# olsonanl/signature_kmers

Hardware: AMD Instinct MI355X
Metric: k-mers/sec (extract+hash+count) at 1/2/4/8 GPUs; achieved HBM GB/s % (higher is better)
Workload: dtype u8

## Files before the change

### signature_kmers_amd/__init__.py

```python
from __future__ import annotations

import ctypes as C
import os
from dataclasses import dataclass

import numpy as np

__all__ = [
    "SkmError", "lib", "K", "UNDEFINED_FUNCTION", "STORED_DTYPE", "CALL_DTYPE",
    "SignatureBuilder", "KeptKmers", "CmphKmerDb", "FunctionCaller", "mph_build",
    "kmer_to_str", "str_to_kmer", "keys_from_strings", "device_count", "MatrixDistance", "SeqIdMap",
    "matrix_tile_rows", "KeptKmerDb", "DeviceKeptKmerDb", "kept_db_plan", "kept_slot",
]

K = 8
UNDEFINED_FUNCTION = 0xFFFF
_HERE = os.path.dirname(os.path.abspath(__file__))
LIB_PATH = os.environ.get("SKM_LIB_PATH") or os.path.join(_HERE, "libskm.so")

STORED_DTYPE = np.dtype([("avg_from_end", "<u2"), ("function_index", "<u2"), ("mean", "<u2"),
                         ("median", "<u2"), ("var", "<u2")])
CALL_DTYPE = np.dtype([("start", "<u4"), ("end", "<u4"), ("count", "<i4"), ("function_index", "<u2"),
                       ("pad", "<u2"), ("protein_length_median", "<u4"),
                       ("protein_length_med_avg_dev", "<f4")])
# ... 269 lines not shown
    def __init__(self, k):
        self.k = k

    def __del__(self):
        try:
            lib().skm_kept_free(C.byref(self.k))
        except Exception:
            pass


class SignatureBuilder:

    def __init__(self, n_functions: int, max_seqs_per_file: int = 100000, device: int = 0, rank: int = 0,
                 world_size: int = 1):
        self._h = C.c_void_p()
        opts = _BuildOpts(8, max_seqs_per_file, n_functions, 1, rank, world_size)
        self.rank, self.world_size = rank, world_size
        dev = (C.c_int * 1)(device)
        _check(lib().skm_build_create(C.byref(self._h), dev, 1, C.byref(opts)))
        self.n_functions = n_functions
        self.device = device

    def add_batch(self, residues, seq_off, seq_len, seq_func, seq_id=None):
        residues = np.ascontiguousarray(residues, dtype=np.uint8)
        seq_off = np.ascontiguousarray(seq_off, dtype=np.uint64)
        seq_len = np.ascontiguousarray(seq_len, dtype=np.uint32)
        seq_func = np.ascontiguousarray(seq_func, dtype=np.uint16)
        n = len(seq_len)
        assert len(seq_off) == n and len(seq_func) == n
        if n:
            end = seq_off.astype(np.int64) + seq_len.astype(np.int64)
            if end.max() > len(residues):
                raise SkmError("seq_off/seq_len exceed the residue buffer")
        sid = None if seq_id is None else np.ascontiguousarray(seq_id, dtype=np.uint32)
        _check(lib().skm_build_add_batch(self._h, _ptr(residues), _ptr(seq_off), _ptr(seq_len), _ptr(seq_func),
                                         _ptr(sid) if sid is not None else None, n))

    def reserve(self, n_residues: int, n_seqs: int):
        _check(lib().skm_build_reserve(self._h, int(n_residues), int(n_seqs)))

    def set_transport(self, transport: "GlooTransport"):
        self._transport = transport
        _check(lib().skm_build_set_transport(self._h, transport.ptr))

    def set_comm(self, unique_id: bytes):
        buf = (C.c_uint8 * 128).from_buffer_copy(bytes(unique_id))
        _check(lib().skm_build_set_comm(self._h, buf))

    def prepare(self):
        _check(lib().skm_build_prepare(self._h))

    def run(self):
        _check(lib().skm_build_run(self._h))

    def timings(self) -> dict:
        ms = (C.c_float * 17)()
        n = lib().skm_build_last_timings(self._h, ms, 17)
        names = ["extract_count", "scan", "extract_scatter", "bucket_process", "overflow", "chains", "stats", "total",
                 "exchange", "partition", "bucket_kernel", "big_groups", "chain_tail", "giant_start", "giant_end",
                 "tail_wait", "groupby_wait"]
        return {names[i]: float(ms[i]) for i in range(n)}

    def set_kernel_timing(self, enable: bool, only: str | None = None):
        _check(lib().skm_build_set_kernel_timing(self._h, 1 if enable else 0, only.encode() if only else None))

    def kernel_timings(self) -> dict:
        n = lib().skm_build_kernel_timings(self._h, None, 0, None, None, 0)
        if n <= 0:
            return {}
        ms = (C.c_float * n)()
        cnt = (C.c_uint64 * n)()
        buf = C.create_string_buffer(64 * n + 64)
        lib().skm_build_kernel_timings(self._h, buf, len(buf), ms, cnt, n)
        names = buf.value.decode().split("\n")[:n]
        return {names[i]: (float(ms[i]), int(cnt[i])) for i in range(n)}

    def set_option(self, name: str, value: int):
        _check(lib().skm_build_set_option(self._h, name.encode(), int(value)))

    def passes(self) -> int:
        return self.counters()["passes"]

    def counters(self) -> dict:
        v = (C.c_uint64 * 50)()
        n = lib().skm_build_counters(self._h, v, 50)
        names = ["windows", "kept", "overflow_subbuckets", "chain_jobs", "chain_samples", "sequences", "grouped",
                 "overflow_elements", "overflow_kept", "big_groups", "big_kept", "passes", "valid", "giant_chains",
                 "giant_max", "redone", "cap_overflow_scratch", "cap_split", "cap_long_samples", "cap_long_jobs",
                 "demand_overflow_scratch", "demand_split", "demand_long_samples", "demand_long_jobs",
                 "long_samples", "routed", "add_batch_us", "prepare_upload_us", "prepare_plan_us", "prepare_rest_us",
                 "pass_groups", "add_pack_us", "add_dma_wait_us", "finish_us", "finish_wait_us", "finish_copy_us",
                 "finish_chunks", "finish_select_dev_us", "finish_sort_dev_us", "finish_gather_dev_us",
                 "finish_d2h_dev_us", "finish_max_chunk", "finish_wide_index", "kept_cap",
                 "free_after_prepare", "recs_rot", "overflow_light_subbuckets", "overflow_light_elements",
                 "groupby_tasks", "groupby_batches"]
        return {names[i]: int(v[i]) for i in range(n)}

    def debug_jobs(self, k: int = 64) -> list:
        v = (C.c_uint32 * k)()
        _check(lib().skm_build_debug_jobs(self._h, v, k))
        return [int(x) for x in v]

    def debug_overflow(self, k: int = 4096) -> list:
        v = (C.c_uint32 * k)()
        n = lib().skm_build_debug_overflow(self._h, v, k)
        return [int(x) for x in v[:min(max(n, 0), k)]]

    def debug_stamps(self, enable: bool) -> list:
        v = (C.c_uint64 * 32)()
        _check(lib().skm_build_debug_stamps(self._h, 1 if enable else 0, v, 32))
        return [int(x) for x in v]

    def finish(self) -> KeptKmers:
        k = _Kept()
        _check(lib().skm_build_finish(self._h, C.byref(k)))
        return self._kept(k)

    def finish_slice(self, slice_bits: int, slice_: int) -> KeptKmers:
        k = _Kept()
        _check(lib().skm_build_finish_slice(self._h, int(slice_bits), int(slice_), C.byref(k)))
        return self._kept(k)

    def signature_flags(self) -> np.ndarray:
        n = self.counters()["sequences"]
        out = np.zeros(max(n, 1), np.uint8)
        _check(lib().skm_build_signature_flags(self._h, _ptr(out), n))
        return out[:n]

    def kept_db(self, load_pct: int = 0, slots: int = 0, release_work: bool = False) -> "DeviceKeptKmerDb":
        opts = _KeptDbOpts(int(load_pct), 1 if release_work else 0, int(slots))
        h = C.c_void_p()
        _check(lib().skm_build_kept_db(self._h, C.byref(opts), C.byref(h)))
        return DeviceKeptKmerDb(h, self.device)

    def mph_db(self, seed: int = 1, release_work: bool = False, verify: bool = False, mph_path: str | None = None,
               dat_path: str | None = None) -> "CmphKmerDb":
        opts = _MphDbOpts(int(seed), 1 if release_work else 0, 1 if verify else 0, 0,
                          mph_path.encode() if mph_path else None, dat_path.encode() if dat_path else None)
        h = C.c_void_p()
        st = _MphStats()
        _check(lib().skm_build_mph_db(self._h, C.byref(opts), C.byref(h), C.byref(st)))
        db = CmphKmerDb(device=self.device, handle=h)
        db.stats = {n: getattr(st, n) for n, _ in _MphStats._fields_ if n != "pad"}
        return db

    @staticmethod
    def _kept(k) -> KeptKmers:
        owner = _KeptOwner(k)
        n = int(k.n)
        if n:
            kb = (C.c_char * (8 * n)).from_address(C.cast(k.keys, C.c_void_p).value)
            db = (C.c_char * (10 * n)).from_address(C.cast(k.data, C.c_void_p).value)
            kb._owner = db._owner = owner
            keys = np.frombuffer(kb, np.uint64)
            data = np.frombuffer(db, STORED_DTYPE)
        else:
            keys, data = np.zeros(0, np.uint64), np.zeros(0, STORED_DTYPE)
        nf = int(k.n_functions)
        df = np.ctypeslib.as_array(k.distinct_functions, shape=(max(nf, 1),))[:nf].copy()
        sw = np.ctypeslib.as_array(k.seqs_with_func, shape=(max(nf, 1),))[:nf].copy()
        return KeptKmers(keys, data, df, sw, int(k.n_seqs_with_signature), int(k.distinct_signatures),
                         int(k.n_windows))

    def close(self):
        if self._h:
            lib().skm_build_destroy(self._h)
            self._h = C.c_void_p()

    def __del__(self):
        try:
            self.close()
        except Exception:
            pass


class GlooTransport:

    def __init__(self):
# ... 743 lines not shown
```

### signature_kmers_amd/csrc/skm_build.hip

```cpp
#include <hip/hip_runtime.h>

#include <algorithm>
#include <type_traits>
#include <chrono>
#include <cmath>
#include <cstdio>
#include <cstdlib>
#include <cstring>
#include <deque>
#include <memory>
#include <numeric>
#include <string>
#include <thread>
#include <vector>

#include "skm_common.h"
#include "skm_keptdb.h"
#include "skm_mphdb.h"
#include "skm_pool.h"
#include "skm_output.h"
#include "skm_util.h"

#if defined(SKM_WITH_RCCL)
#include <rccl/rccl.h>
// ... 275 lines not shown
            uint32_t t = s_wave[w];
            s_wave[w] = acc;
            acc += t;
        }
        s_wave[nw] = acc;
    }
    __syncthreads();
    uint32_t r = s_wave[wave] + x - v;
    total = s_wave[nw];
    __syncthreads();
    return r;
}

__device__ __forceinline__ uint32_t wg_exclusive_scan1(uint32_t v, uint32_t* s_wave, uint32_t& total) {
    const uint32_t lane = threadIdx.x & 63u, wave = threadIdx.x >> 6, nw = blockDim.x >> 6;
    const uint32_t x = wave_incl_scan(v);
    if (lane == 63) s_wave[wave] = x;
    __syncthreads();
    uint32_t pre = 0, tot = 0;
    for (uint32_t w = 0; w < nw; ++w) {
        const uint32_t t = s_wave[w];
        pre += w < wave ? t : 0u;
        tot += t;
    }
    total = tot;
    return pre + x - v;
}

constexpr uint64_t LENS_SEL_SHIFT = 62;
constexpr uint64_t LENS_IN_RECS = 1, LENS_IN_TMP = 2, LENS_IN_BIG = 3;
constexpr uint64_t LENS_OFF_MASK = (1ull << LENS_SEL_SHIFT) - 1;
constexpr int SMALLC = 8;

struct Job {
    uint64_t lens_off;
    uint32_t n;
    uint32_t out_idx;
};

struct GRes {
    uint32_t best_f, avg, cbest, rb;
    uint16_t mean, median, var;
    bool kept;
};


struct GlbView {
    const uint64_t* hi;
    const uint64_t* lo;
    __device__ __forceinline__ uint32_t func(uint64_t j) const { return (uint32_t)(hi[j] & 0xFFFFu); }
    __device__ __forceinline__ uint64_t lov(uint64_t j) const { return lo[j]; }
};

template <int N>
__device__ __forceinline__ void reg_sort(uint32_t* v) {
#pragma unroll
    for (int k = 2; k <= N; k <<= 1)
#pragma unroll
        for (int j = k >> 1; j > 0; j >>= 1)
#pragma unroll
            for (int i = 0; i < N; ++i) {
                const int l = i ^ j;
                if (l > i) {
                    const bool asc = (i & k) == 0;
                    const uint32_t a = v[i], b = v[l];
                    v[i] = asc ? min(a, b) : max(a, b);
                    v[l] = asc ? max(a, b) : min(a, b);
                }
            }
}

__device__ __forceinline__ void stats_small(GRes& r, uint32_t x0, uint32_t x1, uint32_t n) {
    r.median = 0;
    r.var = 0;
    if (n == 2) {
        const uint16_t sum = (uint16_t)(x0 + x1);
        const double mean = (double)sum / 2.0;
        const double tmp = (double)x1 - mean;
        const double v = 0.0 * 1.0 / 2.0 + tmp * tmp / 1.0;
        r.var = d2u16(v);
    }
}

__device__ __forceinline__ void mark_seq(uint32_t* f, uint32_t s) {
    uint32_t* w = f + (s >> 5);
    const uint32_t m = 1u << (s & 31u);
    if (!(*w & m)) atomicOr(w, m);
}

template <int N>
__device__ __forceinline__ void mark_seqs(uint32_t* w, const uint32_t (&s)[N]) {
    uint32_t cur[N];
#pragma unroll
    for (int u = 0; u < N; ++u) cur[u] = s[u] != 0xFFFFFFFFu ? w[s[u] >> 5] : 0xFFFFFFFFu;
#pragma unroll
    for (int u = 0; u < N; ++u) {
        const uint32_t m = 1u << (s[u] & 31u);
        if (!(cur[u] & m)) atomicOr(w + (s[u] >> 5), m);
    }
}

struct Seq8 {
    uint32_t s[8];
};
__device__ __attribute__((noinline)) void mark_seqs8(uint32_t* w, Seq8 q) { mark_seqs<8>(w, q.s); }

template <int N, class V>
__device__ GRes group_thread(const V& v, uint64_t a, uint32_t c, const uint32_t* __restrict__ glen,
                             uint32_t* __restrict__ flags) {
    GRes r;
    r.kept = false;
    uint32_t fn[N], of[N];
#pragma unroll
    for (int t = 0; t < N; ++t) {
        if ((uint32_t)t < c) {
            fn[t] = v.func(a + t);
            of[t] = (uint32_t)(v.lov(a + t) & 0xFFFFu);
        } else {
            fn[t] = 0x10000u;
            of[t] = 0x10000u;
        }
    }
    uint32_t best_f = fn[0], best_c = 0, rb = 0, run_s = 0;
#pragma unroll
    for (int t = 1; t <= N; ++t) {
        if ((uint32_t)t <= c) {
            const bool end = ((uint32_t)t == c) || fn[t < N ? t : N - 1] != fn[t - 1];
            if (end) {
                const uint32_t len = t - run_s;
                if (len > best_c) {
                    best_c = len;
                    best_f = fn[t - 1];
                    rb = run_s;
                }
                run_s = t;
            }
        }
    }
    if ((float)best_c < float(c) * 0.8f) return r;
    r.kept = true;
    r.best_f = best_f;
    r.cbest = best_c;
    r.rb = rb;
    reg_sort<N>(of);
    const uint32_t k = c / 2;
    uint32_t avg = 0;
#pragma unroll
    for (int t = 0; t < N; ++t)
        if ((uint32_t)t == k) avg = of[t];
    r.avg = avg;
    uint32_t sum = 0;
    uint32_t lr0 = 0, lr1 = 0;
    for (uint32_t t = 0; t < c; ++t) {
        const uint64_t lo = v.lov(a + t);
        const uint32_t s = (uint32_t)(lo >> 36);
        mark_seq(flags, s);
        if (t >= rb && t < rb + best_c) {
            const uint32_t len = glen[s];
            sum += len;
            const uint32_t q = rb + best_c - 1 - t;
            if (q == 0) lr0 = len;
            if (q == 1) lr1 = len;
        }
    }
    r.mean = d2u16((double)(uint16_t)sum / (double)best_c);
    r.median = 0;
    r.var = 0;
    if (best_c <= 2) stats_small(r, lr0, lr1, best_c);
    return r;
}

template <class V>
__device__ GRes group_wave(const V& v, uint64_t a, uint32_t c, const uint32_t* __restrict__ glen,
                           uint32_t* __restrict__ flags) {
    const uint32_t lane = threadIdx.x & 63u;
    GRes r;
    r.kept = false;
    uint32_t best_f = 0, best_c = 0, rb = 0, run_s = 0;
    uint32_t run_f = v.func(a);
    for (uint32_t base = 0; base < c; base += 64) {
        const uint32_t t = base + lane;
        const bool valid = t < c;
        const uint32_t f = valid ? v.func(a + t) : 0xFFFFFFFFu;
        const uint32_t fp = (valid && t > 0) ? v.func(a + t - 1) : 0xFFFFFFFFu;
        uint64_t m = __ballot(valid && t > 0 && f != fp);
        while (m) {
            const int q = __ffsll((long long)m) - 1;
            m &= m - 1;
            const uint32_t pos = base + (uint32_t)q;
            const uint32_t len = pos - run_s;
            if (len > best_c) {
                best_c = len;
                best_f = run_f;
                rb = run_s;
            }
            run_s = pos;
            run_f = (uint32_t)__shfl((int)f, q, 64);
        }
    }
    {
        const uint32_t len = c - run_s;
        if (len > best_c) {
            best_c = len;
            best_f = run_f;
            rb = run_s;
        }
    }
    if ((float)best_c < float(c) * 0.8f) return r;
    r.kept = true;
    r.best_f = best_f;
    r.cbest = best_c;
    r.rb = rb;
    uint32_t vmin = 0xFFFFu, vmax = 0;
    for (uint32_t t = lane; t < c; t += 64) {
        const uint32_t o = (uint32_t)(v.lov(a + t) & 0xFFFFu);
        vmin = min(vmin, o);
        vmax = max(vmax, o);
    }
    vmin = wave_min(vmin);
    vmax = wave_max(vmax);
    const uint32_t k = c / 2;
    while (vmin < vmax) {
        const uint32_t mid = (vmin + vmax) >> 1;
        uint32_t cnt = 0;
        for (uint32_t t = lane; t < c; t += 64) cnt += (uint32_t)(v.lov(a + t) & 0xFFFFu) <= mid;
        cnt = wave_sum(cnt);
        if (cnt >= k + 1)
            vmax = mid;
        else
            vmin = mid + 1;
    }
    r.avg = vmin;
    uint32_t sum = 0;
    for (uint32_t t = lane; t < c; t += 64) {
        const uint32_t s = (uint32_t)(v.lov(a + t) >> 36);
        mark_seq(flags, s);
        if (t >= rb && t < rb + best_c) sum += glen[s];
    }
    sum = wave_sum(sum);
    r.mean = d2u16((double)(uint16_t)sum / (double)best_c);
    r.median = 0;
    r.var = 0;
    return r;
}

__device__ __forceinline__ uint32_t wg_sum(uint32_t x, uint32_t* s_wave) {
    const uint32_t lane = threadIdx.x & 63u, wave = threadIdx.x >> 6, nw = blockDim.x >> 6;
    x = wave_sum(x);
    if (lane == 0) s_wave[wave] = x;
    __syncthreads();
    uint32_t t = 0;
    for (uint32_t w = 0; w < nw; ++w) t += s_wave[w];
    __syncthreads();
    return t;
}

__device__ __forceinline__ uint32_t wg_max(uint32_t x, uint32_t* s_wave) {
    const uint32_t lane = threadIdx.x & 63u, wave = threadIdx.x >> 6, nw = blockDim.x >> 6;
    x = wave_max(x);
    if (lane == 0) s_wave[wave] = x;
    __syncthreads();
    uint32_t t = 0;
    for (uint32_t w = 0; w < nw; ++w) t = max(t, s_wave[w]);
    __syncthreads();
    return t;
}

__device__ __forceinline__ uint32_t wg_min(uint32_t x, uint32_t* s_wave) {
    const uint32_t lane = threadIdx.x & 63u, wave = threadIdx.x >> 6, nw = blockDim.x >> 6;
    x = wave_min(x);
    if (lane == 0) s_wave[wave] = x;
    __syncthreads();
    uint32_t t = 0xFFFFFFFFu;
    for (uint32_t w = 0; w < nw; ++w) t = min(t, s_wave[w]);
    __syncthreads();
    return t;
}

template <class V>
__device__ bool group_block(const V& v, uint64_t a, uint32_t c, const uint32_t* __restrict__ glen,
                            uint32_t* __restrict__ flags, uint32_t* heads, uint32_t hcap, uint32_t* s_wave, GRes& r) {
    const uint32_t tid = threadIdx.x, nt = blockDim.x;
    r.kept = false;
    uint32_t H = 0;
    for (uint32_t t0 = 0; t0 < c; t0 += nt) {
        const uint32_t t = t0 + tid;
        const bool head = t < c && (t == 0 || v.func(a + t) != v.func(a + t - 1));
        uint32_t tot;
        const uint32_t pos = wg_exclusive_scan(head ? 1u : 0u, s_wave, tot);
        if (head && H + pos < hcap) heads[H + pos] = t;
        H += tot;
    }
    if (H > hcap) return false;
    __syncthreads();
    uint32_t lmax = 0;
    for (uint32_t j = tid; j < H; j += nt) lmax = max(lmax, (j + 1 < H ? heads[j + 1] : c) - heads[j]);
    const uint32_t best_c = wg_max(lmax, s_wave);
    uint32_t fmin = 0xFFFFFFFFu;
    for (uint32_t j = tid; j < H; j += nt)
        if ((j + 1 < H ? heads[j + 1] : c) - heads[j] == best_c) fmin = min(fmin, (v.func(a + heads[j]) << 16) | j);
    const uint32_t fj = wg_min(fmin, s_wave);
    if ((float)best_c < float(c) * 0.8f) return true;
    const uint32_t rb = heads[fj & 0xFFFFu];
    r.kept = true;
    r.best_f = fj >> 16;
    r.cbest = best_c;
    r.rb = rb;
    uint32_t k = c / 2, pre = 0;
    for (int b = 15; b >= 0; --b) {
        uint32_t n0 = 0;
        for (uint32_t t = tid; t < c; t += nt) {
            const uint32_t o = (uint32_t)(v.lov(a + t) & 0xFFFFu);
            n0 += (o >> b) == (pre >> b);
        }
        n0 = wg_sum(n0, s_wave);
        if (k >= n0) {
            k -= n0;
            pre |= 1u << b;
        }
    }
    r.avg = pre;
    uint32_t sum = 0;
    for (uint32_t t = tid; t < c; t += nt) {
        const uint32_t s = (uint32_t)(v.lov(a + t) >> 36);
        mark_seq(flags, s);
        if (t >= rb && t < rb + best_c) sum += glen[s];
    }
    sum = wg_sum(sum, s_wave);
    r.mean = d2u16((double)(uint16_t)sum / (double)best_c);
    r.median = 0;
    r.var = 0;
    return true;
}

enum : uint32_t {
    RUN_FLAGS = 0,
    RUN_LONG_CUR = 1,
    RUN_LONG_N = 2,
    RUN_LONG_FLUSHED = 3,
    RUN_ACC_BPK_TASKS = 4,
    RUN_ACC_BPK_BATCHES = 5,
    RUN_SNAP = 28,
    RUN_DEM_TOT = 8,
    RUN_DEM_SPLIT = 9,
    RUN_DEM_LONG = 10,
    RUN_DEM_LJOBS = 11,
    RUN_LONG_WANT = 12,
    RUN_LONG_WANTJ = 13,
    RUN_ACC_LIGHT_SUB = 14,
    RUN_ACC_LIGHT_ELEMS = 15,
    RUN_ACC_NOVF = 16,
    RUN_ACC_JOBS = 17,
    RUN_ACC_LENS = 18,
    RUN_ACC_OVF_ELEMS = 19,
    RUN_ACC_OVF_KEPT = 20,
    RUN_ACC_BIG = 21,
    RUN_ACC_BIG_KEPT = 22,
    RUN_ACC_GROUPED = 23,
    RUN_LAST_NOVF = 24,
    RUN_LAST_JOBS = 25,
    RUN_NLOC = 26,
    RUN_SLOTS = 64
};
constexpr unsigned long long RUN_F_ARENA = 1;
constexpr unsigned long long RUN_F_RERUN = 2;
constexpr unsigned long long RUN_F_CAP = 4;
enum : uint32_t {
    PLAN_NOVF = 0,
    PLAN_NSPLIT = 1,
    PLAN_NHEAVY = 2,
    PLAN_SKIP = 3,
    PLAN_Q_SPLIT = 4,
    PLAN_Q_HEAVY = 5,
    PLAN_Q_REST = 6,
    PLAN_Q_LIGHT = 7,
    PLAN_ELEMS = 8,
    PLAN_NLOC = 9,
    PLAN_SLOTS = 16
};

constexpr int JOB_CLASSES = 32;
constexpr int JOB_WG = 256;

__device__ __forceinline__ uint32_t job_class(uint32_t n) { return 31u - (uint32_t)__clz(n | 1u); }

__device__ __forceinline__ void job_chunk(const unsigned long long* nj_p, uint64_t cap, uint64_t& a, uint64_t& e) {
    const uint64_t nj = min((uint64_t)*nj_p, cap);
    const uint64_t chunk = (nj + gridDim.x - 1) / gridDim.x;
    a = min(nj, (uint64_t)blockIdx.x * chunk);
    e = min(nj, a + chunk);
}

__global__ __launch_bounds__(JOB_WG) void k_job_count(const Job* __restrict__ jobs, const unsigned long long* nj_p,
                                                      uint64_t cap, uint32_t* __restrict__ hist) {
    __shared__ uint32_t h[JOB_CLASSES];
    if (threadIdx.x < JOB_CLASSES) h[threadIdx.x] = 0;
    __syncthreads();
    uint64_t a, e;
    job_chunk(nj_p, cap, a, e);
    for (uint64_t j = a + threadIdx.x; j < e; j += blockDim.x) atomicAdd(&h[job_class(jobs[j].n)], 1u);
    __syncthreads();
    if (threadIdx.x < JOB_CLASSES) hist[blockIdx.x * JOB_CLASSES + threadIdx.x] = h[threadIdx.x];
}

constexpr uint32_t LONG_CLASS = 14;

__global__ void k_job_scan(const uint32_t* __restrict__ hist, uint32_t nwg, uint64_t* __restrict__ offs,
                           uint32_t long_class) {
    __shared__ uint64_t tot[JOB_CLASSES];
    const uint32_t c = threadIdx.x;
    if (c < JOB_CLASSES) {
        uint64_t t = 0;
        for (uint32_t w = 0; w < nwg; ++w) t += hist[w * JOB_CLASSES + c];
        tot[c] = t;
    }
    __syncthreads();
    if (c == 0) {
        uint64_t nl = 0;
        for (uint32_t cc = long_class; cc < JOB_CLASSES; ++cc) nl += tot[cc];
        offs[(uint64_t)nwg * JOB_CLASSES] = nl;
    }
    if (c < JOB_CLASSES) {
        uint64_t base = 0;
        for (uint32_t cc = JOB_CLASSES - 1; cc > c; --cc) base += tot[cc];
// ... 1414 lines not shown
    if (b >= NB) return;
    uint32_t w0 = rb * SCAN_ROWS, w1 = min(nwg, w0 + SCAN_ROWS);
    uint32_t s = 0;
    for (uint32_t w = w0; w < w1; ++w) s += hist[(uint64_t)w * NB + b];
    partial[(uint64_t)rb * NB + b] = s;
}

__global__ void k_bstart(const uint32_t* __restrict__ partial, uint32_t nrb, uint32_t NB, int b1_bits,
                         uint32_t* __restrict__ rbbase, uint32_t* __restrict__ bstart, uint64_t* __restrict__ owner_start,
                         uint32_t nowners) {
    __shared__ uint32_t s_wave[34];
    __shared__ unsigned long long s_tot[64];
    const uint32_t per = (NB + blockDim.x - 1) / blockDim.x;
    const uint32_t b0 = threadIdx.x * per;
    uint32_t local = 0;
    for (uint32_t b = b0; b < min(NB, b0 + per); ++b) {
        uint32_t acc = 0;
        for (uint32_t rb = 0; rb < nrb; ++rb) {
            uint32_t v = partial[(uint64_t)rb * NB + b];
            rbbase[(uint64_t)rb * NB + b] = acc;
            acc += v;
        }
        bstart[b] = acc;
        local += acc;
    }
    uint32_t total;
    uint32_t ex = wg_exclusive_scan(local, s_wave, total);
    uint32_t run = ex;
    for (uint32_t b = b0; b < min(NB, b0 + per); ++b) {
        uint32_t t = bstart[b];
        bstart[b] = run;
        run += t;
    }
    __syncthreads();
    if (threadIdx.x < nowners) {
        uint32_t ob = threadIdx.x << b1_bits;
        s_tot[threadIdx.x] = bstart[ob];
    }
    if (threadIdx.x == 0) s_tot[nowners] = total;
    __syncthreads();
    if (threadIdx.x <= nowners) owner_start[threadIdx.x] = s_tot[threadIdx.x];
    for (uint32_t b = b0; b < min(NB, b0 + per); ++b) {
        uint32_t o = b >> b1_bits;
        uint32_t rel = bstart[b] - (uint32_t)s_tot[o];
        for (uint32_t rb = 0; rb < nrb; ++rb) rbbase[(uint64_t)rb * NB + b] += rel;
    }
    __syncthreads();
    for (uint32_t b = b0; b < min(NB, b0 + per); ++b) bstart[b] -= (uint32_t)s_tot[b >> b1_bits];
    if (threadIdx.x == 0) bstart[NB] = 0;
}

__global__ void k_coloffs(const uint32_t* __restrict__ hist, const uint32_t* __restrict__ rbbase, uint32_t nwg, uint32_t NB,
                          uint32_t* __restrict__ offs) {
    uint32_t b = blockIdx.x * blockDim.x + threadIdx.x;
    uint32_t rb = blockIdx.y;
    if (b >= NB) return;
    uint32_t w0 = rb * SCAN_ROWS, w1 = min(nwg, w0 + SCAN_ROWS);
    uint32_t run = rbbase[(uint64_t)rb * NB + b];
    for (uint32_t w = w0; w < w1; ++w) {
        uint64_t idx = (uint64_t)w * NB + b;
        uint32_t v = hist[idx];
        offs[idx] = run;
        run += v;
    }
}

struct BucketArgs {
    uint64_t* recs_hi;
    const uint64_t* recs_lo;
    uint64_t* tmp_hi;
    uint64_t* tmp_lo;
    const uint64_t* bstart;
    const uint64_t* seg_start;
    const uint32_t* seg_len;
    uint32_t nsrc;
    uint32_t* sub_tab;
    unsigned long long* kept_ctr;

    uint32_t nbuckets;
    uint32_t bucket_base;
    int rem_bits;
    const uint32_t* glen;
    uint32_t* flags;
    unsigned long long* ctr;
    uint64_t* out_keys;
    skm_stored_kmer_data* out_data;
    Job* jobs;
    uint32_t* lens;
    OvfEntry* ovf;
    uint32_t ovf_cap;
    unsigned long long* stamps;
    uint64_t* big_desc;
    uint32_t big_cap;
    unsigned long long* big_ctr;
    int prio;
    int pshift;
    const uint32_t* skip;
    uint32_t sub_target;
    const uint32_t* order;
};

#define SKM_STAMP(i)                                                          \
    do {                                                                      \
        if (A.stamps && threadIdx.x == 0) {                                   \
            const uint64_t _t = __builtin_amdgcn_s_memtime();                 \
            atomicAdd(&A.stamps[(i)], (unsigned long long)(_t - *L.tlast));   \
            *L.tlast = _t;                                                    \
        }                                                                     \
    } while (0)

constexpr uint32_t JOB_KEPT = 0x8000u;
constexpr uint32_t JOB_COUNT_MASK = 0x0FFFu;

struct SubLds {
    uint64_t* hi;
    uint64_t* lo;
    uint32_t* tab;
    uint16_t* slot;
    uint16_t* rank;
    uint16_t* goff;
    uint16_t* glist;
    uint16_t* order;
    uint16_t* big;
    uint32_t* wave;
    uint32_t* nbig;
    uint64_t* tlast;
    uint32_t* ccnt;
    uint32_t* lens32;
    uint64_t lens_sel;
};

__device__ __forceinline__ uint64_t kept_hi(uint64_t h43, uint32_t avg) { return (1ull << 63) | (h43 << 16) | avg; }
__device__ __forceinline__ uint64_t kept_lo(uint32_t f, uint32_t mean, uint32_t med, uint32_t var) {
    return (uint64_t)f | ((uint64_t)mean << 16) | ((uint64_t)med << 32) | ((uint64_t)var << 48);
}

__device__ __forceinline__ void write_kept(const BucketArgs& A, uint64_t o, uint64_t H, uint64_t L) {
    A.out_keys[o] = (H >> 16) & KEY_MASK;
    skm_stored_kmer_data d;
    d.avg_from_end = (uint16_t)(H & 0xFFFFu);
    d.function_index = (uint16_t)(L & 0xFFFFu);
    d.mean = (uint16_t)(L >> 16);
    d.median = (uint16_t)(L >> 32);
    d.var = (uint16_t)(L >> 48);
    A.out_data[o] = d;
}



__device__ __forceinline__ uint64_t shfl_xor_u64(uint64_t v, int m) {
    return ((uint64_t)(uint32_t)__shfl_xor((int)(uint32_t)(v >> 32), m, 64) << 32) |
           (uint32_t)__shfl_xor((int)(uint32_t)v, m, 64);
}


__device__ __forceinline__ void bm_combine(uint32_t& cand, uint32_t& cc) {
#pragma unroll
    for (int d = 1; d < 64; d <<= 1) {
        const uint32_t oc = xs(cand, d), on = xs(cc, d);
        if (oc == cand) {
            cc += on;
        } else if (cc >= on) {
            cc -= on;
        } else {
            cand = oc;
            cc = on - cc;
// ... 19 lines not shown
        }
    }
    return key;
}

template <int S>
__device__ __forceinline__ uint32_t seg_bitonic32(uint32_t key, uint32_t m) {
#pragma unroll
    for (int k = 2; k <= S; k <<= 1) {
#pragma unroll
        for (int j = k >> 1; j > 0; j >>= 1) {
            const uint32_t ok = xs(key, j);
            const bool take_min = ((m & (uint32_t)j) == 0) == ((m & (uint32_t)k) == 0);
            key = take_min ? min(key, ok) : max(key, ok);
        }
    }
    return key;
}

template <int S>
__device__ __forceinline__ uint32_t seg_reduce_max(uint32_t x) {
#pragma unroll
    for (int d = 1; d < S; d <<= 1) x = max(x, xs(x, d));
    return x;
}

template <int S>
__device__ __forceinline__ uint32_t seg_reduce_sum(uint32_t x) {
#pragma unroll
    for (int d = 1; d < S; d <<= 1) x += xs(x, d);
    return x;
}

template <int S>
__device__ __forceinline__ void seg_groups(const SubLds& L, uint32_t q0, uint32_t qend, uint32_t G, uint32_t M,
                                           const BucketArgs& A, uint64_t hprefix, uint32_t* jobinfo,
                                           uint32_t* fmean) {
    const uint32_t lane = threadIdx.x & 63u;
    const uint32_t m = lane & (uint32_t)(S - 1);
    const uint32_t sbase = lane - m;
    const uint32_t q = q0 + lane / (uint32_t)S;
    const bool gv = q < qend;
    uint32_t rep = 0, a = 0, c = 0;
    if (gv) {
        const uint32_t g = L.big[q];
        rep = L.glist[g];
        a = L.goff[rep];
        c = (g + 1 < G ? L.goff[L.glist[g + 1]] : M) - a;
    }
    const bool real = gv && m < c;
    uint64_t key = ~0ull;
    uint32_t pay = 0;
    if (real) {
        const uint32_t j = L.order[a + m];
        const uint64_t hj = L.hi[j], lj = L.lo[j];
        key = ((hj & 0xFFFFull) << 48) | (lj >> 16);
        pay = (uint32_t)(hj >> 47);
    }
    key = seg_bitonic64<S>(key, pay, m);
    const uint32_t f = (uint32_t)(key >> 48);
    const uint32_t fprev = (uint32_t)__shfl_up((int)f, 1, 64);
    const bool head = !real || m == 0 || f != fprev;
    const uint64_t H = __ballot(head);
    const uint64_t above = lane == 63 ? 0ull : (H & ~((2ull << lane) - 1ull));
    const uint32_t nh = above ? (uint32_t)__ffsll((long long)above) - 1u : 64u;
    const uint32_t rlen = min(nh, sbase + c) - lane;
    const uint32_t v = (real && head) ? ((rlen << 16) | (0xFFFFu - f)) : 0u;
    const uint32_t best = seg_reduce_max<S>(v);
    const uint32_t cbest = best >> 16, bf = 0xFFFFu - (best & 0xFFFFu);
    const bool kept = gv && !((float)cbest < float(c) * 0.8f);
    const bool inrun = real && f == bf;
    const uint32_t len16 = pay >> 1;
    const uint32_t sum = seg_reduce_sum<S>(inrun ? len16 : 0u);
    const uint32_t i = (uint32_t)(key & ((1u << ELEM_I_BITS) - 1));
    const uint32_t off = real ? ((len16 - i) & 0xFFFFu) : 0x10000u;
    const uint32_t osort = seg_bitonic32<S>(off, m);
    const uint32_t avg = (uint32_t)__shfl((int)osort, (int)(sbase + (c >> 1)), 64);
    const uint64_t R = __ballot(inrun);
    const uint64_t segmask = (S == 64) ? ~0ull : (((1ull << S) - 1ull) << sbase);
    const uint64_t Rs = R & segmask;
    const uint32_t rs = Rs ? (uint32_t)__ffsll((long long)Rs) - 1u : sbase;
    const uint32_t s = (uint32_t)(key >> ELEM_I_BITS) & ((1u << ELEM_S_BITS) - 1u);
    const uint32_t len = (pay & 1u) ? A.glen[s] : len16;
    if (kept && real) mark_seq(A.flags, s);
    const uint32_t x0 = (uint32_t)__shfl((int)len, (int)(rs + cbest - 1), 64);
    const uint32_t x1 = (uint32_t)__shfl((int)len, (int)rs, 64);
    if (kept && inrun && cbest >= 3) L.lens32[2 * a + (rs + cbest - 1 - lane)] = len;
    if (kept && m == 0) {
        GRes r;
        r.kept = true;
        r.best_f = bf;
        r.cbest = cbest;
        r.avg = avg;
        r.mean = d2u16((double)(uint16_t)sum / (double)cbest);
        stats_small(r, x0, cbest == 2 ? x1 : 0u, cbest);
        const uint64_t h43 = key_h43(hprefix, (L.hi[rep] >> 16) & REM_MASK, A.rem_bits, A.pshift);
        L.hi[rep] = kept_hi(h43, r.avg);
        if (cbest >= 3) {
            jobinfo[rep] = (a << 16) | JOB_KEPT | cbest;
            fmean[rep] = bf | ((uint32_t)r.mean << 16);
        } else {
            jobinfo[rep] = JOB_KEPT;
            L.lo[rep] = kept_lo(bf, r.mean, r.median, r.var);
        }
    }
}

constexpr uint32_t LPER = CAP / BPK_THREADS;

__device__ __forceinline__ void load_batch(const uint64_t* __restrict__ src_hi, const uint64_t* __restrict__ src_lo,
                                           uint32_t n, uint64_t (&eh)[LPER], uint64_t (&el)[LPER]) {
#pragma unroll
    for (uint32_t u = 0; u < LPER; ++u) {
        const uint32_t j = threadIdx.x + u * BPK_THREADS;
        if (j < n) {
            eh[u] = __builtin_nontemporal_load(src_hi + j);
            el[u] = __builtin_nontemporal_load(src_lo + j);
        }
    }
}

__device__ __forceinline__ uint32_t process_sub(const uint64_t* __restrict__ src_hi, const uint64_t* __restrict__ src_lo,
                                            uint32_t n, const BucketArgs& A, uint64_t hprefix, const SubLds& L) {
    const uint32_t tid = threadIdx.x, nt = blockDim.x;
    const uint32_t EMPTY = 0xFFFFFFFFu;
    uint64_t eh[LPER], el[LPER];
    load_batch(src_hi, src_lo, n, eh, el);
    for (uint32_t t = tid; t < (uint32_t)TAB; t += nt) L.tab[t] = EMPTY;
#pragma unroll
    for (uint32_t u = 0; u < LPER; ++u) {
        const uint32_t j = tid + u * BPK_THREADS;
        if (j < n) {
            L.hi[j] = eh[u];
            L.lo[j] = el[u];
        }
    }
    if (tid == 0) *L.nbig = 0;
    if (tid < 8) L.ccnt[tid] = 0;
    __syncthreads();
    SKM_STAMP(2);
    for (uint32_t j = tid; j < n; j += nt) {
        const uint32_t rem = (uint32_t)(L.hi[j] >> 16) & REM_MASK;
        uint32_t slot = (rem * 0x9E3779B1u) >> (32 - TAB_BITS);
        uint32_t rk = 0;
        while (true) {
            const uint32_t cur = atomicCAS(&L.tab[slot], EMPTY, (j << 16) | 1u);
            if (cur == EMPTY) break;
            if (((uint32_t)(L.hi[cur >> 16] >> 16) & REM_MASK) == rem) {
                rk = atomicAdd(&L.tab[slot], 1u) & 0xFFFFu;
                break;
            }
            slot = (slot + 1) & (TAB - 1);
        }
        L.slot[j] = (uint16_t)slot;
        L.rank[j] = (uint16_t)rk;
    }
    __syncthreads();
    SKM_STAMP(3);
    uint32_t M = 0, G = 0;
    {
        const uint32_t j0 = tid * LPER;
        uint32_t ev[LPER], loc = 0;
#pragma unroll
        for (uint32_t u = 0; u < LPER; ++u) {
            const uint32_t j = j0 + u;
            ev[u] = j < n ? L.tab[L.slot[j]] : 0u;
            const uint32_t cnt = ev[u] & 0xFFFFu;
            loc += (cnt > 1 && (ev[u] >> 16) == j) ? ((cnt << 13) | 1u) : 0u;
        }
        uint32_t tot;
        uint32_t v = wg_exclusive_scan1(loc, L.wave, tot);
        uint32_t ms[LPER];
#pragma unroll
        for (uint32_t u = 0; u < LPER; ++u) {
            const uint32_t j = j0 + u;
            const uint32_t cnt = ev[u] & 0xFFFFu;
            ms[u] = 0xFFFFFFFFu;
            if (j < n && cnt > 1 && (ev[u] >> 16) == j) {
                L.goff[j] = (uint16_t)(v >> 13);
                L.glist[v & 0x1FFFu] = (uint16_t)j;
                v += (cnt << 13) | 1u;
            } else if (j < n && cnt == 1) {
                const uint64_t H = L.hi[j], Lo = L.lo[j];
                ms[u] = (uint32_t)(Lo >> 36);
                L.hi[j] = kept_hi(key_h43(hprefix, (H >> 16) & REM_MASK, A.rem_bits, A.pshift), (uint32_t)(Lo & 0xFFFFu));
                L.lo[j] = kept_lo((uint32_t)(H & 0xFFFFu), d2u16((double)(uint16_t)(H >> 48) / 1.0), 0, 0);
                L.rank[j] = 0xFFFFu;
            }
        }
        mark_seqs<LPER>(A.flags, ms);
        M = tot >> 13;
        G = tot & 0x1FFFu;
    }
    __syncthreads();
    SKM_STAMP(4);
    for (uint32_t j = tid; j < n; j += nt) {
        const uint32_t e = L.tab[L.slot[j]];
        if ((e & 0xFFFFu) > 1) L.order[L.goff[e >> 16] + L.rank[j]] = (uint16_t)j;
    }
    uint32_t* ccnt = L.ccnt;
    auto cls_of = [](uint32_t c) -> uint32_t {
        return c > 64u ? 6u : 31u - (uint32_t)__clz(c - 1u) - 0u;
    };
    for (uint32_t g = tid; g < G; g += nt) {
        const uint32_t a = L.goff[L.glist[g]];
        const uint32_t c = g + 1 < G ? L.goff[L.glist[g + 1]] - a : M - a;
        atomicAdd(&ccnt[cls_of(c)], 1u);
    }
    __syncthreads();
    SKM_STAMP(5);
    uint32_t* jobinfo = L.tab;
    uint32_t* fmean = L.tab + CAP;
    for (uint32_t j = tid; j < n; j += nt) jobinfo[j] = L.rank[j] == 0xFFFFu ? JOB_KEPT : 0u;
    uint32_t* cstart = ccnt + 8;
    uint32_t* tstart = ccnt + 16;
    if (tid == 0) {
        uint32_t run = 0, acc = 0;
        for (int q = 0; q < 7; ++q) {
            const uint32_t t = ccnt[q];
            ccnt[q] = run;
            cstart[q] = run;
            tstart[q] = acc;
            const uint32_t per = q < 6 ? (64u >> (q + 1)) : 1u;
            acc += (t + per - 1) / per;
            run += t;
        }
        cstart[7] = run;
        tstart[7] = acc;
    }
    unsigned long long big_base = 0;
    if (tid == 0 && cstart[7] > cstart[6]) big_base = atomicAdd(A.big_ctr, (unsigned long long)(cstart[7] - cstart[6]));
    __syncthreads();
    for (uint32_t g = tid; g < G; g += nt) {
        const uint32_t a = L.goff[L.glist[g]];
        const uint32_t c = g + 1 < G ? L.goff[L.glist[g + 1]] - a : M - a;
        L.big[atomicAdd(&ccnt[cls_of(c)], 1u)] = (uint16_t)g;
    }
    if (tid == 0) *reinterpret_cast<unsigned long long*>(L.wave + 44) = big_base;
    __syncthreads();
    SKM_STAMP(6);
    {
        const uint32_t ntask = tstart[6];
        const uint32_t nbig = cstart[7] - cstart[6];
        const uint64_t bbase = *reinterpret_cast<const unsigned long long*>(L.wave + 44);
        const uint32_t wave = tid >> 6, nwaves = nt >> 6, lane = tid & 63u;
        uint64_t* slots = reinterpret_cast<uint64_t*>(L.lens32);
        uint64_t* slots_lo = const_cast<uint64_t*>(src_lo);
        (void)wave;
        (void)nwaves;
        for (;;) {
            uint32_t t = 0;
            if (lane == 0) t = atomicAdd(&ccnt[7], 1u);
            t = (uint32_t)__builtin_amdgcn_readfirstlane((int)t);
            if (t >= nbig + ntask) break;
            if (t < nbig) {
                const uint32_t g = L.big[cstart[6] + t];
                const uint32_t rep = L.glist[g];
                const uint32_t a = L.goff[rep];
                const uint32_t c = g + 1 < G ? L.goff[L.glist[g + 1]] - a : M - a;
                for (uint32_t u = lane; u < c; u += 64) {
                    const uint32_t j = L.order[a + u];
                    const uint64_t hj = L.hi[j], lj = L.lo[j];
                    slots[a + u] = ((hj & 0xFFFFull) << 48) | (lj >> 16);
                    slots_lo[a + u] = elem_len(hj, lj, A.glen);
                }
                const uint64_t q = bbase + t;
                if (lane == 0 && q < A.big_cap) {
                    A.big_desc[2 * q] = key_h43(hprefix, (L.hi[rep] >> 16) & REM_MASK, A.rem_bits, A.pshift) |
                                        ((uint64_t)c << KEY_BITS);
                    A.big_desc[2 * q + 1] = L.lens_sel + 2 * a;
                }
                continue;
            }
// ... 141 lines not shown
        __syncthreads();
        if (task >= ntasks) break;
        const uint32_t bucket = task / BPK_PARTS, part = task % BPK_PARTS;
        const uint64_t r0 = A.bstart[bucket], r1 = A.bstart[bucket + 1];
        const uint64_t n = r1 - r0;
        if (n == 0) continue;
        const uint64_t hprefix = (uint64_t)(A.bucket_base + bucket) << A.rem_bits;

        const bool direct = n <= (uint64_t)CAP && A.nsrc == 1;
        uint32_t nsub = 1;
        if (direct) {
            if (part) continue;
        } else {
            const uint32_t* tab = A.sub_tab + (uint64_t)bucket * SUB_TAB;
            const uint32_t all = tab[0];
            const uint32_t d0 = (uint32_t)((uint64_t)part * all / BPK_PARTS), d1 = (uint32_t)((uint64_t)(part + 1) * all / BPK_PARTS);
            if (d0 == d1) continue;
            nsub = d1 - d0;
            for (uint32_t d = threadIdx.x; d <= nsub; d += blockDim.x) s_sub[d] = tab[1 + d0 + d];
            __syncthreads();
            SKM_STAMP(9);
        }
        struct Batch {
            uint32_t a, cnt;
        };
        auto next_batch = [&](uint32_t& d) -> Batch {
            if (direct) {
                if (d >= 1) return Batch{0, 0};
                d = 1;
                return Batch{0, (uint32_t)n};
            }
            while (d < nsub) {
                const uint32_t a = s_sub[d];
                if (s_sub[d + 1] - a == 0 || s_sub[d + 1] - a > (uint32_t)CAP) {
                    ++d;
                    continue;
                }
                uint32_t d2 = d + 1;
                while (d2 < nsub && s_sub[d2 + 1] - a <= (uint32_t)CAP) ++d2;
                d = d2;
                return Batch{a, s_sub[d2] - a};
            }
            return Batch{0, 0};
        };
        const uint64_t* base_hi = A.tmp_hi + r0;
        const uint64_t* base_lo = A.tmp_lo + r0;
        const uint64_t sel = LENS_IN_TMP;
        uint32_t d = 0, nb = 0;
        for (Batch cur = next_batch(d); cur.cnt; cur = next_batch(d)) {
            L.lens_sel = (sel << LENS_SEL_SHIFT) | (2 * (r0 + cur.a));
            L.lens32 = reinterpret_cast<uint32_t*>(const_cast<uint64_t*>(base_hi + cur.a));
            process_sub(base_hi + cur.a, base_lo + cur.a, cur.cnt, A, hprefix, L);
            __syncthreads();
            SKM_STAMP(10);
            ++nb;
        }
        worked += nb ? 1u : 0u;
        batches += nb;
    }
    if (threadIdx.x == 0 && worked) {
        atomicAdd(&A.ctr[CTR_BPK_TASKS], (unsigned long long)worked);
        atomicAdd(&A.ctr[CTR_BPK_BATCHES], (unsigned long long)batches);
    }
}

struct BigOut {
    uint64_t h43;
    uint64_t lens_off;
    uint32_t n;
    uint16_t avg, func, mean, pad0;
    uint32_t pad1;
};
static_assert(sizeof(BigOut) == 32, "BigOut layout");

struct BigArgs {
    const uint64_t* desc;
    const unsigned long long* ndesc;
    uint32_t cap;
    const uint64_t* recs_hi;
    const uint64_t* tmp_hi;
    const uint64_t* recs_lo;
    const uint64_t* tmp_lo;
    uint32_t* flags;
    BigOut* out;
};

template <int E>
__device__ __forceinline__ uint32_t ballot_count(const bool (&p)[E]) {
    uint32_t n = 0;
#pragma unroll
    for (int e = 0; e < E; ++e) n += (uint32_t)__popcll(__ballot(p[e]));
    return n;
}

template <int E, int D>
__device__ __forceinline__ void bitonic_cross(uint64_t (&ky)[E], bool take_min) {
#pragma unroll
    for (int e = 0; e < E; ++e) {
        const uint64_t o = xshfl64<D>(ky[e]);
        ky[e] = take_min ? (o < ky[e] ? o : ky[e]) : (o > ky[e] ? o : ky[e]);
    }
}

template <int E>
__device__ __forceinline__ void big_group(const BigArgs& B, uint64_t g, uint64_t* mem, const uint64_t* mlen,
                                          uint32_t c, uint64_t h43, uint64_t lens_off) {
    const uint32_t lane = threadIdx.x & 63u;
    uint32_t fo[E];
    uint64_t ky[E];
#pragma unroll
    for (int e = 0; e < E; ++e) {
        const uint32_t t = lane * E + (uint32_t)e;
        fo[e] = 0xFFFFFFFFu;
        ky[e] = ~0ull;
        if (t < c) {
            const uint64_t v = mem[t];
            const uint32_t len = (uint32_t)mlen[t];
            const uint32_t i = (uint32_t)v & ((1u << ELEM_I_BITS) - 1u);
            fo[e] = ((uint32_t)(v >> 48) << 16) | ((len - i) & 0xFFFFu);
            ky[e] = (v << 16) | t;
        }
    }
    uint32_t cand = 0xFFFFFFFFu, cc = 0;
#pragma unroll
    for (int e = 0; e < E; ++e) {
        if (fo[e] != 0xFFFFFFFFu) {
            const uint32_t f = fo[e] >> 16;
            if (cc == 0) {
                cand = f;
                cc = 1;
            } else if (f == cand) {
                ++cc;
            } else {
                --cc;
            }
        }
    }
    bm_combine(cand, cc);
    bool p[E];
#pragma unroll
    for (int e = 0; e < E; ++e) p[e] = (fo[e] >> 16) == cand;
    const uint32_t nb = ballot_count<E>(p);
    BigOut o;
    o.h43 = h43;
    o.lens_off = lens_off;
    o.n = 0;
    o.avg = o.func = o.mean = 0;
    o.pad0 = 0;
    o.pad1 = 0;
    if ((float)nb < float(c) * 0.8f) {
        if (lane == 0) B.out[g] = o;
        return;
    }
    constexpr int MC = E < 8 ? E : 8;
#pragma unroll
    for (int e0 = 0; e0 < E; e0 += MC) {
        uint32_t ms[MC];
#pragma unroll
        for (int u = 0; u < MC; ++u)
            ms[u] = fo[e0 + u] != 0xFFFFFFFFu ? (uint32_t)(ky[e0 + u] >> (16 + ELEM_I_BITS)) : 0xFFFFFFFFu;
        if constexpr (E > 16) {
            Seq8 q;
#pragma unroll
            for (int u = 0; u < 8; ++u) q.s[u] = ms[u];
            mark_seqs8(B.flags, q);
        } else {
            mark_seqs<MC>(B.flags, ms);
        }
    }
    uint32_t sum = 0;
#pragma unroll
    for (int e = 0; e < E; ++e) {
        if (fo[e] != 0xFFFFFFFFu && p[e]) sum += (uint32_t)mlen[ky[e] & 0xFFFFu];
        if (!p[e]) ky[e] = ~0ull;
    }
    sum = wave_sum(sum);
    uint32_t k = c / 2, pre = 0;
#pragma unroll 1
    for (int b = 15; b >= 0; --b) {
#pragma unroll
        for (int e = 0; e < E; ++e) {
            const uint32_t v = fo[e] == 0xFFFFFFFFu ? 0x10000u : (fo[e] & 0xFFFFu);
            p[e] = ((v >> b) ^ (pre >> b)) == 0u;
        }
        const uint32_t n0 = ballot_count<E>(p);
        if (k >= n0) {
            k -= n0;
            pre |= 1u << b;
        }
    }
#pragma unroll 1
    for (uint32_t kk = 2; kk <= 64u * E; kk <<= 1) {
        const bool asc_lane = ((lane * (uint32_t)E) & kk) == 0;
#pragma unroll 1
        for (uint32_t jj = kk >> 1; jj >= (uint32_t)E; jj >>= 1) {
            const uint32_t d = jj / (uint32_t)E;
            const bool take_min = ((lane & d) == 0) == asc_lane;
            switch (d) {
                case 1: bitonic_cross<E, 1>(ky, take_min); break;
                case 2: bitonic_cross<E, 2>(ky, take_min); break;
                case 4: bitonic_cross<E, 4>(ky, take_min); break;
                case 8: bitonic_cross<E, 8>(ky, take_min); break;
                case 16: bitonic_cross<E, 16>(ky, take_min); break;
                default: bitonic_cross<E, 32>(ky, take_min); break;
            }
        }
#pragma unroll
        for (int jj = E / 2; jj > 0; jj >>= 1) {
            if ((uint32_t)jj < kk) {
#pragma unroll
                for (int e = 0; e < E; ++e) {
                    const int l = e ^ jj;
                    if (l > e) {
                        const bool asc = (((lane * (uint32_t)E) + (uint32_t)e) & kk) == 0;
                        const uint64_t x = ky[e], y = ky[l];
                        const bool sw = asc ? (y < x) : (x < y);
                        ky[e] = sw ? y : x;
                        ky[l] = sw ? x : y;
                    }
                }
            }
        }
    }
    uint32_t* lens = reinterpret_cast<uint32_t*>(mem);
#pragma unroll
    for (int e = 0; e < E; ++e) {
        const uint32_t t = lane * E + (uint32_t)e;
        if (t < nb) lens[nb - 1 - t] = (uint32_t)mlen[ky[e] & 0xFFFFu];
    }
    o.n = nb;
    o.avg = (uint16_t)pre;
    o.func = (uint16_t)cand;
    o.mean = d2u16((double)(uint16_t)sum / (double)nb);
    if (lane == 0) B.out[g] = o;
}

constexpr int BIG_WG = 256;

template <bool LARGE>
__global__ __launch_bounds__(BIG_WG, LARGE ? 3 : 4) void k_big_groups(BigArgs B) {
    const uint64_t nd = min((uint64_t)*B.ndesc, (uint64_t)B.cap);
    const uint64_t nw = (uint64_t)gridDim.x * (BIG_WG / 64);
    for (uint64_t g = (uint64_t)blockIdx.x * (BIG_WG / 64) + (threadIdx.x >> 6); g < nd; g += nw) {
        const uint64_t d0 = B.desc[2 * g], d1 = B.desc[2 * g + 1];
        const uint32_t c = (uint32_t)(d0 >> KEY_BITS);
        if (LARGE != (c > 1024u)) continue;
        const uint64_t h43 = d0 & KEY_MASK;
        const uint64_t sel = d1 >> LENS_SEL_SHIFT, off = d1 & LENS_OFF_MASK;
        uint64_t* mem = const_cast<uint64_t*>(sel == LENS_IN_RECS ? B.recs_hi : B.tmp_hi) + off / 2;
        const uint64_t* mlen = (sel == LENS_IN_RECS ? B.recs_lo : B.tmp_lo) + off / 2;
// ... 341 lines not shown
                    s_lo[j] = ~0ull;
                }
            }
            __syncthreads();
            bitonic_lds(s_hi, s_lo, CAP, 2, CAP, CAP);
            for (uint32_t j = tid; j < CAP; j += nt) {
                ghi[c0 + j] = s_hi[j];
                glo[c0 + j] = s_lo[j];
            }
            __threadfence_block();
            __syncthreads();
        }
        for (uint32_t k = 2 * CAP; k <= N; k <<= 1) {
            for (uint32_t j = k >> 1; j >= (uint32_t)CAP; j >>= 1) {
                for (uint32_t t = tid; t < N / 2; t += nt) {
                    const uint32_t i = 2 * t - (t & (j - 1));
                    if (i >= nch) continue;
                    const uint32_t l = j == (k >> 1) ? (i ^ (k - 1)) : i + j;
                    const uint64_t ah = ghi[i], al = glo[i], bh = ghi[l], bl = glo[l];
                    if (elem_less(bh, bl, ah, al)) {
                        ghi[i] = bh;
                        glo[i] = bl;
                        ghi[l] = ah;
                        glo[l] = al;
                    }
                }
                __threadfence_block();
                __syncthreads();
            }
            for (uint32_t c0 = 0; c0 < nch; c0 += CAP) {
                for (uint32_t j = tid; j < CAP; j += nt) {
                    s_hi[j] = ghi[c0 + j];
                    s_lo[j] = glo[c0 + j];
                }
                __syncthreads();
                bitonic_lds(s_hi, s_lo, CAP, k, k, CAP >> 1);
                for (uint32_t j = tid; j < CAP; j += nt) {
                    ghi[c0 + j] = s_hi[j];
                    glo[c0 + j] = s_lo[j];
                }
                __threadfence_block();
                __syncthreads();
            }
        }
        uint32_t G = 0;
        for (uint32_t c0 = 0; c0 < n; c0 += nt) {
            const uint32_t t = c0 + tid;
            const bool head = t < n && (t == 0 || (ghi[t] >> 16) != (ghi[t - 1] >> 16));
            uint32_t tot;
            const uint32_t pos = wg_exclusive_scan(head ? 1u : 0u, s_wave, tot);
            if (head) {
                heads[G + pos] = t;
                jobinfo[t] = 0;
            }
            G += tot;
        }
        __threadfence_block();
        __syncthreads();
        const GlbView V{ghi, glo};
        auto stage = [&](const GRes& r, uint32_t a) {
            if (!r.kept) return;
            const uint64_t h43 = key_h43(hprefix, ghi[a] >> 16, A.rem_bits, A.pshift);
            if (r.cbest >= 3) {
                jobinfo[a] = ((uint64_t)(a + r.rb) << 32) | r.cbest;
                fmean[a] = r.best_f | ((uint32_t)r.mean << 16);
            } else {
                glo[a] = kept_lo(r.best_f, r.mean, r.median, r.var);
            }
            ghi[a] = kept_hi(h43, r.avg);
        };
        for (uint32_t g0 = 0; g0 < G; g0 += nt) {
            if (tid == 0) s_nbig = 0;
            __syncthreads();
            const uint32_t g = g0 + tid;
            if (g < G) {
                const uint32_t a = heads[g];
                const uint32_t b = g + 1 < G ? heads[g + 1] : n;
                const uint32_t c = b - a;
                if (c > (uint32_t)SMALLC) {
                    s_big[atomicAdd(&s_nbig, 1u)] = g;
                } else {
                    GRes r;
                    if (c <= 4)
                        r = group_thread<4>(V, a, c, A.glen, A.flags);
                    else if (c <= 8)
                        r = group_thread<8>(V, a, c, A.glen, A.flags);
                    else
                        r = group_thread<16>(V, a, c, A.glen, A.flags);
                    stage(r, a);
                }
            }
            __syncthreads();
            const uint32_t nbig = s_nbig;
            for (uint32_t bi = tid >> 6; bi < nbig; bi += nt >> 6) {
                const uint32_t gg = s_big[bi];
                const uint32_t a = heads[gg];
                const uint32_t b = gg + 1 < G ? heads[gg + 1] : n;
                if (b - a > OVF_BLOCK_GROUP) continue;
                const GRes r = group_wave(V, a, b - a, A.glen, A.flags);
                if ((tid & 63u) == 0) stage(r, a);
            }
            for (uint32_t bi = 0; bi < nbig; ++bi) {
                const uint32_t gg = s_big[bi];
                const uint32_t a = heads[gg];
                const uint32_t b = gg + 1 < G ? heads[gg + 1] : n;
                if (b - a <= OVF_BLOCK_GROUP) continue;
                GRes r;
                if (!group_block(V, a, b - a, A.glen, A.flags, reinterpret_cast<uint32_t*>(s_hi), 2 * CAP, s_wave, r)) {
                    if (tid < 64) r = group_wave(V, a, b - a, A.glen, A.flags);
                }
                if (tid == 0) stage(r, a);
                __syncthreads();
            }
            __threadfence_block();
            __syncthreads();
        }
        unsigned long long* s_base = reinterpret_cast<unsigned long long*>(s_wave + 36);
        for (uint32_t g0 = 0; g0 < G; g0 += nt) {
            const uint32_t g = g0 + tid;
            const uint32_t a = g < G ? heads[g] : 0u;
            const uint64_t H = g < G ? ghi[a] : 0ull;
            const bool kept = (H >> 63) != 0;
            const uint64_t jb = kept ? jobinfo[a] : 0ull;
            const uint32_t jn = (uint32_t)(jb & 0xFFFFFFFFu);
            uint32_t islot = OVF_INLINE_CAP;
            if (jn >= inline_min) islot = atomicAdd(&s_ninl, 1u);
            const bool inl = islot < OVF_INLINE_CAP;
            uint32_t K, J, Lt;
            const uint32_t kpos = wg_exclusive_scan(kept ? 1u : 0u, s_wave, K);
            const uint32_t jpos = wg_exclusive_scan((jn && !inl) ? 1u : 0u, s_wave, J);
            const uint32_t lpos = wg_exclusive_scan(jn, s_wave, Lt);
            if (K == 0) continue;
            if (tid == 0) {
                s_base[0] = atomicAdd(A.kept_ctr, (unsigned long long)K);
                atomicAdd(&A.ctr[0], (unsigned long long)K);
                if (J) {
                    s_base[1] = atomicAdd(&A.ctr[3], (unsigned long long)J);
                    s_base[2] = atomicAdd(&A.ctr[4], (unsigned long long)Lt);
                }
                s_nbig = 0;
            }
            __syncthreads();
            if (kept) {
                const uint64_t o = s_base[0] + kpos;
                if (jn) {
                    const uint32_t fm = fmean[a];
                    write_kept(A, o, H, kept_lo(fm & 0xFFFFu, fm >> 16, 0, 0));
                    Job jbr;
                    jbr.lens_off = s_base[2] + lpos;
                    jbr.n = jn;
                    jbr.out_idx = (uint32_t)o;
                    if (inl) {
                        s_inl[islot][0] = jbr.lens_off;
                        s_inl[islot][1] = ((uint64_t)jn << 32) | (uint32_t)o;
                    } else {
                        A.jobs[s_base[1] + jpos] = jbr;
                    }
                    if (jn <= 64) {
                        const uint64_t start = jb >> 32;
                        for (uint32_t t = 0; t < jn; ++t)
                            A.lens[jbr.lens_off + t] = A.glen[glo[start + jn - 1 - t] >> 36];
                    } else {
                        const uint32_t bi = atomicAdd(&s_nbig, 1u);
                        s_big[bi] = g;
                        s_lo[bi] = jbr.lens_off;
                    }
                } else {
                    write_kept(A, o, H, glo[a]);
                }
            }
            __syncthreads();
            const uint32_t nb = s_nbig;
            for (uint32_t q = 0; q < nb; ++q) {
                const uint32_t gg = s_big[q];
                const uint32_t aa = heads[gg];
                const uint64_t jbq = jobinfo[aa];
                const uint32_t nq = (uint32_t)(jbq & 0xFFFFFFFFu);
                const uint64_t start = jbq >> 32;
                const uint64_t loff = s_lo[q];
                for (uint32_t t = tid; t < nq; t += nt) A.lens[loff + t] = A.glen[glo[start + nq - 1 - t] >> 36];
            }
            __syncthreads();
        }
        __threadfence_block();
        __syncthreads();
        const uint32_t ninl = min(s_ninl, OVF_INLINE_CAP);
        const uint32_t wave = tid >> 6, pairs = (nt >> 6) / 2;
        if (ninl && prio == 1) __builtin_amdgcn_s_setprio(1);
        if (ninl && prio == 2) __builtin_amdgcn_s_setprio(2);
        if (ninl && prio >= 3) __builtin_amdgcn_s_setprio(3);
        for (uint32_t q = wave / 2; q < ninl; q += pairs) {
            const uint64_t off = s_inl[q][0], w = s_inl[q][1];
// ... 301 lines not shown
            }
            const uint32_t pre = (uint32_t)__popcll(peers & lt);
            const uint32_t tg = tag & 0x1FFFFFFu;
            if (v && pre == 0) s_wc[wave][d] = (tg << 7) | (uint32_t)__popcll(peers);
            __syncthreads();
            if (v) {
                uint32_t o = s_run[d] + pre;
                for (uint32_t w = 0; w < wave; ++w) {
                    const uint32_t c = s_wc[w][d];
                    if ((c >> 7) == tg) o += c & 127u;
                }
                b[o] = k;
            }
            __syncthreads();
            for (uint32_t dd = tid; dd < RBINS; dd += nt) {
                uint32_t add = 0;
                for (uint32_t w = 0; w < nw; ++w) {
                    const uint32_t c = s_wc[w][dd];
                    if ((c >> 7) == tg) add += c & 127u;
                }
                s_run[dd] += add;
            }
            __syncthreads();
        }
        uint32_t* t = a;
        a = b;
        b = t;
    }
    return a;
}

constexpr uint32_t HV_FT = 4096;
constexpr uint32_t HV_NBK = 4096;
constexpr uint32_t HV_BCAP = 512;

__device__ __forceinline__ void wave_hist_add(uint32_t* h, uint32_t bin, bool v) {
    const uint32_t lane = threadIdx.x & 63u;
    uint64_t act = __ballot(v);
    while (act) {
        const uint32_t l0 = (uint32_t)__ffsll((long long)act) - 1u;
        const uint32_t b0 = (uint32_t)__builtin_amdgcn_readlane((int)bin, (int)l0);
        const uint64_t m = __ballot(v && bin == b0) & act;
        if (lane == l0) atomicAdd(&h[b0], (uint32_t)__popcll(m));
        act &= ~m;
    }
}

template <int E>
__device__ __forceinline__ void wave_sort_desc(uint64_t (&v)[E]) {
    const uint32_t lane = threadIdx.x & 63u;
#pragma unroll
    for (int k = 2; k <= 64 * E; k <<= 1) {
#pragma unroll
        for (int j = k >> 1; j > 0; j >>= 1) {
            if (j >= 64) {
#pragma unroll
                for (int e = 0; e < E; ++e) {
                    const int pe = e ^ (j >> 6);
                    if (pe > e) {
                        const bool up = (((uint32_t)e * 64u + lane) & (uint32_t)k) == 0;
                        const uint64_t a = v[e], b = v[pe];
                        if (up ? a < b : a > b) {
                            v[e] = b;
                            v[pe] = a;
                        }
                    }
                }
            } else {
#pragma unroll
                for (int e = 0; e < E; ++e) {
                    const uint32_t i = (uint32_t)e * 64u + lane;
                    const uint64_t o = xs64(v[e], j);
                    const bool keep_max = ((i & (uint32_t)j) == 0) == ((i & (uint32_t)k) == 0);
                    v[e] = keep_max ? (v[e] > o ? v[e] : o) : (v[e] < o ? v[e] : o);
                }
            }
        }
    }
}

template <int E>
__device__ __forceinline__ void heavy_bucket_out(const uint32_t* __restrict__ ks, const uint32_t* __restrict__ ls,
                                                 uint32_t a, uint32_t c, uint32_t nb, uint32_t* __restrict__ out,
                                                 uint32_t* flags) {
    const uint32_t lane = threadIdx.x & 63u;
    uint64_t v[E];
#pragma unroll
    for (int e = 0; e < E; ++e) {
        const uint32_t i = (uint32_t)e * 64u + lane;
        v[e] = i < c ? ((uint64_t)ks[a + i] << 32) | ls[a + i] : 0ull;
    }
    wave_sort_desc<E>(v);
#pragma unroll
    for (int e = 0; e < E; ++e) {
        const uint32_t i = (uint32_t)e * 64u + lane;
        if (i < nb) {
            out[i] = (uint32_t)v[e];
            mark_seq(flags, (uint32_t)(v[e] >> 32) - 1u);
        }
    }
}

__global__ __launch_bounds__(HEAVY_WG) void k_heavy(BucketArgs A, HeavyArgs H) {
    static_assert(RBINS <= HEAVY_WG, "one radix bin per thread in the scan");
    __shared__ uint32_t s_hist[RBINS], s_run[RBINS + 48];
    __shared__ uint32_t s_wc[HEAVY_WG / 64][RBINS];
    __shared__ __align__(16) uint32_t s_wave[48];
    __shared__ uint32_t s_bm[2 * (HEAVY_WG / 64)];
    __shared__ uint32_t s_cur, s_sel[3], s_key;
    __shared__ uint32_t s_fb[HV_FT];
    __shared__ uint32_t s_bk[HV_NBK];
    __shared__ uint32_t s_oh[256], s_ol[256];
    static_assert(HV_FT == HV_NBK, "s_fb doubles as the per-bucket best counts");
    const uint32_t tid = threadIdx.x, nt = blockDim.x, lane = tid & 63u, wave = tid >> 6, nw = nt >> 6;
    const uint64_t lt = (1ull << lane) - 1ull;
    const uint32_t nkeys = (uint32_t)*H.nkeys;
    uint32_t tag = 0;
    for (uint32_t q = tid; q < (HEAVY_WG / 64) * RBINS; q += nt) (&s_wc[0][0])[q] = 0;
    __syncthreads();
    constexpr uint32_t U = SPLIT_U;
    for (;;) {
        __syncthreads();
        if (tid == 0) s_key = (uint32_t)min((unsigned long long)nkeys, atomicAdd(H.queue, 1ull));
        __syncthreads();
        const uint32_t q = s_key;
        if (q >= nkeys) break;
        const HeavyKey K = H.keys[q];
        const uint64_t* rec = H.rec + K.off;
        const uint32_t* rlen = H.len + K.off;
        const uint32_t n = K.n;
        uint32_t best_f = 0, cb = 0, NBK = 0;
        bool bucketed = false;
        if (H.fast) {
            NBK = 1;
            while (NBK < HV_NBK && NBK * 256u < n) NBK <<= 1;
            for (uint32_t d = tid; d < HV_FT; d += nt) s_fb[d] = 0;
            for (uint32_t d = tid; d < NBK; d += nt) s_bk[d] = 0;
            for (uint32_t d = tid; d < 256; d += nt) s_oh[d] = 0;
            __syncthreads();
            for (uint32_t j0 = 0; j0 < n; j0 += nt * U) {
                uint64_t x[U];
#pragma unroll
                for (uint32_t u = 0; u < U; ++u) {
                    const uint32_t j = j0 + u * nt + tid;
                    x[u] = j < n ? rec[j] : ~0ull;
                }
#pragma unroll
                for (uint32_t u = 0; u < U; ++u) {
                    const bool v = x[u] != ~0ull;
                    const uint32_t f = v ? hr_func(x[u]) : 0xFFFFFFFFu;
                    const uint32_t f0 = (uint32_t)__builtin_amdgcn_readfirstlane((int)f);
                    const uint64_t same = __ballot(v && f == f0);
                    if (v && f != f0) atomicAdd(&s_fb[f], 1u);
                    if (v && f == f0 && (same & lt) == 0) atomicAdd(&s_fb[f], (uint32_t)__popcll(same));
                    wave_hist_add(s_oh, hr_off(x[u]) >> 8, v);
                    if (v) atomicAdd(&s_bk[(uint32_t)(((uint64_t)hr_seq(x[u]) * NBK) / H.n_total)], 1u);
                }
            }
            __syncthreads();
            uint32_t cm = 0;
            for (uint32_t d = tid; d < HV_FT; d += nt) cm = max(cm, s_fb[d]);
            cm = wg_max(cm, s_wave);
            uint32_t fm = 0;
            for (uint32_t d = tid; d < HV_FT; d += nt)
                if (s_fb[d] == cm) fm = max(fm, HV_FT - 1u - d);
            fm = wg_max(fm, s_wave);
            best_f = HV_FT - 1u - fm;
            cb = cm;
            uint32_t bm = 0;
            for (uint32_t d = tid; d < NBK; d += nt) bm = max(bm, s_bk[d]);
            bm = wg_max(bm, s_wave);
            bucketed = bm <= HV_BCAP;
        } else {
            uint32_t cand = 0xFFFFFFFFu, cc = 0;
            for (uint32_t j0 = 0; j0 < n; j0 += nt * U) {
                uint32_t f[U];
    #pragma unroll
                for (uint32_t u = 0; u < U; ++u) {
                    const uint32_t j = j0 + u * nt + tid;
                    f[u] = j < n ? hr_func(rec[j]) : 0xFFFFFFFFu;
                }
// ... 22 lines not shown
                    const uint32_t c1 = s_bm[2 * w], n1 = s_bm[2 * w + 1];
                    if (c1 == c0) {
                        n0 += n1;
                    } else if (n0 >= n1) {
                        n0 -= n1;
                    } else {
                        c0 = c1;
                        n0 = n1 - n0;
                    }
                }
                s_sel[0] = c0;
            }
            __syncthreads();
            best_f = s_sel[0];
            cb = 0;
            for (uint32_t j0 = 0; j0 < n; j0 += nt * U) {
                uint32_t f[U];
    #pragma unroll
                for (uint32_t u = 0; u < U; ++u) {
                    const uint32_t j = j0 + u * nt + tid;
                    f[u] = j < n ? hr_func(rec[j]) : 0xFFFFFFFFu;
                }
    #pragma unroll
                for (uint32_t u = 0; u < U; ++u) cb += f[u] == best_f;
            }
            cb = wg_sum(cb, s_wave);
        }
        if ((float)cb < float(n) * 0.8f) continue;
        uint32_t pre = 0;
        uint16_t mean = 0;
        const uint32_t* sorted = nullptr;
        if (bucketed) {
            {
                const uint32_t per = (NBK + nt - 1) / nt, b0 = min(NBK, tid * per), b1 = min(NBK, b0 + per);
                uint32_t loc = 0;
                for (uint32_t d = b0; d < b1; ++d) loc += s_bk[d];
                uint32_t tot;
                uint32_t x = wg_exclusive_scan(loc, s_wave, tot);
                for (uint32_t d = b0; d < b1; ++d) {
                    const uint32_t c = s_bk[d];
                    s_bk[d] = x;
                    x += c;
                }
            }
            for (uint32_t d = tid; d < NBK; d += nt) s_fb[d] = 0;
            for (uint32_t d = tid; d < 256; d += nt) s_ol[d] = 0;
            if (tid == 0) {
                uint32_t kk = n / 2, d = 0;
                while (kk >= s_oh[d]) kk -= s_oh[d++];
                s_sel[0] = d;
                s_sel[1] = kk;
            }
            __syncthreads();
            const uint32_t hb = s_sel[0], krem = s_sel[1];
            uint32_t* ks = H.s0 + K.off;
            uint32_t* ls = H.s1 + K.off;
            uint32_t sum = 0;
            for (uint32_t j0 = 0; j0 < n; j0 += nt * U) {
                uint64_t x[U];
                uint32_t ln[U];
#pragma unroll
                for (uint32_t u = 0; u < U; ++u) {
                    const uint32_t j = j0 + u * nt + tid;
                    x[u] = j < n ? rec[j] : ~0ull;
                    ln[u] = j < n ? rlen[j] : 0u;
                }
#pragma unroll
                for (uint32_t u = 0; u < U; ++u) {
                    if (x[u] == ~0ull) continue;
                    const uint32_t sq = hr_seq(x[u]);
                    const uint32_t bk = (uint32_t)(((uint64_t)sq * NBK) / H.n_total);
                    const uint32_t off = hr_off(x[u]);
                    if ((off >> 8) == hb) atomicAdd(&s_ol[off & 255u], 1u);
                    const bool best = hr_func(x[u]) == best_f;
                    const uint32_t slot = atomicAdd(&s_bk[bk], 1u);
                    if (best) {
                        sum += ln[u] & 0xFFFFu;
                        atomicAdd(&s_fb[bk], 1u);
                        ks[slot] = sq + 1u;
                        ls[slot] = ln[u];
                    } else {
                        ks[slot] = 0u;
                        ls[slot] = 0u;
                        mark_seq(A.flags, sq);
                    }
                }
            }
            sum = wg_sum(sum, s_wave);
            mean = d2u16((double)(uint16_t)sum / (double)cb);
            if (tid == 0) {
                uint32_t kk = krem, d = 0;
                while (kk >= s_ol[d]) kk -= s_ol[d++];
                s_sel[0] = (hb << 8) | d;
            }
            {
                const uint32_t per = (NBK + nt - 1) / nt, r0 = min(NBK, tid * per), r1 = min(NBK, r0 + per);
                uint32_t loc = 0;
                for (uint32_t r = r0; r < r1; ++r) loc += s_fb[NBK - 1 - r];
                uint32_t tot;
                uint32_t x = wg_exclusive_scan(loc, s_wave, tot);
                for (uint32_t r = r0; r < r1; ++r) {
                    const uint32_t c = s_fb[NBK - 1 - r];
                    s_fb[NBK - 1 - r] = x;
                    x += c;
                }
            }
            __syncthreads();
            pre = s_sel[0];
        } else {
            if (tid == 0) s_cur = 0;
            for (uint32_t d = tid; d < 256; d += nt) s_hist[d] = 0;
            __syncthreads();
            uint32_t* sa = H.s0 + K.off;
            uint32_t* sb = H.s1 + K.off;
            uint32_t sum = 0, smax = 0;
            for (uint32_t j0 = 0; j0 < n; j0 += nt * U) {
                uint64_t l[U];
                uint32_t f[U], gl[U];
    #pragma unroll
                for (uint32_t u = 0; u < U; ++u) {
                    const uint32_t j = j0 + u * nt + tid;
                    const uint64_t x = j < n ? rec[j] : ~0ull;
                    f[u] = j < n ? hr_func(x) : 0xFFFFFFFFu;
                    gl[u] = j < n ? rlen[j] & 0xFFFFu : 0u;
                    l[u] = x;
                }
    #pragma unroll
                for (uint32_t u = 0; u < U; ++u) gl[u] = f[u] == best_f ? gl[u] : 0u;
    #pragma unroll
                for (uint32_t u = 0; u < U; ++u) {
                    const bool v = f[u] != 0xFFFFFFFFu;
                    const uint32_t s = hr_seq(l[u]);
                    const bool best = f[u] == best_f;
                    if (v && !best) mark_seq(A.flags, s);
                    wave_hist_add(s_hist, hr_off(l[u]) >> 8, v);
                    if (best) {
                        sum += gl[u];
                        smax = max(smax, s);
                    }
                    const uint64_t bm = __ballot(best);
                    uint32_t base = 0;
                    if (bm) {
                        const uint32_t leader = (uint32_t)(__ffsll((long long)bm) - 1);
                        if (lane == leader) base = atomicAdd(&s_cur, (uint32_t)__popcll(bm));
                        base = (uint32_t)__shfl((int)base, (int)leader, 64);
                    }
                    if (best) sa[base + (uint32_t)__popcll(bm & lt)] = s;
                }
            }
            sum = wg_sum(sum, s_wave);
            smax = wg_max(smax, s_wave);
            mean = d2u16((double)(uint16_t)sum / (double)cb);
            uint32_t k = n / 2;
            for (int sh = 8; sh >= 0; sh -= 8) {
                if (sh == 0) {
                    for (uint32_t d = tid; d < 256; d += nt) s_hist[d] = 0;
                    __syncthreads();
                    for (uint32_t j0 = 0; j0 < n; j0 += nt * U) {
                        uint32_t o[U];
    #pragma unroll
                        for (uint32_t u = 0; u < U; ++u) {
                            const uint32_t j = j0 + u * nt + tid;
                            o[u] = j < n ? hr_off(rec[j]) : 0xFFFFFFFFu;
                        }
    #pragma unroll
                        for (uint32_t u = 0; u < U; ++u)
                            if (o[u] != 0xFFFFFFFFu && (o[u] >> 8) == (pre >> 8)) atomicAdd(&s_hist[o[u] & 255u], 1u);
                    }
                }
                __syncthreads();
                if (tid == 0) {
                    uint32_t d = 0;
                    while (k >= s_hist[d]) k -= s_hist[d++];
                    s_sel[0] = d;
                    s_sel[1] = k;
                }
                __syncthreads();
                pre |= s_sel[0] << sh;
                k = s_sel[1];
                __syncthreads();
            }
            int bits = 0;
            while (bits < 32 && (smax >> bits)) bits += RB;
            sorted = wg_radix_sort_u32(sa, sb, cb, bits, s_hist, s_wc, s_run, tag);
            __syncthreads();
        }
        if (tid == 0) {
            s_sel[0] = (uint32_t)atomicAdd(A.kept_ctr, 1ull);
            atomicAdd(&A.ctr[0], 1ull);
            bool g = false;
            if (H.giant_min && cb >= H.giant_min) {
                const uint64_t c = atomicAdd(&H.gcount[1], (unsigned long long)cb);
                if (c + cb <= H.gcap) {
                    g = true;
                    s_cur = (uint32_t)c;
                    s_sel[1] = (uint32_t)atomicAdd(&H.gcount[0], 1ull);
                    atomicAdd(&H.gstat[0], 1ull);
                    atomicMax(&H.gstat[1], (unsigned long long)cb);
                }
            }
            if (!g) {
                s_sel[1] = (uint32_t)atomicAdd(&A.ctr[3], 1ull);
                s_cur = (uint32_t)atomicAdd(&A.ctr[4], (unsigned long long)cb);
            }
            s_sel[2] = g ? 1u : 0u;
        }
        __syncthreads();
        const uint32_t o = s_sel[0], jb = s_sel[1], loff = s_cur;
        const bool giant = s_sel[2] != 0;
        uint32_t* lens_out = giant ? H.gsamples : A.lens;
        if (bucketed) {
            const uint32_t* ks = H.s0 + K.off;
            const uint32_t* ls = H.s1 + K.off;
            for (uint32_t bk = wave; bk < NBK; bk += nw) {
                const uint32_t a = bk ? s_bk[bk - 1] : 0u, c = s_bk[bk] - a;
                const uint32_t nb = (bk ? s_fb[bk - 1] : cb) - s_fb[bk];
                if (nb == 0) continue;
                uint32_t* out = lens_out + (uint64_t)loff + s_fb[bk];
                if (c <= 64)
                    heavy_bucket_out<1>(ks, ls, a, c, nb, out, A.flags);
                else if (c <= 128)
                    heavy_bucket_out<2>(ks, ls, a, c, nb, out, A.flags);
                else if (c <= 256)
                    heavy_bucket_out<4>(ks, ls, a, c, nb, out, A.flags);
                else
                    heavy_bucket_out<8>(ks, ls, a, c, nb, out, A.flags);
            }
        } else {
            for (uint32_t t0 = 0; t0 < cb; t0 += nt * U) {
                uint32_t sv[U];
    #pragma unroll
                for (uint32_t u = 0; u < U; ++u) {
                    const uint32_t t = t0 + u * nt + tid;
                    sv[u] = t < cb ? sorted[cb - 1 - t] : 0u;
                }
    #pragma unroll
                for (uint32_t u = 0; u < U; ++u) {
                    const uint32_t t = t0 + u * nt + tid;
                    if (t < cb) {
                        lens_out[(uint64_t)loff + t] = A.glen[sv[u]];
                        mark_seq(A.flags, sv[u]);
                    }
                }
            }
        }
        if (tid == 0) {
            const uint64_t h43 = key_h43((uint64_t)(A.bucket_base + K.bucket) << A.rem_bits, K.rem, A.rem_bits, A.pshift);
            write_kept(A, o, kept_hi(h43, pre), kept_lo(best_f, mean, 0, 0));
            Job jbr;
            jbr.n = cb;
            jbr.out_idx = o;
            if (giant) {
                jbr.lens_off = reinterpret_cast<uint64_t>(H.gsamples + loff);
                H.gjobs[jb] = jbr;
            } else {
                jbr.lens_off = loff;
                A.jobs[jb] = jbr;
            }
        }
        __syncthreads();
    }
}

struct PlanArgs {
    const OvfEntry* in;
    OvfEntry* out;
    const unsigned long long* ctr;
    const unsigned long long* kept;
    const unsigned long long* nloc;
    unsigned long long* run;
    uint32_t* plan;
    const uint32_t* prev_plan;
    const unsigned long long* prev_ctr;
    uint32_t ovf_cap, split_min, heavy_min, big_cap;
    uint64_t kept_cap, tot_cap, split_cap;
};

constexpr uint32_t PLAN_BINS = 3 * 32;

__device__ __forceinline__ uint32_t plan_bin(uint32_t n, uint32_t split_min, uint32_t heavy_min) {
    const uint32_t tier = (n >= split_min ? 1u : 0u) + (n >= heavy_min ? 1u : 0u);
    return PLAN_BINS - 1u - (tier * 32u + (31u - (uint32_t)__clz(n | 1u)));
}

__global__ __launch_bounds__(1024) void k_ovf_plan(PlanArgs P) {
    __shared__ uint32_t s_cnt[PLAN_BINS];
    __shared__ unsigned long long s_part[1024];
    __shared__ unsigned long long s_tot, s_elems, s_split;
    __shared__ uint32_t s_nsplit, s_nheavy;
    const uint32_t tid = threadIdx.x, nt = blockDim.x;
    const uint64_t raw = P.ctr[1] & 0xFFFFFFFFull;
    const uint32_t n = (uint32_t)min<uint64_t>(raw, P.ovf_cap);
    for (uint32_t i = tid; i < PLAN_BINS; i += nt) s_cnt[i] = 0;
    if (tid == 0) {
        s_tot = s_elems = s_split = 0;
        s_nsplit = s_nheavy = 0;
    }
    __syncthreads();
    for (uint32_t i = tid; i < n; i += nt) atomicAdd(&s_cnt[plan_bin(P.in[i].n, P.split_min, P.heavy_min)], 1u);
    __syncthreads();
    if (tid == 0) {
        uint32_t r = 0;
        for (uint32_t b = 0; b < PLAN_BINS; ++b) {
            const uint32_t c = s_cnt[b];
            s_cnt[b] = r;
            r += c;
        }
    }
    __syncthreads();
    unsigned long long lt = 0, le = 0, ls = 0;
    uint32_t lns = 0, lnh = 0;
    for (uint32_t i = tid; i < n; i += nt) {
        OvfEntry e = P.in[i];
        const uint32_t pos = atomicAdd(&s_cnt[plan_bin(e.n, P.split_min, P.heavy_min)], 1u);
        uint64_t np = 1;
        while (np < e.n) np <<= 1;
        e.npad = (uint32_t)np;
        P.out[pos] = e;
        lt += np;
        le += e.n;
        if (e.n >= P.split_min) {
            ls += e.n;
            ++lns;
        }
// ... 57 lines not shown
        P.plan[PLAN_NLOC] = (uint32_t)min<uint64_t>(nl, 0xFFFFFFFFull);
        R[RUN_ACC_NOVF] += n;
        R[RUN_ACC_OVF_ELEMS] += s_elems;
        R[RUN_ACC_GROUPED] += nl;
        R[RUN_LAST_NOVF] = n;
    }
}

__global__ void k_poison_jobs(Job* __restrict__ jobs, uint64_t n, uint64_t samples, uint32_t idx,
                             skm_stored_kmer_data* __restrict__ out) {
    const uint64_t t = (uint64_t)blockIdx.x * blockDim.x + threadIdx.x;
    for (uint64_t j = t; j < n; j += (uint64_t)gridDim.x * blockDim.x) jobs[j] = Job{samples, 8u, idx};
    if (t == 0) out[idx] = skm_stored_kmer_data{0xC0DE, 0xC0DE, 0xC0DE, 0xC0DE, 0xC0DE};
}

__global__ void k_pass_account(const unsigned long long* __restrict__ ctr, unsigned long long* __restrict__ run,
                               uint64_t jobs_cap, uint64_t jobs2_cap, uint64_t big_cap, uint64_t lens_cap) {
    const unsigned long long j = ctr[3] + ctr[8 + 3];
    run[RUN_ACC_JOBS] += j;
    run[RUN_ACC_LENS] += ctr[8 + 4];
    run[RUN_ACC_OVF_KEPT] += ctr[8];
    run[RUN_ACC_BIG] += ctr[5];
    run[RUN_ACC_BIG_KEPT] += ctr[6];
    run[RUN_ACC_LIGHT_SUB] += ctr[21];
    run[RUN_ACC_LIGHT_ELEMS] += ctr[22];
    run[RUN_ACC_BPK_TASKS] += ctr[CTR_BPK_TASKS];
    run[RUN_ACC_BPK_BATCHES] += ctr[CTR_BPK_BATCHES];
    run[RUN_LAST_JOBS] = j;
    if (ctr[3] > jobs_cap || ctr[8 + 3] > jobs2_cap || ctr[5] > big_cap || ctr[8 + 4] > lens_cap)
        atomicOr(&run[RUN_FLAGS], RUN_F_CAP);
}

__global__ void k_kept_finalize(uint64_t* __restrict__ keys, const skm_stored_kmer_data* __restrict__ data,
                                const unsigned long long* __restrict__ n_p, uint32_t nf, uint32_t* __restrict__ dfunc) {
    extern __shared__ uint32_t s_h[];
    const uint64_t n = *n_p;
    const bool lds = nf <= 16384;
    if (lds)
        for (uint32_t f = threadIdx.x; f < nf; f += blockDim.x) s_h[f] = 0;
    __syncthreads();
    for (uint64_t i = (uint64_t)blockIdx.x * blockDim.x + threadIdx.x; i < n; i += (uint64_t)gridDim.x * blockDim.x) {
        keys[i] = decode_key(unmix43(keys[i]));
        uint32_t f = data[i].function_index;
        if (f < nf) {
            if (lds)
                atomicAdd(&s_h[f], 1u);
            else
                atomicAdd(&dfunc[f], 1u);
        }
    }
    __syncthreads();
    if (lds)
        for (uint32_t f = threadIdx.x; f < nf; f += blockDim.x)
            if (s_h[f]) atomicAdd(&dfunc[f], s_h[f]);
}

__global__ void k_func_hist_seqs(const SeqMeta* __restrict__ meta, uint32_t nseq, uint32_t nf, uint32_t* __restrict__ swf) {
    extern __shared__ uint32_t s_h[];
    const bool lds = nf <= 16384;
    if (lds)
        for (uint32_t f = threadIdx.x; f < nf; f += blockDim.x) s_h[f] = 0;
    __syncthreads();
    for (uint32_t s = blockIdx.x * blockDim.x + threadIdx.x; s < nseq; s += gridDim.x * blockDim.x) {
        uint32_t f = meta[s].func;
        if (f < nf) {
            if (lds)
                atomicAdd(&s_h[f], 1u);
            else
                atomicAdd(&swf[f], 1u);
        }
    }
    __syncthreads();
    if (lds)
        for (uint32_t f = threadIdx.x; f < nf; f += blockDim.x)
            if (s_h[f]) atomicAdd(&swf[f], s_h[f]);
}

__global__ void k_flags_from_bits(const uint32_t* __restrict__ bits, uint32_t nseq, uint8_t* __restrict__ flags) {
    for (uint32_t w = blockIdx.x * blockDim.x + threadIdx.x; w < (nseq + 31) / 32; w += gridDim.x * blockDim.x) {
        const uint32_t v = bits[w];
        const uint32_t n = min(32u, nseq - 32 * w);
        uint8_t* o = flags + 32 * (uint64_t)w;
        for (uint32_t t = 0; t < n; ++t) o[t] = (uint8_t)((v >> t) & 1u);
    }
}

__global__ void k_count_flags(const uint8_t* __restrict__ flags, uint32_t nseq, unsigned long long* __restrict__ out) {
    uint32_t local = 0;
    for (uint32_t s = blockIdx.x * blockDim.x + threadIdx.x; s < nseq; s += gridDim.x * blockDim.x) local += flags[s] ? 1u : 0u;
#pragma unroll
    for (int d = 32; d > 0; d >>= 1) local += __shfl_down(local, d, 64);
    if ((threadIdx.x & 63) == 0 && local) atomicAdd(out, (unsigned long long)local);
}

__global__ void k_send_counts(const uint64_t* __restrict__ bstart, uint32_t NB, uint32_t NB1, uint32_t W,
                              const unsigned long long* __restrict__ expect, unsigned long long* __restrict__ run,
                              uint32_t* __restrict__ out) {
    const uint32_t t = blockIdx.x * blockDim.x + threadIdx.x;
    if (t < NB) out[t] = (uint32_t)(bstart[t + 1] - bstart[t]);
    if (t < W && bstart[(uint64_t)(t + 1) * NB1] - bstart[(uint64_t)t * NB1] != expect[t])
        atomicOr(&run[RUN_FLAGS], (unsigned long long)RUN_F_CAP);
}

__global__ __launch_bounds__(1024) void k_recv_plan(const uint32_t* __restrict__ cnt, uint32_t W, uint32_t NB1,
                                                    const unsigned long long* __restrict__ expect,
                                                    unsigned long long* __restrict__ run,
                                                    uint64_t* __restrict__ seg_start, uint32_t* __restrict__ seg_len,
                                                    uint64_t* __restrict__ vstart) {
    __shared__ uint32_t s_wave[17];
    __shared__ unsigned long long s_tot[64];
    const uint32_t tid = threadIdx.x, nt = blockDim.x;
    const uint32_t N = W * NB1;
    {
        const uint32_t per = (N + nt - 1) / nt, a = min(N, tid * per), e = min(N, a + per);
        uint32_t loc = 0;
        for (uint32_t i = a; i < e; ++i) loc += cnt[i];
        uint32_t tot;
        uint64_t run_ = wg_exclusive_scan(loc, s_wave, tot);
        for (uint32_t i = a; i < e; ++i) {
            seg_start[i] = run_;
            seg_len[i] = cnt[i];
            run_ += cnt[i];
        }
    }
    if (tid < 64) s_tot[tid] = 0;
    __syncthreads();
    for (uint32_t i = tid; i < N; i += nt) atomicAdd(&s_tot[i / NB1], (unsigned long long)cnt[i]);
    __syncthreads();
    if (tid < W && s_tot[tid] != expect[tid]) atomicOr(&run[RUN_FLAGS], (unsigned long long)RUN_F_CAP);
    {
        const uint32_t per = (NB1 + nt - 1) / nt, a = min(NB1, tid * per), e = min(NB1, a + per);
        uint32_t loc = 0;
        for (uint32_t k = a; k < e; ++k)
            for (uint32_t p = 0; p < W; ++p) loc += cnt[(uint64_t)p * NB1 + k];
        uint32_t tot;
        uint64_t run_ = wg_exclusive_scan(loc, s_wave, tot);
        for (uint32_t k = a; k < e; ++k) {
            vstart[k] = run_;
            for (uint32_t p = 0; p < W; ++p) run_ += cnt[(uint64_t)p * NB1 + k];
        }
        if (tid == 0) vstart[NB1] = tot;
    }
}

__global__ __launch_bounds__(256) void k_slice_select(const uint64_t* __restrict__ keys,
                                                      const skm_stored_kmer_data* __restrict__ data, uint64_t n,
                                                      int bits, uint64_t slice, unsigned long long* __restrict__ cursor,
                                                      uint64_t* __restrict__ out_keys,
                                                      skm_stored_kmer_data* __restrict__ out_data) {
    const uint32_t lane = threadIdx.x & 63u;
    const uint64_t stride = (uint64_t)gridDim.x * blockDim.x;
    for (uint64_t b0 = (uint64_t)blockIdx.x * blockDim.x; b0 < n; b0 += stride) {
        const uint64_t j = b0 + threadIdx.x;
        const uint64_t k = j < n ? keys[j] : 0ull;
        const bool in = j < n && (bits == 0 || (slice_hash(k) >> (64 - bits)) == slice);
        const uint64_t m = __ballot(in);
        if (!m) continue;
        unsigned long long base = 0;
        if (lane == 0) base = atomicAdd(cursor, (unsigned long long)__popcll(m));
        base = __shfl(base, 0, 64);
        if (in && out_keys) {
            const uint64_t o = base + (uint64_t)__popcll(m & ((1ull << lane) - 1ull));
            out_keys[o] = k;
            out_data[o] = data[j];
        }
    }
// ... 27 lines not shown
    int chain_streams = 1;
    int poison_jobs = 0;
    int route_vacate = 0;
    int tail_async = 1;
    int big_grid = 2048;
    int big_grid_large = 512;
    int big_split = 0;
    int part_order = 1;
    int emit_group = 0;
    int route_first = -1;
    int route_first_min = 1 << 17;
    int route_heavy_min = 1 << 14;
    int chain_cus = 0;
    int side_cus = 0;
    int serial_overflow = 0;
    int stage_round = 1;
    int lane_long = 1 << 20;
    int lane_grid = 256;
    int lane_streams = 1;
    int lane_tail = 1 << 16;
    int sub_target = 0;
    int heavy_lsd = 0;
    int handoff_index_limit = 0;
    int handoff_max_chunk = 0;
};

}

using namespace skm;

struct ChainSet {
    DevBuf hist, offs, sorted, long_off;
};

struct skm_build {
    skm_build_opts opts{};
    int device = 0;
    hipStream_t stream = nullptr;
    struct EvSet {
        hipEvent_t ev[16] = {}, o[3] = {}, o3[3] = {};
    };
    std::deque<EvSet> evsets;
    hipEvent_t* ev = nullptr;
    hipEvent_t* ev_o = nullptr;
    hipEvent_t* ev_o3 = nullptr;
    float last_ms[17] = {};
    uint64_t ovf_elems = 0, ovf_kept = 0, ovf_light_sub = 0, ovf_light_elems = 0, bpk_tasks = 0, bpk_batches = 0;

    uint8_t* st_pin[2] = {};
    size_t st_fill[2] = {};
    hipEvent_t st_ev[2] = {};
    bool st_busy[2] = {};
    int st_cur = 0;
    uint64_t rp_total = 0;
    uint64_t rp_dev = 0;
    uint64_t res_cap = 0;
    std::vector<SeqMeta> h_meta;
    std::vector<uint32_t> h_seqid;
    std::unique_ptr<HostPool> pool;
    HandoffStats handoff;
    std::vector<uint32_t> h_keep;
    std::vector<uint64_t> h_cum;
    double add_s = 0, add_pack_s = 0, add_wait_s = 0, prep_upload_s = 0, prep_plan_s = 0, prep_rest_s = 0;
    uint64_t n_windows = 0;
    bool seqid_strict = true;
    bool prepared = false, ran = false;
    bool work_released = false;

    DevBuf d_res, d_meta, d_blk2seq, d_glen;
    uint64_t rp = 0;
    uint32_t nseq = 0;
    int world = 1, rank = 0;
    int owner_bits = 0, b1_bits = 12;
    uint32_t s_base = 0;
    uint32_t n_total = 0;
    std::vector<uint32_t> g_seqid;
    bool g_strict = true;
    DevBuf d_hist, d_offs, d_partial, d_rbbase, d_bstart32, d_bstart, d_owner_start;
    DevBuf d_recs_hi, d_recs_lo, d_tmp_hi, d_tmp_lo;
    DevBuf d_stg_hi, d_stg_lo;
    DevBuf d_part_order;
    DevBuf d_cur0, d_cur1, d_slices;
    DevBuf d_flagbits;
    DevBuf d_keys, d_data, d_ctr, d_flags, d_dfunc, d_swf, d_ovf, d_ovf_hi, d_ovf_lo, d_ovf_heads, d_ovf_job, d_ovf_fm;
    DevBuf d_jobs, d_lens, d_stamps, d_big_desc, d_big_out;
    uint64_t big_cap = 0, n_big = 0, big_kept = 0;
    bool stamps = false;
    uint32_t n_cus = 0;
    uint64_t jobs_cap = 0, lens_cap = 0, n_jobs = 0, n_lens = 0;
    uint32_t n_overflow = 0, n_overflow_last = 0;
    uint32_t nwg = 0;
    uint64_t span = 0;
    uint64_t n_kept = 0;
    uint64_t ovf_cap = 0;

    DevBuf d_rhi, d_rlo;
    DevBuf d_cnt_send, d_cnt_recv;
    DevBuf d_seg_start, d_seg_len, d_vstart;
    std::vector<uint64_t> xs_send, xs_recv;
    DevBuf d_xs;
    uint64_t n_local_max = 0;
    uint64_t n_local = 0;
    uint64_t cap_local = 0;

#if defined(SKM_WITH_RCCL)
    ncclComm_t comm = nullptr;
#endif
    std::vector<skm_build*> group;
    skm_transport tp{};

    hipStream_t stream2 = nullptr, stream3 = nullptr;
    hipStream_t stream_tail = nullptr;
    hipStream_t stream_tail2 = nullptr;
    hipEvent_t ev_tail_bp = nullptr, ev_tail_done[2] = {}, ev_tail2 = nullptr;
    bool tail_pending[2] = {};
    hipEvent_t ev_tail_jobs = nullptr;
    bool jobs_pending = false;
    uint64_t free_after_prepare = 0;
    hipEvent_t ev_part = nullptr, ev_split = nullptr, ev_light = nullptr;
    DevBuf d_hv_keys, d_hv_rec, d_hv_len, d_hv_s0, d_hv_s1;
    DevBuf d_sub_tab, d_jobs2, d_jobs3;

    unsigned long long* h_pin = nullptr;
    OvfEntry* h_ovf = nullptr;
    size_t h_ovf_cap = 0;
    unsigned long long* pinned_ctr() {
        if (!h_pin) SKM_HIP(hipHostMalloc(reinterpret_cast<void**>(&h_pin), 128 * 8, hipHostMallocDefault));
        return h_pin;
    }
    OvfEntry* pinned_ovf(size_t n) {
        if (n > h_ovf_cap) {
            if (h_ovf) SKM_HIP(hipHostFree(h_ovf));
            h_ovf = nullptr;
            h_ovf_cap = std::max<size_t>(n, 1024);
            SKM_HIP(hipHostMalloc(reinterpret_cast<void**>(&h_ovf), sizeof(OvfEntry) * h_ovf_cap, hipHostMallocDefault));
        }
        return h_ovf;
    }

    uint64_t jobs2_cap = 0;
    ChainSet cs_main, cs_ovf, cs_ovf3;
    uint32_t n_ovf_heavy = 0;

    int pass_bits = 0;
    uint64_t pass_max = 0;
    uint64_t valid_total = 0;
    DevBuf d_ids;
    DevBuf d_bloom;
    std::vector<uint64_t> cnt64;
    bool route = false;
    bool route_first = false;
    uint64_t routed = 0;
    DevBuf d_posg, d_histg, d_npos;
    uint32_t emit_g = 1;
    DevBuf d_selrows, d_seloff;
    uint64_t sel_span = 0;
    uint32_t sel_wg = SEL_WG;
    hipStream_t stx = nullptr;
    hipEvent_t ev_staged = nullptr, ev_emit = nullptr;
    int64_t emit_q = -1;
    uint32_t pf_nwg = 1;
    uint64_t pf_span = 0;
    uint64_t kept_cap = 0;
    hipEvent_t ev_start = nullptr;
    struct Acc {
        uint64_t novf, jobs, lens, ovf_elems, ovf_kept, big, big_kept, grouped;
// ... 642 lines not shown
        b->d_bloom.ensure(nbl / 8);
        hipLaunchKernelGGL(k_bloom_pack, dim3((uint32_t)(nbl / 32 + 255) / 256), dim3(256), 0, b->stream,
                           bl8[k].as<uint8_t>(), b->d_bloom.as<uint32_t>());
        SKM_HIP(hipGetLastError());
    }
    std::vector<uint64_t> ok(bs.size(), 1), heavy(bs.size(), 0);
    std::vector<uint64_t> routed_m(bs.size()), routed_n(bs.size());
    auto count_routed = [&]() {
        for (size_t k = 0; k < bs.size(); ++k) {
            skm_build* b = bs[k];
            const uint32_t P = 1u << pb;
            DevBuf d_cnt;
            d_cnt.ensure(8 * 64);
            SKM_HIP(hipMemsetAsync(d_cnt.p, 0, 8 * 64, b->stream));
            if (b->rp)
                hipLaunchKernelGGL(k_pass_ids, dim3(1024), dim3(256), 4u * 64 + (uint32_t)(nbl / 8), b->stream,
                                   b->d_res.as<uint8_t>(), b->rp, pb, 0, nullptr, d_cnt.as<unsigned long long>(),
                                   b->d_bloom.as<uint32_t>(), 64u, nullptr, 0, route_arg(b));
            SKM_HIP(hipGetLastError());
            uint64_t cnt[64];
            SKM_HIP(hipMemcpyAsync(cnt, d_cnt.p, sizeof(cnt), hipMemcpyDeviceToHost, b->stream));
            SKM_HIP(hipStreamSynchronize(b->stream));
            const int R = b->tune.route_vacate > 0 ? std::min(b->tune.route_vacate, (int)P - 1) : (int)(P >> 1);
            uint64_t natural_late = 0, late = 0, m = 0;
            if (first) {
                natural_late = cnt[0];
            } else {
                for (int p = (int)P - R; p < (int)P; ++p) {
                    for (int i = 0; i < (64 >> pb); ++i) natural_late += b->cnt64[p * (64 >> pb) + i];
                    late += cnt[p];
                }
            }
            for (uint32_t p = 0; p < P; ++p) m = std::max<uint64_t>(m, cnt[p]);
            size_t fr = 0, tot = 0;
            SKM_HIP(hipMemGetInfo(&fr, &tot));
            const uint64_t budget = b->tune.mem_budget_mb > 0 ? (uint64_t)b->tune.mem_budget_mb << 20 : (uint64_t)fr;
            const bool forced = b->tune.passes > 0;
            const bool giant = b->tune.giant_class > 0 || (b->tune.giant_class < 0 && (pb == 0 || b->world > 1));
            ok[k] = m < (1ull << 32) - (1ull << 28) &&
                    (forced || m <= b->pass_max || work_fits(pass_work(m, pb, b->rp, giant), budget));
            routed_m[k] = m;
            routed_n[k] = natural_late - late;
            heavy[k] = first ? cnt[0] : 0;
        }
    };
    auto turn_off = [&]() {
        for (auto* b : bs) b->route_first = false;
    };
    count_routed();
    if (first) {
        const std::vector<uint64_t> all = W > 1 ? allgather_u64(bs, heavy) : heavy;
        uint64_t any = 0;
        for (auto v : all) any |= v;
        if (!any) return turn_off();
        if (pb < 2 && b0->tune.passes <= 0 && pb < 6) {
            ++pb;
            for (auto* b : bs) {
                size_passes(b, pb);
                b->route_first = true;
            }
            count_routed();
        }
        if (pb == 0) return turn_off();
    }
    {
        const std::vector<uint64_t> all = W > 1 ? allgather_u64(bs, ok) : ok;
        for (auto v : all)
            if (!v) return turn_off();
    }
    for (size_t k = 0; k < bs.size(); ++k) {
        bs[k]->pass_max = routed_m[k];
        bs[k]->routed = routed_n[k];
        bs[k]->route = true;
    }
}

void check_not_released(const Ranks& bs) {
    for (auto* b : bs)
        SKM_CHECK(!b->work_released, SKM_E_STATE,
                  "the build's work buffers were released (skm_build_kept_db release_work): the handle can only be "
                  "read out and destroyed");
}

void prepare(const Ranks& bs) {
    check_not_released(bs);
    bool need = false;
    for (auto* b : bs) need |= !b->prepared;
    if (!need) return;
    using clk = std::chrono::steady_clock;
    const auto t0 = clk::now();
    for (auto* b : bs) prepare_local(b);
    for (auto* b : bs) SKM_HIP(hipStreamSynchronize(b->stream));
    const auto t1 = clk::now();
    for (auto* b : bs) size_passes(b);
    {
        std::vector<uint64_t> mine;
        for (auto* b : bs) mine.push_back((uint64_t)b->pass_bits);
        const std::vector<uint64_t> all = bs[0]->world > 1 ? allgather_u64(bs, mine) : mine;
        uint64_t pb = 0;
        for (auto v : all) pb = std::max(pb, v);
        for (auto* b : bs)
            if ((uint64_t)b->pass_bits != pb) size_passes(b, (int)pb);
        route_plan(bs);
        for (auto* b : bs) SKM_HIP(hipStreamSynchronize(b->stream));
    }
    const auto t2 = clk::now();
    for (auto* b : bs) {
        b->prep_upload_s = std::chrono::duration<double>(t1 - t0).count();
        b->prep_plan_s = std::chrono::duration<double>(t2 - t1).count();
    }
    for (auto* b : bs) size_local(b);
    skm_build* b0 = bs[0];
    if (b0->world == 1) {
        b0->s_base = 0;
        b0->n_total = b0->nseq;
        b0->d_glen.ensure(4 * (b0->nseq + 1));
        std::vector<uint32_t> len(b0->nseq);
        for (uint32_t s = 0; s < b0->nseq; ++s) len[s] = b0->h_meta[s].len;
        if (b0->nseq) SKM_HIP(hipMemcpyAsync(b0->d_glen.p, len.data(), 4 * b0->nseq, hipMemcpyHostToDevice, b0->stream));
        ensure_local(b0, b0->pass_max);
    } else {
        std::vector<uint64_t> mine;
        for (auto* b : bs) mine.push_back(b->nseq);
        const std::vector<uint64_t> ns = allgather_u64(bs, mine);
        uint64_t tot = 0;
        for (auto v : ns) tot += v;
        SKM_CHECK(tot < (1ull << ELEM_S_BITS), SKM_E_ARG, "too many sequences in one build");
        std::vector<uint64_t> bytes(ns.size());
        for (size_t r = 0; r < ns.size(); ++r) bytes[r] = 4 * ns[r];
        std::vector<DevBuf> lens_src(bs.size()), ids_src(bs.size()), ids_all(bs.size());
        std::vector<const void*> src_l, src_i;
        std::vector<void*> dst_l, dst_i;
        for (size_t k = 0; k < bs.size(); ++k) {
            skm_build* b = bs[k];
            uint64_t base = 0;
            for (int r = 0; r < b->rank; ++r) base += ns[r];
            b->s_base = (uint32_t)base;
            b->n_total = (uint32_t)tot;
            std::vector<uint32_t> len(b->nseq);
            for (uint32_t s = 0; s < b->nseq; ++s) len[s] = b->h_meta[s].len;
            lens_src[k].ensure(4 * (b->nseq + 1));
            ids_src[k].ensure(4 * (b->nseq + 1));
            ids_all[k].ensure(4 * (tot + 1));
            b->d_glen.ensure(4 * (tot + 1));
            SKM_HIP(hipMemcpy(lens_src[k].p, len.data(), 4 * b->nseq, hipMemcpyHostToDevice));
            SKM_HIP(hipMemcpy(ids_src[k].p, b->h_seqid.data(), 4 * b->nseq, hipMemcpyHostToDevice));
            src_l.push_back(lens_src[k].p);
            src_i.push_back(ids_src[k].p);
            dst_l.push_back(b->d_glen.p);
            dst_i.push_back(ids_all[k].p);
        }
        if (is_group(bs)) {
            allgatherv(bs, src_l, dst_l, bytes);
            allgatherv(bs, src_i, dst_i, bytes);
        } else {
            allgatherv(bs, {src_l[0]}, {dst_l[0]}, bytes);
            allgatherv(bs, {src_i[0]}, {dst_i[0]}, bytes);
        }
        sync_all(bs);
        pass_peer_counts(bs);
        for (size_t k = 0; k < bs.size(); ++k) {
            skm_build* b = bs[k];
            b->g_seqid.resize(tot);
            if (tot) SKM_HIP(hipMemcpy(b->g_seqid.data(), ids_all[k].p, 4 * tot, hipMemcpyDeviceToHost));
            b->g_strict = true;
            for (uint64_t s = 1; s < tot; ++s)
                if (b->g_seqid[s] <= b->g_seqid[s - 1]) b->g_strict = false;
            ensure_local(b, std::max(b->pass_max, b->n_local_max));
        }
    }
    for (auto* b : bs) {
        if (!b->tot_cap) {
            b->tot_cap = b->cap_local / 8 * 5 + (1u << 16);
            b->split_cap = b->tot_cap / 2;
            b->long_cap = b->pass_bits ? b->valid_total / 8 + (1u << 16) : 0;
        }
        alloc_caps(b);
        size_arena(b);
        b->d_flags.ensure(std::max<uint64_t>(b->n_total, 1));
        b->d_flagbits.ensure(4 * ((b->n_total + 31) / 32 + 1));
        {
            size_t fr = 0, tot = 0;
            SKM_HIP(hipMemGetInfo(&fr, &tot));
            b->free_after_prepare = fr;
        }
        SKM_HIP(hipStreamSynchronize(b->stream));
        b->prepared = true;
        b->ran = false;
    }
    for (auto* b : bs) b->prep_rest_s = std::chrono::duration<double>(clk::now() - t2).count();
}

void emit_group(skm_build* b, uint32_t g, hipStream_t st) {
    const uint32_t G = b->emit_g;
    const uint32_t NB = 1u << (b->owner_bits + b->b1_bits);
    const int rem_bits = KEY_BITS - b->pass_bits - b->owner_bits - b->b1_bits;
    const uint64_t cap = std::max<uint64_t>(b->pass_max, 1);
#define SKM_EMIT(GG)                                                                                                    \
    SKM_LAUNCH_AS(b, "k_pass_emit", k_pass_emit<GG>, dim3(b->sel_wg), dim3(EMIT_THREADS), 0, st, b->d_res.as<uint8_t>(), \
                  b->d_ids.as<uint8_t>(), b->rp, g * G, b->sel_span, b->d_seloff.as<uint64_t>(), b->sel_wg, \
                  b->d_posg.as<uint64_t>(), cap)
    if (G == 16)
        SKM_EMIT(16);
    else if (G == 8)
        SKM_EMIT(8);
    else if (G == 4)
        SKM_EMIT(4);
    else if (G == 2)
        SKM_EMIT(2);
    else
        SKM_EMIT(1);
#undef SKM_EMIT
    SKM_HIP(hipMemsetAsync(b->d_histg.p, 0, sizeof(uint32_t) * NB * G, st));
    SKM_LAUNCH(b, k_pass_hist, dim3(256, G), dim3(PH_THREADS), 4u * NB, st, b->d_posg.as<uint64_t>(), cap,
               b->d_npos.as<unsigned long long>() + (uint64_t)g * G, NB, rem_bits, b->d_histg.as<uint32_t>());
    SKM_LAUNCH(b, k_pass_starts, dim3(G), dim3(1024), 0, st, b->d_histg.as<uint32_t>(), NB,
               b->owner_bits + b->b1_bits - SC_L0_BITS, (g & 1u) * G, b->d_bstart.as<uint64_t>(),
               b->d_cur0.as<unsigned long long>(), b->d_cur1.as<unsigned long long>(), b->d_slices.as<uint32_t>(),
               b->world == 1 && b->tune.part_order ? b->d_part_order.as<uint32_t>() : nullptr);
    SKM_HIP(hipGetLastError());
    if (st != b->stream) SKM_HIP(hipEventRecord(b->ev_emit, st));
}

inline uint32_t pass_par(const skm_build* b, uint32_t pass) { return tail_async_on(b) ? pass & 1u : 0u; }
inline unsigned long long* pass_ctr(skm_build* b, uint32_t pass) {
    return b->d_ctr.as<unsigned long long>() + 32 + 32 * pass_par(b, pass);
}
inline uint64_t* pass_hi(skm_build* b, uint32_t pass) { return (pass_par(b, pass) ? b->d_stg_hi : b->d_tmp_hi).as<uint64_t>(); }
inline uint64_t* pass_lo(skm_build* b, uint32_t pass) { return (pass_par(b, pass) ? b->d_stg_lo : b->d_tmp_lo).as<uint64_t>(); }

void join_tail_par(skm_build* b, uint32_t par) {
    if (!b->tail_pending[par]) return;
    SKM_HIP(hipStreamWaitEvent(b->stream, b->ev_tail_done[par], 0));
    b->tail_pending[par] = false;
}
void join_tail(skm_build* b) {
    join_tail_par(b, 0);
    join_tail_par(b, 1);
}

void phase_extract(skm_build* b, uint32_t pass) {
    hipStream_t st = b->stream;
    const int nbits = b->owner_bits + b->b1_bits;
    const uint32_t NB = 1u << nbits;
    const uint32_t nowners = 1u << b->owner_bits;
    SKM_HIP(hipEventRecord(b->ev[0], st));
    const size_t lds_cnt = sizeof(uint32_t) * NB;
    ExtractArgs X;
    X.res = b->d_res.as<uint8_t>();
    X.rp = b->rp;
    X.span = b->span;
    X.owner_bits = b->owner_bits;
    X.b1_bits = b->b1_bits;
    X.pass_bits = b->pass_bits;
    X.pass_id = pass;
    X.pos_cap = b->pass_max;
    X.ids = nullptr;
    X.hist = b->d_hist.as<uint32_t>();
    X.offs = b->d_offs.as<uint32_t>();
    X.owner_start = b->d_owner_start.as<uint64_t>();
    X.blk2seq = b->d_blk2seq.as<uint32_t>();
    X.meta = b->d_meta.as<SeqMeta>();
    X.s_base = b->s_base;
// ... 181 lines not shown
        SKM_HIP(hipMemcpy(b->d_xs.as<uint64_t>() + (uint64_t)P * W, b->xs_recv.data(), 8ull * P * W, hipMemcpyHostToDevice));
    }
}

uint64_t giant_cap(const skm_build* b) { return std::min<uint64_t>(std::max<uint64_t>(b->split_cap, 1), 1ull << 28); }

int giant_class(const skm_build* b) {
    return b->tune.giant_class >= 0 ? b->tune.giant_class : (b->pass_bits == 0 || b->world > 1 ? 14 : 0);
}

constexpr uint32_t JOB_NWG = 256;
constexpr uint32_t LONG_GRID = 2048;

void launch_chains(skm_build* b, hipStream_t st, const Job* jobs, const unsigned long long* nj_d, uint64_t cap,
                   ChainSet& cs, const uint32_t* lens, const uint32_t* recs32, const uint32_t* tmp32,
                   const uint32_t* big32, skm_stored_kmer_data* out, uint32_t long_class,
                   hipStream_t st_short = nullptr, hipEvent_t ev_sorted = nullptr, uint32_t max_wgs = 0) {
    const Tune& tn = b->tune;
    SKM_LAUNCH(b, k_job_count, dim3(JOB_NWG), dim3(JOB_WG), 0, st, jobs, nj_d, cap, cs.hist.as<uint32_t>());
    SKM_LAUNCH(b, k_job_scan, dim3(1), dim3(64), 0, st, cs.hist.as<uint32_t>(), JOB_NWG, cs.offs.as<uint64_t>(),
                       long_class);
    SKM_LAUNCH(b, k_job_scatter, dim3(JOB_NWG), dim3(JOB_WG), 0, st, jobs, nj_d, cap, cs.offs.as<uint64_t>(),
                       cs.sorted.as<Job>());
    if (ev_sorted) SKM_HIP(hipEventRecord(ev_sorted, st));
    const uint64_t* nlong_d = cs.offs.as<uint64_t>() + (uint64_t)JOB_NWG * JOB_CLASSES;
    const auto* nlong_u = reinterpret_cast<const unsigned long long*>(nlong_d);
    if (b->pass_bits == 0) {
        const uint32_t lds = (uint32_t)tn.chain_lds_kb * 1024u;
        static bool attr = false;
        if (lds > 65536 && !attr) {
            SKM_HIP(hipFuncSetAttribute(reinterpret_cast<const void*>(k_chain_long),
                                        hipFuncAttributeMaxDynamicSharedMemorySize, (int)lds));
            attr = true;
        }
        SKM_LAUNCH(b, k_chain_long, dim3(LONG_GRID), dim3(128), lds, st, cs.sorted.as<Job>(), nullptr, nlong_u,
                   lens, recs32, tmp32, big32, out, tn.chain_prio);
    } else {
        SKM_LAUNCH(b, k_long_plan, dim3(1), dim3(1024), 0, st, cs.sorted.as<Job>(), nlong_d,
                           cs.long_off.as<uint64_t>(), b->d_run.as<unsigned long long>(), b->long_cap,
                           b->long_jobs_cap);
        SKM_LAUNCH(b, k_long_stash, dim3(LONG_GRID), dim3(256), 0, st, cs.sorted.as<Job>(), nlong_d,
                           cs.long_off.as<uint64_t>(), lens, recs32, tmp32, big32, b->d_long_arena.as<uint32_t>(),
                           b->d_long_jobs.as<Job>());
    }
    hipStream_t ss = st;
    if (st_short && ev_sorted) {
        SKM_HIP(hipStreamWaitEvent(st_short, ev_sorted, 0));
        ss = st_short;
    }
    SKM_LAUNCH(b, k_chains, dim3(max_wgs ? max_wgs : (uint32_t)std::max(1, tn.chain_grid)), dim3(256), 0, ss,
               cs.sorted.as<Job>(), nlong_u, nj_d, cap, lens, recs32, tmp32, big32, out, 0u);
    SKM_HIP(hipGetLastError());
}

void phase_group(skm_build* b, uint32_t pass) {
    hipStream_t st = b->stream, st2 = b->stream2, st3 = b->stream3;
    const bool multi = b->world > 1;
    const uint32_t NB1 = 1u << b->b1_bits;
    SKM_HIP(hipEventRecord(b->ev[4], st));
    const uint32_t par = pass_par(b, pass);
    unsigned long long* ctr_d = pass_ctr(b, pass);
    SKM_HIP(hipMemsetAsync(ctr_d, 0, 256, st));
    unsigned long long* run_d = b->d_run.as<unsigned long long>();
    uint32_t* plan_d = b->d_plan.as<uint32_t>() + par * PLAN_SLOTS;
    OvfEntry* ovf2_d = b->d_ovf2.as<OvfEntry>() + (uint64_t)par * std::max<uint64_t>(b->ovf_cap, 1);
    BucketArgs A;
    A.recs_hi = (multi ? b->d_rhi : b->d_recs_hi).as<uint64_t>();
    A.recs_lo = (multi ? b->d_rlo : b->d_recs_lo).as<uint64_t>();
    A.tmp_hi = pass_hi(b, pass);
    A.tmp_lo = pass_lo(b, pass);
    const uint32_t pc = pass_copy(b, pass);
    A.bstart = multi ? b->d_vstart.as<uint64_t>() : b->d_bstart.as<uint64_t>() + (uint64_t)pc * (NB1 + 1);
    A.seg_start = multi ? b->d_seg_start.as<uint64_t>() : nullptr;
    A.seg_len = multi ? b->d_seg_len.as<uint32_t>() : nullptr;
    A.nsrc = multi ? (uint32_t)b->world : 1u;
    A.sub_tab = b->d_sub_tab.as<uint32_t>();
    A.kept_ctr = b->d_ctr.as<unsigned long long>();
    A.nbuckets = NB1;
    A.bucket_base = (pass << (b->owner_bits + b->b1_bits)) | ((uint32_t)b->rank << b->b1_bits);
    A.rem_bits = KEY_BITS - b->pass_bits - b->owner_bits - b->b1_bits;
    A.pshift = KEY_BITS - b->pass_bits;
    A.glen = b->d_glen.as<uint32_t>();
    A.flags = b->d_flagbits.as<uint32_t>();
    A.ctr = ctr_d;
    A.out_keys = b->d_keys.as<uint64_t>();
    A.out_data = b->d_data.as<skm_stored_kmer_data>();
    A.jobs = b->d_jobs.as<Job>();
    A.lens = b->d_lens.as<uint32_t>();
    A.ovf = b->d_ovf.as<OvfEntry>();
    A.ovf_cap = (uint32_t)b->ovf_cap;
    A.prio = b->tune.bucket_prio;
    A.stamps = nullptr;
    A.big_desc = b->d_big_desc.as<uint64_t>();
    A.big_cap = (uint32_t)std::min<uint64_t>(b->big_cap, 0xFFFFFFFFull);
    A.big_ctr = ctr_d + 5;
    A.skip = nullptr;
    A.sub_target = (uint32_t)std::max(0, b->tune.sub_target);
    if (b->stamps) {
        SKM_HIP(hipMemsetAsync(b->d_stamps.p, 0, 32 * 8, st));
        A.stamps = b->d_stamps.as<unsigned long long>();
    }
    A.order = nullptr;
    if (b->tune.part_order) {
        A.order = b->d_part_order.as<uint32_t>() + (multi ? 0 : (uint64_t)pc * (NB1 + 1));
        if (multi || !b->pass_bits) SKM_LAUNCH(b, k_part_order, dim3(1), dim3(1024), 0, st, A.bstart, NB1, b->d_part_order.as<uint32_t>());
    }
    SKM_LAUNCH(b, k_partition, dim3(NB1), dim3(BP_THREADS), 0, st, A);
    SKM_HIP(hipGetLastError());
    SKM_HIP(hipEventRecord(b->ev[10], st));
    if (b->pass_bits && pass % b->emit_g == b->emit_g - 1) SKM_HIP(hipEventRecord(b->ev_staged, st));
    const unsigned long long* nloc_d;
    if (multi) {
        nloc_d = reinterpret_cast<const unsigned long long*>(b->d_vstart.as<uint64_t>() + NB1);
    } else {
        nloc_d = reinterpret_cast<const unsigned long long*>(A.bstart + NB1);
    }
    const uint32_t split_min = (uint32_t)std::max(b->tune.split_min, CAP + 1);
    const uint32_t key_min = (uint32_t)std::max(b->tune.heavy_min, 2);
    PlanArgs P;
    P.in = b->d_ovf.as<OvfEntry>();
    P.out = ovf2_d;
    P.ctr = ctr_d;
    P.kept = b->d_ctr.as<unsigned long long>();
    P.nloc = nloc_d;
    P.run = run_d;
    P.plan = plan_d;
    const bool prev = tail_async_on(b) && pass > 0;
    P.prev_plan = prev ? b->d_plan.as<uint32_t>() + (par ^ 1u) * PLAN_SLOTS : nullptr;
    P.prev_ctr = prev ? pass_ctr(b, pass - 1) : nullptr;
    P.big_cap = A.big_cap;
    P.ovf_cap = (uint32_t)b->ovf_cap;
    P.split_min = split_min;
    P.heavy_min = (uint32_t)b->tune.ovf_heavy;
    P.kept_cap = b->kept_cap;
    P.tot_cap = b->tot_cap;
    P.split_cap = b->split_cap;
    SKM_LAUNCH(b, k_ovf_plan, dim3(1), dim3(1024), 0, st, P);
    SKM_HIP(hipGetLastError());
    A.skip = plan_d + PLAN_SKIP;
    BucketArgs A2 = A, A3 = A;
    OvfScratch S;
    S.hi = b->d_ovf_hi.as<uint64_t>();
    S.lo = b->d_ovf_lo.as<uint64_t>();
    S.heads = b->d_ovf_heads.as<uint32_t>();
    S.jobinfo = b->d_ovf_job.as<uint64_t>();
    S.fmean = b->d_ovf_fm.as<uint32_t>();
    A2.ovf = ovf2_d;
    A2.ctr = ctr_d + 8;
    A2.jobs = b->d_jobs2.as<Job>();
    A2.lens = b->d_lens.as<uint32_t>();
    A3.ovf = A2.ovf;
    A3.ctr = A2.ctr;
    A3.jobs = A2.jobs;
    A3.lens = A2.lens;
    const uint32_t inline_min = (uint32_t)b->tune.ovf_inline_min;
    const int prio = b->tune.inline_prio;
    HeavyArgs H;
    H.keys = b->d_hv_keys.as<HeavyKey>();
    H.nkeys = ctr_d + 18;
    H.cursor = ctr_d + 19;
    H.queue = ctr_d + 20;
    H.rec = b->d_hv_rec.as<uint64_t>();
    H.len = b->d_hv_len.as<uint32_t>();
    H.s0 = b->d_hv_s0.as<uint32_t>();
    H.s1 = b->d_hv_s1.as<uint32_t>();
    H.fast = b->opts.n_functions <= HV_FT && !b->tune.heavy_lsd ? 1u : 0u;
    H.n_total = std::max<uint32_t>(b->n_total, 1);
    const int gs = (int)(pass % skm_build::GSLOTS);
    const uint32_t NP = 1u << b->pass_bits;
    const bool late = b->tune.giant_passes <= 0 || pass + (uint32_t)b->tune.giant_passes >= NP;
    const int gcls = giant_class(b);
    H.giant_min = gcls > 0 && late && pass < b->gsamples.size() ? 1u << gcls : 0u;
    H.gsamples = nullptr;
    H.gjobs = nullptr;
    H.gcount = nullptr;
    H.gcap = 0;
    H.gstat = nullptr;
    if (H.giant_min) {
        H.gsamples = b->gsamples[pass].as<uint32_t>();
        H.gjobs = b->gjobs[pass].as<Job>();
        H.gcount = b->gcount[pass].as<unsigned long long>();
        H.gcap = giant_cap(b);
        H.gstat = b->d_gstat.as<unsigned long long>();
    }
    const bool light = b->tune.ovf_light != 0;
    auto launch_overflow = [&]() {
    SKM_HIP(hipEventRecord(b->ev_part, st));
    SKM_HIP(hipStreamWaitEvent(st2, b->ev_part, 0));
    SKM_HIP(hipStreamWaitEvent(st3, b->ev_part, 0));
    if (prev) SKM_HIP(hipStreamWaitEvent(st2, b->evsets[pass - 1].o3[1], 0));
    if (b->jobs_pending) {
        SKM_HIP(hipStreamWaitEvent(st2, b->ev_tail_jobs, 0));
        SKM_HIP(hipStreamWaitEvent(st3, b->ev_tail_jobs, 0));
    }
    SKM_HIP(hipEventRecord(b->ev_o[0], st2));
    SKM_HIP(hipEventRecord(b->ev_o3[0], st3));
    if (H.giant_min) SKM_HIP(hipMemsetAsync(b->gcount[pass].p, 0, 16, st2));
    SKM_LAUNCH(b, k_ovf_split, dim3((uint32_t)std::max(1, b->tune.split_grid)), dim3(BP_THREADS), 0, st2, A2, H, key_min, plan_d);
    SKM_HIP(hipEventRecord(b->ev_split, st2));
    SKM_HIP(hipStreamWaitEvent(st3, b->ev_split, 0));
    if (light) {
        SKM_LAUNCH(b, k_ovf_light, dim3(LIGHT_GRID), dim3(BPK_THREADS), 0, st3, A3, plan_d,
                   ctr_d + 21);
        SKM_HIP(hipEventRecord(b->ev_light, st3));
    }
    SKM_LAUNCH(b, k_heavy, dim3((uint32_t)std::max(1, b->tune.heavy_grid)), dim3(HEAVY_WG), 0, st2, A2, H);
    SKM_HIP(hipGetLastError());
    if (H.giant_min) {
        SKM_HIP(hipEventRecord(b->gev_ready[gs], st2));
        SKM_HIP(hipStreamWaitEvent(b->gst[gs], b->gev_ready[gs], 0));
        SKM_LAUNCH(b, k_giant_order, dim3(1), dim3(1024), 0, b->gst[gs], H.gjobs, H.gcount);
        if (!b->giant_timed) SKM_HIP(hipEventRecord(b->ev_giant[0], b->gst[gs]));
        SKM_LAUNCH(b, k_chain_dyn, dim3(1024), dim3(128), 0, b->gst[gs], H.gjobs, H.gcount, A.out_data,
                           b->tune.chain_prio);
        SKM_HIP(hipGetLastError());
        if (!b->giant_timed) SKM_HIP(hipEventRecord(b->ev_giant[1], b->gst[gs]));
        b->giant_timed = true;
        SKM_HIP(hipEventRecord(b->gev_done[gs], b->gst[gs]));
        b->gused[gs] = true;
    }
    if (light) SKM_HIP(hipStreamWaitEvent(st2, b->ev_light, 0));
    SKM_LAUNCH(b, k_overflow, dim3((uint32_t)std::max(1, b->tune.ovf_grid)), dim3(BP_THREADS), 0, st2, A2, S, plan_d, -1, (int)PLAN_NHEAVY,
                       (int)PLAN_Q_HEAVY, inline_min, prio);
    SKM_HIP(hipEventRecord(b->ev_o[1], st2));
    SKM_LAUNCH(b, k_overflow, dim3((uint32_t)std::max(1, b->tune.ovf_grid)), dim3(BP_THREADS), 0, st3, A3, S, plan_d, (int)PLAN_NHEAVY,
                       (int)PLAN_NOVF, (int)PLAN_Q_REST, inline_min, prio);
    SKM_HIP(hipGetLastError());
    };
    if (!b->tune.serial_overflow) launch_overflow();
    BigArgs BA;
    BA.desc = A.big_desc;
    BA.ndesc = ctr_d + 5;
    BA.cap = A.big_cap;
    BA.recs_hi = A.recs_hi;
    BA.tmp_hi = A.tmp_hi;
    BA.recs_lo = A.recs_lo;
    BA.tmp_lo = A.tmp_lo;
    BA.flags = A.flags;
    BA.out = b->d_big_out.as<BigOut>();
    SKM_HIP(hipEventRecord(b->ev[15], st));
    if (b->jobs_pending) {
        SKM_HIP(hipStreamWaitEvent(st, b->ev_tail_jobs, 0));
        b->jobs_pending = false;
    }
    SKM_HIP(hipEventRecord(b->ev[11], st));
    SKM_LAUNCH(b, k_bucket_process, dim3(std::min<uint32_t>(NB1 * BPK_PARTS, 2u * b->n_cus)), dim3(BPK_THREADS), 0, st, A);
    SKM_HIP(hipGetLastError());
    SKM_HIP(hipEventRecord(b->ev[5], st));
    if (b->tune.serial_overflow) launch_overflow();
    if (b->pass_bits && pass + 1 < NP && (pass + 1) % b->emit_g == 0 && b->tune.prefetch) {
        SKM_HIP(hipStreamWaitEvent(b->stx, b->ev_staged, 0));
        emit_group(b, (pass + 1) / b->emit_g, b->stx);
        b->emit_q = (pass + 1) / b->emit_g;
    }
    const bool tail_async = tail_async_on(b);
    hipStream_t tt = tail_async ? b->stream_tail : st;
    if (tail_async) {
        SKM_HIP(hipEventRecord(b->ev_tail_bp, st));
        SKM_HIP(hipStreamWaitEvent(tt, b->ev_tail_bp, 0));
    }
    SKM_HIP(hipEventRecord(b->ev_o3[0], st3));
    SKM_HIP(hipStreamWaitEvent(st2, b->ev_o3[0], 0));
    launch_chains(b, st2, A2.jobs, ctr_d + 8 + 3, b->jobs2_cap, b->cs_ovf, A2.lens, reinterpret_cast<const uint32_t*>(A.recs_hi),
                  reinterpret_cast<const uint32_t*>(A.tmp_hi), nullptr, A.out_data, (uint32_t)b->tune.ovf_long_class, st3, b->ev_o3[2], (uint32_t)b->tune.ovf_chain_wgs);
    SKM_HIP(hipEventRecord(b->ev_o[2], st2));
    SKM_HIP(hipEventRecord(b->ev_o3[1], st3));
    if (light) SKM_HIP(hipStreamWaitEvent(tt, b->ev_light, 0));
    if (tail_async && b->tune.big_split) {
        SKM_HIP(hipStreamWaitEvent(b->stream_tail2, b->ev_tail_bp, 0));
        if (light) SKM_HIP(hipStreamWaitEvent(b->stream_tail2, b->ev_light, 0));
        SKM_LAUNCH(b, k_big_groups<true>, dim3((uint32_t)std::max(1, b->tune.big_grid_large)), dim3(BIG_WG), 0,
                   b->stream_tail2, BA);
        SKM_HIP(hipEventRecord(b->ev_tail2, b->stream_tail2));
        SKM_LAUNCH(b, k_big_groups<false>, dim3((uint32_t)std::max(1, b->tune.big_grid)), dim3(BIG_WG), 0, tt, BA);
        SKM_HIP(hipStreamWaitEvent(tt, b->ev_tail2, 0));
    } else {
        SKM_LAUNCH(b, k_big_groups<false>, dim3((uint32_t)std::max(1, b->tune.big_grid)), dim3(BIG_WG), 0, tt, BA);
        SKM_LAUNCH(b, k_big_groups<true>, dim3((uint32_t)std::max(1, b->tune.big_grid_large)), dim3(BIG_WG), 0, tt, BA);
    }
    SKM_LAUNCH(b, k_big_append, dim3(256), dim3(BIG_WG), 0, tt, BA.out, BA, A);
    SKM_HIP(hipGetLastError());
    SKM_HIP(hipEventRecord(b->ev[12], tt));
    launch_chains(b, tt, A.jobs, ctr_d + 3, b->jobs_cap, b->cs_main, A.lens, reinterpret_cast<const uint32_t*>(A.recs_hi),
                  reinterpret_cast<const uint32_t*>(A.tmp_hi), nullptr, A.out_data, (uint32_t)b->tune.main_long_class,
                  nullptr, tail_async ? b->ev_tail_jobs : nullptr);
    b->jobs_pending = tail_async;
    SKM_HIP(hipStreamWaitEvent(tt, b->ev_o[2], 0));
    SKM_HIP(hipStreamWaitEvent(tt, b->ev_o3[1], 0));
    SKM_HIP(hipEventRecord(b->ev[6], tt));
    SKM_LAUNCH(b, k_pass_account, dim3(1), dim3(1), 0, tt, ctr_d, run_d, b->jobs_cap, b->jobs2_cap, b->big_cap,
                       b->lens_cap);
    SKM_HIP(hipGetLastError());
    SKM_HIP(hipEventRecord(b->ev[7], tt));
    if (tail_async) {
        SKM_HIP(hipEventRecord(b->ev_tail_done[par], tt));
        b->tail_pending[par] = true;
    }
}

void alloc_caps(skm_build* b) {
    const uint64_t T = std::max<uint64_t>(b->tot_cap, 1), Sp = std::max<uint64_t>(b->split_cap, 1);
    b->d_ovf_hi.ensure(8 * T);
    b->d_ovf_lo.ensure(8 * T);
    b->d_ovf_heads.ensure(4 * T);
    b->d_ovf_job.ensure(8 * T);
    b->d_ovf_fm.ensure(4 * T);
    b->jobs2_cap = T / 3 + 16;
    b->d_jobs2.ensure(sizeof(Job) * b->jobs2_cap);
    const uint32_t key_min = (uint32_t)std::max(b->tune.heavy_min, 2);
    b->d_hv_keys.ensure(sizeof(HeavyKey) * (Sp / key_min + 16));
    b->d_hv_rec.ensure(8 * Sp);
    b->d_hv_len.ensure(4 * Sp);
    b->d_hv_s0.ensure(4 * Sp);
    b->d_hv_s1.ensure(4 * Sp);
    b->d_ovf2.ensure(2 * sizeof(OvfEntry) * std::max<uint64_t>(b->ovf_cap, 1));
    b->d_plan.ensure(2 * 4 * PLAN_SLOTS);
    b->d_run.ensure(8 * RUN_SLOTS);
    b->d_sub_tab.ensure(4ull * (1u << b->b1_bits) * SUB_TAB);
    b->d_stamps.ensure(32 * 8);
    const int cls = std::max(1, std::min(b->tune.main_long_class, b->tune.ovf_long_class));
    struct {
        ChainSet* cs;
        uint64_t cap, elems;
    } sets[2] = {{&b->cs_main, b->jobs_cap, b->cap_local}, {&b->cs_ovf, b->jobs2_cap, T}};
    for (auto& c : sets) {
        c.cs->hist.ensure(4ull * JOB_NWG * JOB_CLASSES);
        c.cs->offs.ensure(8ull * JOB_NWG * JOB_CLASSES + 16);
        c.cs->sorted.ensure(sizeof(Job) * c.cap);
        c.cs->long_off.ensure(8ull * (std::min(c.cap, (c.elems >> cls) + 16) + 8));
    }
    if (b->pass_bits) {
        b->long_jobs_cap = std::max<uint64_t>(b->long_jobs_cap, b->world * (b->valid_total >> cls) + 4096);
        b->d_long_jobs.ensure(sizeof(Job) * b->long_jobs_cap);
        b->d_long_arena.ensure(4 * std::max<uint64_t>(b->long_cap, 1));
    }
    const uint32_t NP = 1u << b->pass_bits;
    if (giant_class(b) > 0) {
        while (b->gsamples.size() < NP) {
            b->gsamples.emplace_back();
            b->gjobs.emplace_back();
            b->gcount.emplace_back();
        }
        for (uint32_t p = 0; p < NP; ++p) {
            b->gsamples[p].ensure(4 * giant_cap(b));
            b->gjobs[p].ensure(sizeof(Job) * (giant_cap(b) / (1u << giant_class(b)) + 16));
            b->gcount[p].ensure(16);
        }
    }
}

void begin_run(skm_build* b) {
    hipStream_t st = b->stream;
    alloc_caps(b);
    b->emit_q = -1;
    b->giant_timed = false;
    b->tail_pending[0] = b->tail_pending[1] = b->jobs_pending = false;
    SKM_HIP(hipEventRecord(b->ev_start, st));
    SKM_HIP(hipMemsetAsync(b->d_ctr.p, 0, 3 * 256, st));
    SKM_HIP(hipMemsetAsync(b->d_run.p, 0, 8 * RUN_SLOTS, st));
    SKM_HIP(hipMemsetAsync(b->d_flags.p, 0, b->n_total ? b->n_total : 1, st));
    SKM_HIP(hipMemsetAsync(b->d_flagbits.p, 0, 4 * ((b->n_total + 31) / 32 + 1), st));
    b->d_gstat.ensure(16);
    SKM_HIP(hipMemsetAsync(b->d_gstat.p, 0, 16, st));
    if (b->tune.poison_jobs && b->pass_bits && b->long_jobs_cap)
        hipLaunchKernelGGL(k_poison_jobs, dim3(256), dim3(256), 0, st, b->d_long_jobs.as<Job>(), b->long_jobs_cap,
                           reinterpret_cast<uint64_t>(b->d_long_arena.p), (uint32_t)b->kept_cap,
                           b->d_data.as<skm_stored_kmer_data>());
    if (b->pass_bits) {
        const uint32_t P = 1u << b->pass_bits;
        SKM_LAUNCH(b, k_pass_ids, dim3(b->sel_wg), dim3(256), 4u * P + (b->route ? (1u << BLOOM_BITS) / 8 : 0u), st,
                   b->d_res.as<uint8_t>(), b->rp, b->pass_bits, 0, b->d_ids.as<uint8_t>(), nullptr,
                   b->route ? b->d_bloom.as<uint32_t>() : nullptr, P, b->d_selrows.as<uint32_t>(), b->sel_span,
                   route_arg(b));
        SKM_LAUNCH(b, k_sel_scan, dim3(P), dim3(1024), 0, st, b->d_selrows.as<uint32_t>(), b->sel_wg, P,
                   b->d_seloff.as<uint64_t>(), b->d_npos.as<unsigned long long>(), b->pass_max,
                   b->d_run.as<unsigned long long>());
    }
    SKM_HIP(hipGetLastError());
    b->acc = skm_build::Acc{};
    b->kt_used = 0;
    b->kt_recs.clear();
    std::memset(b->pass_ms, 0, sizeof(b->pass_ms));
    for (bool& g : b->gused) g = false;
    for (bool& g : b->chain_used) g = false;
    b->n_kept = 0;
}

void use_evset(skm_build* b, uint32_t pass) {
    while (b->evsets.size() <= pass) {
        b->evsets.emplace_back();
        skm_build::EvSet& e = b->evsets.back();
        for (auto& x : e.ev) SKM_HIP(hipEventCreate(&x));
        for (auto& x : e.o) SKM_HIP(hipEventCreate(&x));
        for (auto& x : e.o3) SKM_HIP(hipEventCreate(&x));
    }
    b->ev = b->evsets[pass].ev;
    b->ev_o = b->evsets[pass].o;
    b->ev_o3 = b->evsets[pass].o3;
}

void pass_times(skm_build* b, uint32_t npass) {
    const int idx[11] = {0, 1, 2, 3, 5, 8, 9, 10, 11, 12, 13};
    const int from[11] = {0, 1, 2, 4, 12, 3, 4, 11, 5, 13, 15}, to[11] = {1, 2, 3, 12, 6, 4, 10, 5, 12, 14, 11};
    for (uint32_t p = 0; p < npass && p < b->evsets.size(); ++p) {
        const skm_build::EvSet& e = b->evsets[p];
        for (int i = 0; i < 11; ++i) {
            float t = 0.f;
            SKM_HIP(hipEventElapsedTime(&t, e.ev[from[i]], e.ev[to[i]]));
            b->pass_ms[idx[i]] += t;
        }
        float t2 = 0.f, t3 = 0.f;
        SKM_HIP(hipEventElapsedTime(&t2, e.o[0], e.o[2]));
        SKM_HIP(hipEventElapsedTime(&t3, e.o[0], e.o3[1]));
        b->pass_ms[4] += std::max(t2, t3);
    }
}

hipStream_t chain_stream(skm_build* b, int slot) {
    const int k = slot % std::max(1, std::min(b->tune.chain_streams, 1 + skm_build::GSLOTS));
    return k == 0 ? b->chain_st : b->gst[k - 1];
}

void flush_long_chains(skm_build* b, int slot) {
    join_tail(b);
    unsigned long long* run_d = b->d_run.as<unsigned long long>();
    unsigned long long* rng = run_d + RUN_SNAP + 2 * slot;
    SKM_LAUNCH(b, k_long_snap, dim3(1), dim3(1), 0, b->stream, run_d, rng, b->long_jobs_cap);
    SKM_HIP(hipEventRecord(b->chain_ev[0], b->stream));
    hipStream_t cs = chain_stream(b, slot);
    SKM_HIP(hipStreamWaitEvent(cs, b->chain_ev[0], 0));
    b->chain_used[slot % std::max(1, std::min(b->tune.chain_streams, 1 + skm_build::GSLOTS))] = true;
    const bool few = (1 << b->pass_bits) < 8;
    const int lmax = slot < 16 && !few ? b->tune.lane_long : std::min(b->tune.lane_long, b->tune.lane_tail);
    const uint32_t lane_max = lmax > 0 ? (uint32_t)lmax : 0u;
    SKM_LAUNCH(b, k_chain_long, dim3(LONG_GRID), dim3(128), 0, cs, b->d_long_jobs.as<Job>(), rng, rng + 1,
               nullptr, nullptr, nullptr, nullptr, b->d_data.as<skm_stored_kmer_data>(), b->tune.chain_prio,
               lane_max);
    if (lane_max) {
        const int ls = slot % std::max(1, std::min(b->tune.lane_streams, (int)skm_build::LANE_ST));
        hipStream_t lst = b->lane_st[ls];
        SKM_HIP(hipStreamWaitEvent(lst, b->chain_ev[0], 0));
        SKM_LAUNCH(b, k_chains_stash, dim3((uint32_t)std::max(1, b->tune.lane_grid)), dim3(256), 0, lst,
                   b->d_long_jobs.as<Job>(), rng, rng + 1, b->long_jobs_cap, b->d_data.as<skm_stored_kmer_data>(),
                   lane_max);
        b->lane_used[ls] = true;
    }
    SKM_HIP(hipGetLastError());
}

void phase_stats(skm_build* b) {
    hipStream_t st = b->stream;
    const uint32_t F = b->opts.n_functions;
    SKM_HIP(hipEventRecord(b->ev_tail[0], st));
    join_tail(b);
    if (b->n_total)
        SKM_LAUNCH(b, k_flags_from_bits, dim3(1024), dim3(256), 0, st, b->d_flagbits.as<uint32_t>(),
                   (uint32_t)b->n_total, b->d_flags.as<uint8_t>());
    SKM_HIP(hipMemsetAsync(b->d_dfunc.p, 0, sizeof(uint32_t) * (F ? F : 1), st));
    SKM_HIP(hipMemsetAsync(b->d_swf.p, 0, sizeof(uint32_t) * (F ? F : 1), st));
    const size_t lds_f = F <= 16384 ? sizeof(uint32_t) * F : 0;
    if (b->pass_bits) flush_long_chains(b, 16);
    SKM_LAUNCH(b, k_kept_finalize, dim3(2048), dim3(256), lds_f, st, b->d_keys.as<uint64_t>(),
                       b->d_data.as<skm_stored_kmer_data>(), b->d_ctr.as<unsigned long long>(), F,
                       b->d_dfunc.as<uint32_t>());
    if (b->nseq)
        SKM_LAUNCH(b, k_func_hist_seqs, dim3(256), dim3(256), lds_f, st, b->d_meta.as<SeqMeta>(), b->nseq, F,
                           b->d_swf.as<uint32_t>());
    if (b->pass_bits) {
        for (int k = 0; k < skm_build::LANE_ST; ++k) {
            if (!b->lane_used[k]) continue;
            SKM_HIP(hipEventRecord(b->lane_ev[k], b->lane_st[k]));
            SKM_HIP(hipStreamWaitEvent(st, b->lane_ev[k], 0));
            b->lane_used[k] = false;
        }
        for (int k = 0; k <= skm_build::GSLOTS; ++k) {
            if (!b->chain_used[k]) continue;
            const hipStream_t cs = chain_stream(b, k);
            hipEvent_t e = k == 0 ? b->chain_ev[2] : b->gev_done[k - 1];
            SKM_HIP(hipEventRecord(e, cs));
            SKM_HIP(hipStreamWaitEvent(st, e, 0));
        }
    }
    for (int g = 0; g < skm_build::GSLOTS; ++g)
        if (b->gused[g]) SKM_HIP(hipStreamWaitEvent(st, b->gev_done[g], 0));
    SKM_HIP(hipEventRecord(b->ev_tail[1], st));
    SKM_HIP(hipEventRecord(b->ev[7], st));
    SKM_HIP(hipGetLastError());
}

void phase_final(skm_build* b) {
    hipStream_t st = b->stream;
    SKM_LAUNCH(b, k_count_flags, dim3(256), dim3(256), 0, st, b->d_flags.as<uint8_t>(), b->n_total,
                       b->d_ctr.as<unsigned long long>() + 2);
    SKM_HIP(hipGetLastError());
    unsigned long long* pin = b->pinned_ctr();
    SKM_HIP(hipMemcpyAsync(pin + 48, b->d_gstat.p, 16, hipMemcpyDeviceToHost, st));
    SKM_HIP(hipMemcpyAsync(pin + 56, b->d_ctr.p, 8, hipMemcpyDeviceToHost, st));
    SKM_HIP(hipMemcpyAsync(pin + 64, b->d_run.p, 8 * RUN_SLOTS, hipMemcpyDeviceToHost, st));
    const bool canary = b->tune.poison_jobs && b->pass_bits && b->long_jobs_cap;
    if (canary)
        SKM_HIP(hipMemcpyAsync(pin + 42, b->d_data.as<skm_stored_kmer_data>() + b->kept_cap,
                               sizeof(skm_stored_kmer_data), hipMemcpyDeviceToHost, st));
    SKM_HIP(hipEventRecord(b->ev[8], st));
    SKM_HIP(hipEventSynchronize(b->ev[8]));
    const unsigned long long* R = pin + 64;
    b->giant_jobs = pin[48];
    b->giant_max = pin[49];
    b->n_kept = pin[56];
    b->run_flags = R[RUN_FLAGS];
    if (canary) {
        const auto* c = reinterpret_cast<const skm_stored_kmer_data*>(pin + 42);
        if (c->median != 0xC0DE || c->var != 0xC0DE) b->run_flags |= RUN_F_CAP;
    }
    for (int i = 0; i < 4; ++i) b->demand[i] = R[RUN_DEM_TOT + i];
    b->demand[2] = std::max<uint64_t>(b->demand[2], R[RUN_LONG_WANT]);
    b->demand[3] = std::max<uint64_t>(b->demand[3], R[RUN_LONG_WANTJ]);
    pass_times(b, 1u << b->pass_bits);
    for (int i = 0; i < 12; ++i) b->last_ms[i] = b->pass_ms[i];
    SKM_HIP(hipEventElapsedTime(&b->last_ms[6], b->ev[7], b->ev[8]));
    SKM_HIP(hipEventElapsedTime(&b->last_ms[7], b->ev_start, b->ev[8]));
    SKM_HIP(hipEventElapsedTime(&b->last_ms[12], b->ev_tail[0], b->ev_tail[1]));
    b->last_ms[15] = b->pass_ms[12];
    b->last_ms[16] = b->pass_ms[13];
    b->last_ms[13] = b->last_ms[14] = -1.0f;
    if (b->giant_timed) {
        SKM_HIP(hipEventElapsedTime(&b->last_ms[13], b->ev_start, b->ev_giant[0]));
        SKM_HIP(hipEventElapsedTime(&b->last_ms[14], b->ev_start, b->ev_giant[1]));
    }
    b->long_samples = R[RUN_LONG_CUR];
    kt_collect(b);
    b->n_overflow = (uint32_t)R[RUN_ACC_NOVF];
    b->n_overflow_last = (uint32_t)R[RUN_LAST_NOVF];
    b->n_jobs = R[RUN_ACC_JOBS];
    b->n_jobs_last = R[RUN_LAST_JOBS];
    b->n_lens = R[RUN_ACC_LENS];
    b->ovf_elems = R[RUN_ACC_OVF_ELEMS];
    b->ovf_kept = R[RUN_ACC_OVF_KEPT];
    b->n_big = R[RUN_ACC_BIG];
    b->big_kept = R[RUN_ACC_BIG_KEPT];
    b->ovf_light_sub = R[RUN_ACC_LIGHT_SUB];
    b->ovf_light_elems = R[RUN_ACC_LIGHT_ELEMS];
    b->bpk_tasks = R[RUN_ACC_BPK_TASKS];
    b->bpk_batches = R[RUN_ACC_BPK_BATCHES];
    b->n_local = R[RUN_ACC_GROUPED];
    b->ran = true;
}

void grow_caps(skm_build* b) {
    auto grow = [](uint64_t& cap, uint64_t dem) {
        if (dem > cap) cap = dem + dem / 8 + 1024;
    };
    grow(b->tot_cap, b->demand[0]);
    grow(b->split_cap, b->demand[1]);
    grow(b->long_cap, b->demand[2]);
    grow(b->long_jobs_cap, b->demand[3]);
    SKM_HIP(hipDeviceSynchronize());
    alloc_caps(b);
}

void run_once(const Ranks& bs) {
    for (auto* b : bs) begin_run(b);
    const uint32_t P = 1u << bs[0]->pass_bits;
    for (uint32_t pass = 0; pass < P; ++pass) {
        for (auto* b : bs) {
            use_evset(b, pass);
            phase_extract(b, pass);
        }
        if (bs[0]->world > 1) exchange(bs, pass);
        for (auto* b : bs) {
            phase_group(b, pass);
            const uint32_t nb = std::min<uint32_t>(P >= 2 ? std::min<uint32_t>(P, (uint32_t)std::max(1, b->tune.chain_batches)) : 1u, 16u);
            const uint32_t per = std::max<uint32_t>(1u, P / nb);
            if (nb > 1 && (pass + 1) % per == 0 && pass + 1 < P) {
                flush_long_chains(b, (int)((pass + 1) / per - 1));
            }
        }
    }
    for (auto* b : bs) phase_stats(b);
    if (bs[0]->world > 1) {
        std::vector<void*> df, sw, fl;
        for (auto* b : bs) {
            df.push_back(b->d_dfunc.p);
            sw.push_back(b->d_swf.p);
            fl.push_back(b->d_flags.p);
        }
        const uint32_t F = bs[0]->opts.n_functions;
        allreduce(bs, df, F, Red::SumU32);
        allreduce(bs, sw, F, Red::SumU32);
        allreduce(bs, fl, bs[0]->n_total, Red::MaxU8);
    }
    for (auto* b : bs) phase_final(b);
}

void run_ranks(const Ranks& bs) {
    check_not_released(bs);
    prepare(bs);
    for (int attempt = 0;; ++attempt) {
        run_once(bs);
        std::vector<uint64_t> mine;
        for (auto* b : bs) mine.push_back((b->run_flags & RUN_F_RERUN) ? 1u : 0u);
        const std::vector<uint64_t> all = bs[0]->world > 1 ? allgather_u64(bs, mine) : mine;
        bool redo = false;
        for (auto v : all) redo |= v != 0;
        if (!redo) break;
        SKM_CHECK(attempt < 3, SKM_E_STATE, "build work buffers did not converge");
        for (auto* b : bs) {
            grow_caps(b);
            ++b->n_redo;
        }
    }
    for (auto* b : bs) {
        SKM_CHECK(!(b->run_flags & RUN_F_ARENA), SKM_E_OOM,
                  "kept k-mer arena exhausted (raise the device memory budget or the key-range passes)");
        SKM_CHECK(!(b->run_flags & RUN_F_CAP), SKM_E_STATE, "build work list capacity exceeded");
    }
}

Ranks ranks_of(skm_build* b) {
    if (!b->group.empty()) return b->group;
    return Ranks{b};
}

}

__attribute__((constructor)) static void skm_hw_queues() {
// ... 458 lines not shown
    for (int i = 0; i < cap; ++i) out[i] = (uint32_t)i < n ? e[i].n : 0u;
    return (int)n;
}

int skm_debug_chain_bench(uint32_t n, uint32_t njobs, int mode, float* ms) {
    SKM_API_BEGIN
    SKM_CHECK(ms && n && njobs, SKM_E_ARG, "bad argument");
    std::vector<uint32_t> lens((size_t)n * njobs);
    uint32_t x = 12345;
    for (auto& v : lens) {
        x = x * 1664525u + 1013904223u;
        v = 240 + (x >> 16) % 121;
    }
    std::vector<Job> jobs(njobs);
    for (uint32_t i = 0; i < njobs; ++i) jobs[i] = Job{(uint64_t)i * n, n, i};
    DevBuf dl, dj, dout;
    dl.ensure(4 * lens.size());
    dj.ensure(sizeof(Job) * njobs);
    dout.ensure(std::max(sizeof(skm_stored_kmer_data), sizeof(double)) * njobs);
    SKM_HIP(hipMemcpy(dl.p, lens.data(), 4 * lens.size(), hipMemcpyHostToDevice));
    SKM_HIP(hipMemcpy(dj.p, jobs.data(), sizeof(Job) * njobs, hipMemcpyHostToDevice));
    DevBuf dn;
    dn.ensure(8);
    const unsigned long long nj64 = njobs;
    SKM_HIP(hipMemcpy(dn.p, &nj64, 8, hipMemcpyHostToDevice));
    hipEvent_t e0, e1;
    SKM_HIP(hipEventCreate(&e0));
    SKM_HIP(hipEventCreate(&e1));
    const uint64_t threads = ceil_div(njobs, 64) * 128;
    for (int it = 0; it < 2; ++it) {
        SKM_HIP(hipEventRecord(e0, 0));
        if (mode == 3 || mode == 4 || mode == 5)
            hipLaunchKernelGGL(k_chain_long_half, dim3(njobs), dim3(64), 0, 0, dj.as<Job>(), dl.as<uint32_t>(),
                               mode - 3, reinterpret_cast<double*>(dout.p));
        else if (mode == 2 || (mode == 0 && n >= (1u << LONG_CLASS)))
            hipLaunchKernelGGL(k_chain_long, dim3(njobs), dim3(128), 0, 0, dj.as<Job>(), nullptr, dn.as<unsigned long long>(),
                               dl.as<uint32_t>(), dl.as<uint32_t>(), dl.as<uint32_t>(), dl.as<uint32_t>(),
                               dout.as<skm_stored_kmer_data>(), 0);
        else
            hipLaunchKernelGGL(k_chains, dim3((uint32_t)ceil_div(threads, 256)), dim3(256), 0, 0, dj.as<Job>(), nullptr,
                               dn.as<unsigned long long>(), (uint64_t)njobs, dl.as<uint32_t>(), dl.as<uint32_t>(),
                               dl.as<uint32_t>(), dl.as<uint32_t>(), dout.as<skm_stored_kmer_data>());
        SKM_HIP(hipEventRecord(e1, 0));
        SKM_HIP(hipEventSynchronize(e1));
        SKM_HIP(hipEventElapsedTime(ms, e0, e1));
    }
    (void)hipEventDestroy(e0);
    (void)hipEventDestroy(e1);
    SKM_API_END
}

int skm_debug_chain_eval(const uint32_t* samples, uint32_t n, int mode, double* median, double* var) {
    SKM_API_BEGIN
    SKM_CHECK(samples && n && median && var && (mode == 1 || mode == 2), SKM_E_ARG, "bad argument");
    DevBuf dx, dout;
    dx.ensure(4ull * n);
    dout.ensure(16);
    SKM_HIP(hipMemcpy(dx.p, samples, 4ull * n, hipMemcpyHostToDevice));
    hipLaunchKernelGGL(k_chain_eval, dim3(1), dim3(128), 0, 0, dx.as<uint32_t>(), n, mode, dout.as<double>());
    SKM_HIP(hipGetLastError());
    double r[2];
    SKM_HIP(hipMemcpy(r, dout.p, 16, hipMemcpyDeviceToHost));
    *median = r[0];
    *var = r[1];
    SKM_API_END
}

int skm_debug_div_check(uint64_t nm, uint32_t per, uint64_t* mismatches) {
    SKM_API_BEGIN
    SKM_CHECK(mismatches && nm, SKM_E_ARG, "bad argument");
    DevBuf d;
    d.ensure(8);
    SKM_HIP(hipMemset(d.p, 0, 8));
    hipLaunchKernelGGL(k_div_check, dim3((uint32_t)ceil_div(nm, 256)), dim3(256), 0, 0, nm, per,
                       d.as<unsigned long long>());
    SKM_HIP(hipGetLastError());
    SKM_HIP(hipMemcpy(mismatches, d.p, 8, hipMemcpyDeviceToHost));
    SKM_API_END
}

int skm_build_counters(skm_build* b, uint64_t* out, int cap) {
    if (!b || !out) return SKM_E_ARG;
    auto us = [](double sec) { return (uint64_t)(sec * 1e6); };
    const uint64_t v[50] = {b->n_windows, b->n_kept, b->n_overflow, b->n_jobs, b->n_lens, b->nseq, b->n_local,
                            b->ovf_elems, b->ovf_kept, b->n_big, b->big_kept, 1ull << b->pass_bits, b->valid_total,
                            b->giant_jobs, b->giant_max, b->n_redo, b->tot_cap, b->split_cap, b->long_cap,
                            b->long_jobs_cap, b->demand[0], b->demand[1], b->demand[2], b->demand[3],
                            b->long_samples, b->routed, us(b->add_s), us(b->prep_upload_s), us(b->prep_plan_s),
                            us(b->prep_rest_s), b->pass_bits ? (1ull << b->pass_bits) / b->emit_g : 0ull, us(b->add_pack_s),
                            us(b->add_wait_s), us(b->handoff.total_s), us(b->handoff.wait_s),
                            us(b->handoff.copy_s), b->handoff.chunks, (uint64_t)(1e3 * b->handoff.select_ms),
                            (uint64_t)(1e3 * b->handoff.sort_ms), (uint64_t)(1e3 * b->handoff.gather_ms),
                            (uint64_t)(1e3 * b->handoff.d2h_ms), b->handoff.max_chunk,
                            (uint64_t)b->handoff.wide_index, b->kept_cap, b->free_after_prepare,
                            0ull , b->ovf_light_sub, b->ovf_light_elems, b->bpk_tasks,
                            b->bpk_batches};
    int n = std::min(cap, 50);
    for (int i = 0; i < n; ++i) out[i] = v[i];
    return n;
}

int skm_build_set_kernel_timing(skm_build* b, int enable, const char* only) {
    SKM_API_BEGIN
    SKM_CHECK(b, SKM_E_ARG, "null build");
    b->kt_mode = enable ? 1 : 0;
    b->kt_only = only ? std::string(only) : std::string();
    SKM_API_END
}

int skm_build_kernel_timings(skm_build* b, char* names, size_t names_cap, float* ms, uint64_t* launches, int cap) {
    if (!b) return SKM_E_ARG;
    const int n = (int)b->kt_names.size();
    std::string all;
    for (int k = 0; k < n; ++k) {
        if (k < cap) {
            if (ms) ms[k] = (float)b->kt_ms[k];
            if (launches) launches[k] = b->kt_n[k];
        }
        all += b->kt_names[k];
        all += '\n';
    }
    if (names && names_cap) {
        const size_t c = std::min(names_cap - 1, all.size());
        std::memcpy(names, all.data(), c);
        names[c] = 0;
    }
    return n;
}

int skm_build_last_timings(skm_build* b, float* ms, int cap) {
    if (!b || !ms) return SKM_E_ARG;
    int n = std::min(cap, 17);
    for (int i = 0; i < n; ++i) ms[i] = b->last_ms[i];
    return n;
}

int skm_build_finish(skm_build* b, skm_kept* out) {
    SKM_API_BEGIN
    SKM_CHECK(b && out, SKM_E_ARG, "null argument");
    check_transport(b);
    SKM_HIP(hipSetDevice(b->device));
    const Ranks bs = ranks_of(b);
    bool need = false;
    for (auto* x : bs) need |= !x->prepared || !x->ran;
    if (need) run_ranks(bs);
    std::memset(out, 0, sizeof(*out));
    const uint32_t F = b->opts.n_functions;
    std::vector<uint64_t> mine;
    for (auto* x : bs) mine.push_back(x->n_kept);
    const std::vector<uint64_t> nk = b->world > 1 ? allgather_u64(bs, mine) : mine;
    uint64_t total = 0;
    for (auto v : nk) total += v;
    const bool gather = b->world > 1 && b->rank == 0;
    const uint64_t n = gather ? total : b->n_kept;
    DevBuf gk, gd;
    const uint64_t* src_k = b->d_keys.as<uint64_t>();
    const skm_stored_kmer_data* src_d = b->d_data.as<skm_stored_kmer_data>();
    if (b->world > 1 && bs.size() > 1) {
        if (gather) {
            gk.ensure(8 * (total + 1));
            gd.ensure(sizeof(skm_stored_kmer_data) * (total + 1));
            uint64_t o = 0;
            for (auto* x : bs) {
                if (x->n_kept) {
                    SKM_HIP(hipMemcpy(gk.as<uint64_t>() + o, x->d_keys.p, 8 * x->n_kept, hipMemcpyDeviceToDevice));
                    SKM_HIP(hipMemcpy(gd.as<skm_stored_kmer_data>() + o, x->d_data.p,
                                      sizeof(skm_stored_kmer_data) * x->n_kept, hipMemcpyDeviceToDevice));
                }
                o += x->n_kept;
            }
            src_k = gk.as<uint64_t>();
            src_d = gd.as<skm_stored_kmer_data>();
        }
    } else if (b->world > 1) {
        const int W = b->world;
        A2A xk, xd;
        std::vector<uint64_t> so(W, 0), sck(W, 0), scd(W, 0), rok(W, 0), rod(W, 0), rck(W, 0), rcd(W, 0);
        sck[0] = 8 * b->n_kept;
        scd[0] = sizeof(skm_stored_kmer_data) * b->n_kept;
        if (gather) {
// ... 64 lines not shown
    out->n_records = b->n_local;
    SKM_API_END
}

int skm_build_finish_slice(skm_build* b, int slice_bits, uint32_t slice, skm_kept* out) {
    SKM_API_BEGIN
    SKM_CHECK(b && out, SKM_E_ARG, "null argument");
    SKM_CHECK(slice_bits >= 0 && slice_bits <= 16 && slice < (1u << slice_bits), SKM_E_ARG, "bad slice");
    check_transport(b);
    SKM_HIP(hipSetDevice(b->device));
    const Ranks bs = ranks_of(b);
    bool need = false;
    for (auto* x : bs) need |= !x->prepared || !x->ran;
    if (need) run_ranks(bs);
    std::memset(out, 0, sizeof(*out));
    hipStream_t st = b->stream;
    const uint32_t F = b->opts.n_functions;
    DevBuf cur, dk, dd;
    cur.ensure(8);
    SKM_HIP(hipMemsetAsync(cur.p, 0, 8, st));
    const uint64_t nk = b->n_kept;
    if (nk)
        hipLaunchKernelGGL(k_slice_select, dim3(2048), dim3(256), 0, st, b->d_keys.as<uint64_t>(),
                           b->d_data.as<skm_stored_kmer_data>(), nk, slice_bits, (uint64_t)slice,
                           cur.as<unsigned long long>(), nullptr, nullptr);
    SKM_HIP(hipGetLastError());
    uint64_t n = 0;
    SKM_HIP(hipMemcpyAsync(&n, cur.p, 8, hipMemcpyDeviceToHost, st));
    SKM_HIP(hipStreamSynchronize(st));
    if (n) {
        dk.ensure(8 * n);
        dd.ensure(sizeof(skm_stored_kmer_data) * n + 16);
        SKM_HIP(hipMemsetAsync(cur.p, 0, 8, st));
        hipLaunchKernelGGL(k_slice_select, dim3(2048), dim3(256), 0, st, b->d_keys.as<uint64_t>(),
                           b->d_data.as<skm_stored_kmer_data>(), nk, slice_bits, (uint64_t)slice,
                           cur.as<unsigned long long>(), dk.as<uint64_t>(), dd.as<skm_stored_kmer_data>());
        SKM_HIP(hipGetLastError());
    }
    out->distinct_functions = (uint32_t*)std::malloc(sizeof(uint32_t) * std::max<uint32_t>(F, 1));
    out->seqs_with_func = (uint32_t*)std::malloc(sizeof(uint32_t) * std::max<uint32_t>(F, 1));
    SKM_CHECK(out->distinct_functions && out->seqs_with_func, SKM_E_OOM, "host allocation failed");
    if (F) {
        SKM_HIP(hipMemcpyAsync(out->distinct_functions, b->d_dfunc.p, sizeof(uint32_t) * F, hipMemcpyDeviceToHost, st));
        SKM_HIP(hipMemcpyAsync(out->seqs_with_func, b->d_swf.p, sizeof(uint32_t) * F, hipMemcpyDeviceToHost, st));
    }
    unsigned long long ctr[3];
    SKM_HIP(hipMemcpyAsync(ctr, b->d_ctr.p, sizeof(ctr), hipMemcpyDeviceToHost, st));
    SKM_HIP(hipStreamSynchronize(st));
    if (!b->pool) b->pool.reset(new HostPool(HostPool::default_threads()));
    kept_handoff(dk.as<uint64_t>(), dd.as<skm_stored_kmer_data>(), n, st, b->pool.get(), &out->keys, &out->data,
                 &b->handoff, (uint64_t)b->tune.handoff_index_limit, (uint64_t)b->tune.handoff_max_chunk);
    out->n = n;
    out->n_functions = F;
    uint64_t total = b->n_kept;
    if (b->world > 1) {
        std::vector<uint64_t> mine;
        for (auto* x : bs) mine.push_back(x->n_kept);
        total = 0;
        for (auto v : allgather_u64(bs, mine)) total += v;
    }
    out->distinct_signatures = total;
    out->n_seqs_with_signature = ctr[2];
    out->n_windows = b->n_windows;
    out->n_records = b->n_local;
    SKM_API_END
}

int skm_build_signature_flags(skm_build* b, uint8_t* out, uint64_t cap) {
    SKM_API_BEGIN
    SKM_CHECK(b && out, SKM_E_ARG, "null argument");
    SKM_CHECK(b->ran, SKM_E_STATE, "no completed run");
    SKM_HIP(hipSetDevice(b->device));
    const uint64_t n = std::min<uint64_t>(cap, b->n_total);
    if (n) SKM_HIP(hipMemcpy(out, b->d_flags.p, n, hipMemcpyDeviceToHost));
    SKM_API_END
}

static void release_work(skm_build* b) {
    SKM_HIP(hipDeviceSynchronize());
    DevBuf* work[] = {
        &b->d_res, &b->d_meta, &b->d_blk2seq, &b->d_glen, &b->d_hist, &b->d_offs, &b->d_partial, &b->d_rbbase,
        &b->d_bstart32, &b->d_bstart, &b->d_owner_start, &b->d_recs_hi, &b->d_recs_lo, &b->d_tmp_hi, &b->d_tmp_lo,
        &b->d_stg_hi, &b->d_stg_lo, &b->d_part_order, &b->d_cur0, &b->d_cur1, &b->d_slices, &b->d_flagbits,
        &b->d_ovf, &b->d_ovf_hi, &b->d_ovf_lo, &b->d_ovf_heads, &b->d_ovf_job, &b->d_ovf_fm, &b->d_jobs,
        &b->d_lens, &b->d_stamps, &b->d_big_desc, &b->d_big_out, &b->d_rhi, &b->d_rlo, &b->d_cnt_send, &b->d_cnt_recv,
        &b->d_seg_start, &b->d_seg_len, &b->d_vstart, &b->d_xs, &b->d_hv_keys, &b->d_hv_rec, &b->d_hv_len, &b->d_hv_s0,
        &b->d_hv_s1, &b->d_sub_tab, &b->d_jobs2, &b->d_jobs3, &b->d_ids, &b->d_bloom, &b->d_posg, &b->d_histg,
        &b->d_npos, &b->d_selrows, &b->d_seloff, &b->d_gstat, &b->d_long_arena, &b->d_long_jobs, &b->d_ovf2, &b->d_plan,
        &b->d_run};
    for (DevBuf* d : work) d->release();
    for (ChainSet* cs : {&b->cs_main, &b->cs_ovf, &b->cs_ovf3})
        for (DevBuf* d : {&cs->hist, &cs->offs, &cs->sorted, &cs->long_off}) d->release();
    for (auto* q : {&b->gsamples, &b->gjobs, &b->gcount})
        for (DevBuf& d : *q) d.release();
    b->work_released = true;
}

int skm_build_kept_db(skm_build* b, const skm_kept_db_opts* opts, skm_db** out) {
    SKM_API_BEGIN
    SKM_CHECK(b && out, SKM_E_ARG, "null argument");
    *out = nullptr;
    SKM_CHECK(b->world == 1, SKM_E_STATE,
              "skm_build_kept_db needs world_size 1: the kept set of a multi-rank build is sharded over the ranks");
    (void)kept_db_slots(0, opts);
    SKM_HIP(hipSetDevice(b->device));
    if (!b->prepared || !b->ran) run_ranks(Ranks{b});
    const uint64_t slots = kept_db_slots(b->n_kept, opts);
    if (opts && opts->release_work && !b->work_released) release_work(b);
    *out = db_from_device_kept(b->d_keys.as<uint64_t>(), b->d_data.as<skm_stored_kmer_data>(), b->n_kept, slots,
                               b->device, b->stream);
    SKM_API_END
}

int skm_build_mph_db(skm_build* b, const skm_mph_db_opts* opts, skm_db** out, skm_mph_stats* stats) {
    SKM_API_BEGIN
    SKM_CHECK(b && out, SKM_E_ARG, "null argument");
    *out = nullptr;
    SKM_CHECK(b->world == 1, SKM_E_STATE,
              "skm_build_mph_db needs world_size 1: the kept set of a multi-rank build is sharded over the ranks");
    skm_mph_db_opts o{};
    o.seed = 1;
    if (opts) o = *opts;
    SKM_HIP(hipSetDevice(b->device));
    if (!b->prepared || !b->ran) run_ranks(Ranks{b});
    uint64_t plan[4];
    mph_db_plan(b->n_kept, plan);
    if (o.release_work && !b->work_released) release_work(b);
    if (b->n_kept < 1024) {
        skm_kept kept{};
        const int rc = skm_build_finish(b, &kept);
        if (rc) return rc;
        try {
            *out = db_from_host_mph(kept.keys, kept.data, kept.n, &o, b->device, stats);
        } catch (...) {
            skm_kept_free(&kept);
            throw;
        }
        skm_kept_free(&kept);
        return SKM_OK;
    }
    SKM_HIP(hipDeviceSynchronize());
    *out = db_from_device_mph(b->d_keys.as<uint64_t>(), b->d_data.as<skm_stored_kmer_data>(), b->n_kept, &o, b->device,
                              stats);
    SKM_API_END
}

void skm_kept_free(skm_kept* k) {
    if (!k) return;
    std::free(k->keys);
    std::free(k->data);
    std::free(k->distinct_functions);
    std::free(k->seqs_with_func);
    std::memset(k, 0, sizeof(*k));
}

void skm_build_destroy(skm_build* b) {
    if (!b) return;
    (void)hipSetDevice(b->device);
    if (b->stream) (void)hipStreamSynchronize(b->stream);
#if defined(SKM_WITH_RCCL)
    if (b->comm) (void)ncclCommDestroy(b->comm);
#endif
    for (auto* x : b->group)
        if (x != b) x->group.clear();
    if (b->stream2) (void)hipStreamSynchronize(b->stream2);
    if (b->stream3) (void)hipStreamSynchronize(b->stream3);
    if (b->stream_tail) (void)hipStreamSynchronize(b->stream_tail);
// ... 68 lines not shown
```

Measured before the change: 12.30 billion.

## Add hierarchical flag-word summary to skip marking already-full sequence flag words

Adds a second-level bitmap in which each bit records whether a 32-bit sequence flag word is already fully set, counting sequences shorter than 8 as always set. Every mark_seq and mark_seqs call checks this summary first and skips the read and the atomicOr when the word is full. The summary is rebuilt between passes by a new kernel, which aims to cut redundant global reads and atomic traffic on hot flag words in later passes. In exchange it adds an eligibility kernel at prepare, a summary kernel per pass, an extra dependent load on every mark, and a new counter.

Result: no change. 12.33 billion, median of 6 (+0.3%).

```diff
diff --git a/signature_kmers_amd/__init__.py b/signature_kmers_amd/__init__.py
--- a/signature_kmers_amd/__init__.py
+++ b/signature_kmers_amd/__init__.py
@@ -375,8 +375,8 @@
         return self.counters()["passes"]
 
     def counters(self) -> dict:
-        v = (C.c_uint64 * 50)()
-        n = lib().skm_build_counters(self._h, v, 50)
+        v = (C.c_uint64 * 51)()
+        n = lib().skm_build_counters(self._h, v, 51)
         names = ["windows", "kept", "overflow_subbuckets", "chain_jobs", "chain_samples", "sequences", "grouped",
                  "overflow_elements", "overflow_kept", "big_groups", "big_kept", "passes", "valid", "giant_chains",
                  "giant_max", "redone", "cap_overflow_scratch", "cap_split", "cap_long_samples", "cap_long_jobs",
@@ -386,7 +386,7 @@
                  "finish_chunks", "finish_select_dev_us", "finish_sort_dev_us", "finish_gather_dev_us",
                  "finish_d2h_dev_us", "finish_max_chunk", "finish_wide_index", "kept_cap",
                  "free_after_prepare", "recs_rot", "overflow_light_subbuckets", "overflow_light_elements",
-                 "groupby_tasks", "groupby_batches"]
+                 "groupby_tasks", "groupby_batches", "flag_words_full"]
         return {names[i]: int(v[i]) for i in range(n)}
 
     def debug_jobs(self, k: int = 64) -> list:
diff --git a/signature_kmers_amd/csrc/skm_build.hip b/signature_kmers_amd/csrc/skm_build.hip
--- a/signature_kmers_amd/csrc/skm_build.hip
+++ b/signature_kmers_amd/csrc/skm_build.hip
@@ -381,17 +381,24 @@
     }
 }
 
-__device__ __forceinline__ void mark_seq(uint32_t* f, uint32_t s) {
+__device__ __forceinline__ bool flag_word_full(const uint32_t* sm, uint32_t s) {
+    return (sm[s >> 10] >> ((s >> 5) & 31u)) & 1u;
+}
+
+__device__ __forceinline__ void mark_seq(uint32_t* f, const uint32_t* sm, uint32_t s) {
+    if (flag_word_full(sm, s)) return;
     uint32_t* w = f + (s >> 5);
     const uint32_t m = 1u << (s & 31u);
     if (!(*w & m)) atomicOr(w, m);
 }
 
 template <int N>
-__device__ __forceinline__ void mark_seqs(uint32_t* w, const uint32_t (&s)[N]) {
+__device__ __forceinline__ void mark_seqs(uint32_t* w, const uint32_t* sm, const uint32_t (&s)[N]) {
     uint32_t cur[N];
 #pragma unroll
-    for (int u = 0; u < N; ++u) cur[u] = s[u] != 0xFFFFFFFFu ? w[s[u] >> 5] : 0xFFFFFFFFu;
+    for (int u = 0; u < N; ++u) cur[u] = s[u] != 0xFFFFFFFFu ? sm[s[u] >> 10] : 0xFFFFFFFFu;
+#pragma unroll
+    for (int u = 0; u < N; ++u) cur[u] = (cur[u] >> ((s[u] >> 5) & 31u)) & 1u ? 0xFFFFFFFFu : w[s[u] >> 5];
 #pragma unroll
     for (int u = 0; u < N; ++u) {
         const uint32_t m = 1u << (s[u] & 31u);
@@ -402,11 +409,13 @@
 struct Seq8 {
     uint32_t s[8];
 };
-__device__ __attribute__((noinline)) void mark_seqs8(uint32_t* w, Seq8 q) { mark_seqs<8>(w, q.s); }
+__device__ __attribute__((noinline)) void mark_seqs8(uint32_t* w, const uint32_t* sm, Seq8 q) {
+    mark_seqs<8>(w, sm, q.s);
+}
 
 template <int N, class V>
 __device__ GRes group_thread(const V& v, uint64_t a, uint32_t c, const uint32_t* __restrict__ glen,
-                             uint32_t* __restrict__ flags) {
+                             uint32_t* __restrict__ flags, const uint32_t* fsum) {
     GRes r;
     r.kept = false;
     uint32_t fn[N], of[N];
@@ -453,7 +462,7 @@
     for (uint32_t t = 0; t < c; ++t) {
         const uint64_t lo = v.lov(a + t);
         const uint32_t s = (uint32_t)(lo >> 36);
-        mark_seq(flags, s);
+        mark_seq(flags, fsum, s);
         if (t >= rb && t < rb + best_c) {
             const uint32_t len = glen[s];
             sum += len;
@@ -471,7 +480,7 @@
 
 template <class V>
 __device__ GRes group_wave(const V& v, uint64_t a, uint32_t c, const uint32_t* __restrict__ glen,
-                           uint32_t* __restrict__ flags) {
+                           uint32_t* __restrict__ flags, const uint32_t* fsum) {
     const uint32_t lane = threadIdx.x & 63u;
     GRes r;
     r.kept = false;
@@ -533,7 +542,7 @@
     uint32_t sum = 0;
     for (uint32_t t = lane; t < c; t += 64) {
         const uint32_t s = (uint32_t)(v.lov(a + t) >> 36);
-        mark_seq(flags, s);
+        mark_seq(flags, fsum, s);
         if (t >= rb && t < rb + best_c) sum += glen[s];
     }
     sum = wave_sum(sum);
@@ -578,7 +587,7 @@
 
 template <class V>
 __device__ bool group_block(const V& v, uint64_t a, uint32_t c, const uint32_t* __restrict__ glen,
-                            uint32_t* __restrict__ flags, uint32_t* heads, uint32_t hcap, uint32_t* s_wave, GRes& r) {
+                            uint32_t* __restrict__ flags, const uint32_t* fsum, uint32_t* heads, uint32_t hcap, uint32_t* s_wave, GRes& r) {
     const uint32_t tid = threadIdx.x, nt = blockDim.x;
     r.kept = false;
     uint32_t H = 0;
@@ -622,7 +631,7 @@
     uint32_t sum = 0;
     for (uint32_t t = tid; t < c; t += nt) {
         const uint32_t s = (uint32_t)(v.lov(a + t) >> 36);
-        mark_seq(flags, s);
+        mark_seq(flags, fsum, s);
         if (t >= rb && t < rb + best_c) sum += glen[s];
     }
     sum = wg_sum(sum, s_wave);
@@ -639,6 +648,7 @@
     RUN_LONG_FLUSHED = 3,
     RUN_ACC_BPK_TASKS = 4,
     RUN_ACC_BPK_BATCHES = 5,
+    RUN_FLAG_WORDS_FULL = 6,
     RUN_SNAP = 28,
     RUN_DEM_TOT = 8,
     RUN_DEM_SPLIT = 9,
@@ -2219,6 +2229,7 @@
     int rem_bits;
     const uint32_t* glen;
     uint32_t* flags;
+    const uint32_t* fsum;
     unsigned long long* ctr;
     uint64_t* out_keys;
     skm_stored_kmer_data* out_data;
@@ -2404,7 +2415,7 @@
     const uint32_t rs = Rs ? (uint32_t)__ffsll((long long)Rs) - 1u : sbase;
     const uint32_t s = (uint32_t)(key >> ELEM_I_BITS) & ((1u << ELEM_S_BITS) - 1u);
     const uint32_t len = (pay & 1u) ? A.glen[s] : len16;
-    if (kept && real) mark_seq(A.flags, s);
+    if (kept && real) mark_seq(A.flags, A.fsum, s);
     const uint32_t x0 = (uint32_t)__shfl((int)len, (int)(rs + cbest - 1), 64);
     const uint32_t x1 = (uint32_t)__shfl((int)len, (int)rs, 64);
     if (kept && inrun && cbest >= 3) L.lens32[2 * a + (rs + cbest - 1 - lane)] = len;
@@ -2510,7 +2521,7 @@
                 L.rank[j] = 0xFFFFu;
             }
         }
-        mark_seqs<LPER>(A.flags, ms);
+        mark_seqs<LPER>(A.flags, A.fsum, ms);
         M = tot >> 13;
         G = tot & 0x1FFFu;
     }
@@ -2818,6 +2829,7 @@
     const uint64_t* recs_lo;
     const uint64_t* tmp_lo;
     uint32_t* flags;
+    const uint32_t* fsum;
     BigOut* out;
 };
 
@@ -2899,9 +2911,9 @@
             Seq8 q;
 #pragma unroll
             for (int u = 0; u < 8; ++u) q.s[u] = ms[u];
-            mark_seqs8(B.flags, q);
+            mark_seqs8(B.flags, B.fsum, q);
         } else {
-            mark_seqs<MC>(B.flags, ms);
+            mark_seqs<MC>(B.flags, B.fsum, ms);
         }
     }
     uint32_t sum = 0;
@@ -3409,11 +3421,11 @@
                 } else {
                     GRes r;
                     if (c <= 4)
-                        r = group_thread<4>(V, a, c, A.glen, A.flags);
+                        r = group_thread<4>(V, a, c, A.glen, A.flags, A.fsum);
                     else if (c <= 8)
-                        r = group_thread<8>(V, a, c, A.glen, A.flags);
+                        r = group_thread<8>(V, a, c, A.glen, A.flags, A.fsum);
                     else
-                        r = group_thread<16>(V, a, c, A.glen, A.flags);
+                        r = group_thread<16>(V, a, c, A.glen, A.flags, A.fsum);
                     stage(r, a);
                 }
             }
@@ -3424,7 +3436,7 @@
                 const uint32_t a = heads[gg];
                 const uint32_t b = gg + 1 < G ? heads[gg + 1] : n;
                 if (b - a > OVF_BLOCK_GROUP) continue;
-                const GRes r = group_wave(V, a, b - a, A.glen, A.flags);
+                const GRes r = group_wave(V, a, b - a, A.glen, A.flags, A.fsum);
                 if ((tid & 63u) == 0) stage(r, a);
             }
             for (uint32_t bi = 0; bi < nbig; ++bi) {
@@ -3433,8 +3445,8 @@
                 const uint32_t b = gg + 1 < G ? heads[gg + 1] : n;
                 if (b - a <= OVF_BLOCK_GROUP) continue;
                 GRes r;
-                if (!group_block(V, a, b - a, A.glen, A.flags, reinterpret_cast<uint32_t*>(s_hi), 2 * CAP, s_wave, r)) {
-                    if (tid < 64) r = group_wave(V, a, b - a, A.glen, A.flags);
+                if (!group_block(V, a, b - a, A.glen, A.flags, A.fsum, reinterpret_cast<uint32_t*>(s_hi), 2 * CAP, s_wave, r)) {
+                    if (tid < 64) r = group_wave(V, a, b - a, A.glen, A.flags, A.fsum);
                 }
                 if (tid == 0) stage(r, a);
                 __syncthreads();
@@ -3902,7 +3914,7 @@
 template <int E>
 __device__ __forceinline__ void heavy_bucket_out(const uint32_t* __restrict__ ks, const uint32_t* __restrict__ ls,
                                                  uint32_t a, uint32_t c, uint32_t nb, uint32_t* __restrict__ out,
-                                                 uint32_t* flags) {
+                                                 uint32_t* flags, const uint32_t* fsum) {
     const uint32_t lane = threadIdx.x & 63u;
     uint64_t v[E];
 #pragma unroll
@@ -3916,7 +3928,7 @@
         const uint32_t i = (uint32_t)e * 64u + lane;
         if (i < nb) {
             out[i] = (uint32_t)v[e];
-            mark_seq(flags, (uint32_t)(v[e] >> 32) - 1u);
+            mark_seq(flags, fsum, (uint32_t)(v[e] >> 32) - 1u);
         }
     }
 }
@@ -4105,7 +4117,7 @@
                     } else {
                         ks[slot] = 0u;
                         ls[slot] = 0u;
-                        mark_seq(A.flags, sq);
+                        mark_seq(A.flags, A.fsum, sq);
                     }
                 }
             }
@@ -4155,7 +4167,7 @@
                     const bool v = f[u] != 0xFFFFFFFFu;
                     const uint32_t s = hr_seq(l[u]);
                     const bool best = f[u] == best_f;
-                    if (v && !best) mark_seq(A.flags, s);
+                    if (v && !best) mark_seq(A.flags, A.fsum, s);
                     wave_hist_add(s_hist, hr_off(l[u]) >> 8, v);
                     if (best) {
                         sum += gl[u];
@@ -4241,13 +4253,13 @@
                 if (nb == 0) continue;
                 uint32_t* out = lens_out + (uint64_t)loff + s_fb[bk];
                 if (c <= 64)
-                    heavy_bucket_out<1>(ks, ls, a, c, nb, out, A.flags);
+                    heavy_bucket_out<1>(ks, ls, a, c, nb, out, A.flags, A.fsum);
                 else if (c <= 128)
-                    heavy_bucket_out<2>(ks, ls, a, c, nb, out, A.flags);
+                    heavy_bucket_out<2>(ks, ls, a, c, nb, out, A.flags, A.fsum);
                 else if (c <= 256)
-                    heavy_bucket_out<4>(ks, ls, a, c, nb, out, A.flags);
+                    heavy_bucket_out<4>(ks, ls, a, c, nb, out, A.flags, A.fsum);
                 else
-                    heavy_bucket_out<8>(ks, ls, a, c, nb, out, A.flags);
+                    heavy_bucket_out<8>(ks, ls, a, c, nb, out, A.flags, A.fsum);
             }
         } else {
             for (uint32_t t0 = 0; t0 < cb; t0 += nt * U) {
@@ -4262,7 +4274,7 @@
                     const uint32_t t = t0 + u * nt + tid;
                     if (t < cb) {
                         lens_out[(uint64_t)loff + t] = A.glen[sv[u]];
-                        mark_seq(A.flags, sv[u]);
+                        mark_seq(A.flags, A.fsum, sv[u]);
                     }
                 }
             }
@@ -4486,6 +4498,30 @@
         const uint32_t n = min(32u, nseq - 32 * w);
         uint8_t* o = flags + 32 * (uint64_t)w;
         for (uint32_t t = 0; t < n; ++t) o[t] = (uint8_t)((v >> t) & 1u);
+    }
+}
+
+__global__ void k_flag_eligible(const uint32_t* __restrict__ glen, uint32_t nseq, uint32_t* __restrict__ elig) {
+    for (uint32_t w = blockIdx.x * blockDim.x + threadIdx.x; w < (nseq + 31) / 32; w += gridDim.x * blockDim.x) {
+        const uint32_t n = min(32u, nseq - 32 * w);
+        uint32_t v = 0;
+        for (uint32_t t = 0; t < n; ++t) v |= (glen[32 * w + t] >= 8u ? 1u : 0u) << t;
+        elig[w] = v;
+    }
+}
+
+__global__ void k_flag_summary(const uint32_t* __restrict__ flags, const uint32_t* __restrict__ elig, uint32_t nwords,
+                               uint32_t nw32, uint32_t* __restrict__ sum, unsigned long long* __restrict__ full) {
+    const uint32_t lane = threadIdx.x & 63u;
+    for (uint32_t w0 = (blockIdx.x * blockDim.x + threadIdx.x) & ~63u; w0 < nw32; w0 += gridDim.x * blockDim.x) {
+        const uint32_t w = w0 + lane;
+        const bool f = w < nwords && (flags[w] | ~elig[w]) == 0xFFFFFFFFu;
+        const unsigned long long m = __ballot(f);
+        if ((lane & 31u) == 0 && w < nw32) {
+            const uint32_t v = sum[w >> 5] | (uint32_t)(m >> lane);
+            sum[w >> 5] = v;
+            if (full && v) atomicAdd(full, (unsigned long long)__popc(v));
+        }
     }
 }
 
@@ -4679,6 +4715,8 @@
     DevBuf d_part_order;
     DevBuf d_cur0, d_cur1, d_slices;
     DevBuf d_flagbits;
+    DevBuf d_flagsum, d_flagelig;
+    uint64_t flag_words_full = 0;
     DevBuf d_keys, d_data, d_ctr, d_flags, d_dfunc, d_swf, d_ovf, d_ovf_hi, d_ovf_lo, d_ovf_heads, d_ovf_job, d_ovf_fm;
     DevBuf d_jobs, d_lens, d_stamps, d_big_desc, d_big_out;
     uint64_t big_cap = 0, n_big = 0, big_kept = 0;
@@ -5487,6 +5525,17 @@
                   "read out and destroyed");
 }
 
+inline uint64_t flag_sum_words(const skm_build* b) { return (((uint64_t)b->n_total + 31) / 32 + 31) / 32; }
+
+void flag_summary(skm_build* b, hipStream_t st, bool count) {
+    const uint32_t nw32 = (uint32_t)(32 * flag_sum_words(b));
+    if (!nw32) return;
+    SKM_LAUNCH(b, k_flag_summary, dim3(std::min<uint32_t>((nw32 + 255) / 256, 1024u)), dim3(256), 0, st,
+               b->d_flagbits.as<uint32_t>(), b->d_flagelig.as<uint32_t>(), (uint32_t)(((uint64_t)b->n_total + 31) / 32), nw32,
+               b->d_flagsum.as<uint32_t>(),
+               count ? b->d_run.as<unsigned long long>() + RUN_FLAG_WORDS_FULL : nullptr);
+}
+
 void prepare(const Ranks& bs) {
     check_not_released(bs);
     bool need = false;
@@ -5584,6 +5633,13 @@
         size_arena(b);
         b->d_flags.ensure(std::max<uint64_t>(b->n_total, 1));
         b->d_flagbits.ensure(4 * ((b->n_total + 31) / 32 + 1));
+        b->d_flagsum.ensure(4 * (flag_sum_words(b) + 1));
+        b->d_flagelig.ensure(4 * (32 * flag_sum_words(b) + 1));
+        SKM_HIP(hipMemsetAsync(b->d_flagelig.p, 0, 4 * (32 * flag_sum_words(b) + 1), b->stream));
+        if (b->n_total)
+            hipLaunchKernelGGL(k_flag_eligible, dim3(1024), dim3(256), 0, b->stream, b->d_glen.as<uint32_t>(),
+                               (uint32_t)b->n_total, b->d_flagelig.as<uint32_t>());
+        SKM_HIP(hipGetLastError());
         {
             size_t fr = 0, tot = 0;
             SKM_HIP(hipMemGetInfo(&fr, &tot));
@@ -5931,6 +5987,7 @@
     A.pshift = KEY_BITS - b->pass_bits;
     A.glen = b->d_glen.as<uint32_t>();
     A.flags = b->d_flagbits.as<uint32_t>();
+    A.fsum = b->d_flagsum.as<uint32_t>();
     A.ctr = ctr_d;
     A.out_keys = b->d_keys.as<uint64_t>();
     A.out_data = b->d_data.as<skm_stored_kmer_data>();
@@ -5987,6 +6044,7 @@
     SKM_LAUNCH(b, k_ovf_plan, dim3(1), dim3(1024), 0, st, P);
     SKM_HIP(hipGetLastError());
     A.skip = plan_d + PLAN_SKIP;
+    if (pass > 0) flag_summary(b, st, false);
     BucketArgs A2 = A, A3 = A;
     OvfScratch S;
     S.hi = b->d_ovf_hi.as<uint64_t>();
@@ -6086,6 +6144,7 @@
     BA.recs_lo = A.recs_lo;
     BA.tmp_lo = A.tmp_lo;
     BA.flags = A.flags;
+    BA.fsum = A.fsum;
     BA.out = b->d_big_out.as<BigOut>();
     SKM_HIP(hipEventRecord(b->ev[15], st));
     if (b->jobs_pending) {
@@ -6209,6 +6268,7 @@
     SKM_HIP(hipMemsetAsync(b->d_run.p, 0, 8 * RUN_SLOTS, st));
     SKM_HIP(hipMemsetAsync(b->d_flags.p, 0, b->n_total ? b->n_total : 1, st));
     SKM_HIP(hipMemsetAsync(b->d_flagbits.p, 0, 4 * ((b->n_total + 31) / 32 + 1), st));
+    SKM_HIP(hipMemsetAsync(b->d_flagsum.p, 0, 4 * (flag_sum_words(b) + 1), st));
     b->d_gstat.ensure(16);
     SKM_HIP(hipMemsetAsync(b->d_gstat.p, 0, 16, st));
     if (b->tune.poison_jobs && b->pass_bits && b->long_jobs_cap)
@@ -6305,6 +6365,7 @@
     if (b->n_total)
         SKM_LAUNCH(b, k_flags_from_bits, dim3(1024), dim3(256), 0, st, b->d_flagbits.as<uint32_t>(),
                    (uint32_t)b->n_total, b->d_flags.as<uint8_t>());
+    flag_summary(b, st, true);
     SKM_HIP(hipMemsetAsync(b->d_dfunc.p, 0, sizeof(uint32_t) * (F ? F : 1), st));
     SKM_HIP(hipMemsetAsync(b->d_swf.p, 0, sizeof(uint32_t) * (F ? F : 1), st));
     const size_t lds_f = F <= 16384 ? sizeof(uint32_t) * F : 0;
@@ -6390,6 +6451,7 @@
     b->ovf_light_sub = R[RUN_ACC_LIGHT_SUB];
     b->ovf_light_elems = R[RUN_ACC_LIGHT_ELEMS];
     b->bpk_tasks = R[RUN_ACC_BPK_TASKS];
+    b->flag_words_full = R[RUN_FLAG_WORDS_FULL];
     b->bpk_batches = R[RUN_ACC_BPK_BATCHES];
     b->n_local = R[RUN_ACC_GROUPED];
     b->ran = true;
@@ -7014,7 +7076,7 @@
 int skm_build_counters(skm_build* b, uint64_t* out, int cap) {
     if (!b || !out) return SKM_E_ARG;
     auto us = [](double sec) { return (uint64_t)(sec * 1e6); };
-    const uint64_t v[50] = {b->n_windows, b->n_kept, b->n_overflow, b->n_jobs, b->n_lens, b->nseq, b->n_local,
+    const uint64_t v[51] = {b->n_windows, b->n_kept, b->n_overflow, b->n_jobs, b->n_lens, b->nseq, b->n_local,
                             b->ovf_elems, b->ovf_kept, b->n_big, b->big_kept, 1ull << b->pass_bits, b->valid_total,
                             b->giant_jobs, b->giant_max, b->n_redo, b->tot_cap, b->split_cap, b->long_cap,
                             b->long_jobs_cap, b->demand[0], b->demand[1], b->demand[2], b->demand[3],
@@ -7026,8 +7088,8 @@
                             (uint64_t)(1e3 * b->handoff.d2h_ms), b->handoff.max_chunk,
                             (uint64_t)b->handoff.wide_index, b->kept_cap, b->free_after_prepare,
                             0ull , b->ovf_light_sub, b->ovf_light_elems, b->bpk_tasks,
-                            b->bpk_batches};
-    int n = std::min(cap, 50);
+                            b->bpk_batches, b->flag_words_full};
+    int n = std::min(cap, 51);
     for (int i = 0; i < n; ++i) out[i] = v[i];
     return n;
 }
@@ -7258,7 +7320,7 @@
         &b->d_res, &b->d_meta, &b->d_blk2seq, &b->d_glen, &b->d_hist, &b->d_offs, &b->d_partial, &b->d_rbbase,
         &b->d_bstart32, &b->d_bstart, &b->d_owner_start, &b->d_recs_hi, &b->d_recs_lo, &b->d_tmp_hi, &b->d_tmp_lo,
         &b->d_stg_hi, &b->d_stg_lo, &b->d_part_order, &b->d_cur0, &b->d_cur1, &b->d_slices, &b->d_flagbits,
-        &b->d_ovf, &b->d_ovf_hi, &b->d_ovf_lo, &b->d_ovf_heads, &b->d_ovf_job, &b->d_ovf_fm, &b->d_jobs,
+        &b->d_flagsum, &b->d_flagelig, &b->d_ovf, &b->d_ovf_hi, &b->d_ovf_lo, &b->d_ovf_heads, &b->d_ovf_job, &b->d_ovf_fm, &b->d_jobs,
         &b->d_lens, &b->d_stamps, &b->d_big_desc, &b->d_big_out, &b->d_rhi, &b->d_rlo, &b->d_cnt_send, &b->d_cnt_recv,
         &b->d_seg_start, &b->d_seg_len, &b->d_vstart, &b->d_xs, &b->d_hv_keys, &b->d_hv_rec, &b->d_hv_len, &b->d_hv_s0,
         &b->d_hv_s1, &b->d_sub_tab, &b->d_jobs2, &b->d_jobs3, &b->d_ids, &b->d_bloom, &b->d_posg, &b->d_histg,
```
